# Fastaxx/Penguin.jl

Measured on AMD Instinct MI355X. Metric: time-steps/sec + SpMV GB/s (% HBM roofline), 3D mono diffusion 512^3, higher is better.
Workload: dtype f64

## Files before the change

### include/penguin_hip.h

```cpp
#ifndef PENGUIN_HIP_H
#define PENGUIN_HIP_H

#include <stddef.h>
#include <stdint.h>

#ifdef __cplusplus
extern "C" {
#endif

typedef struct pg_mesh pg_mesh;
typedef struct pg_capacity pg_capacity;
typedef struct pg_diffops pg_diffops;
typedef struct pg_solver pg_solver;
typedef struct pg_streamvort pg_streamvort;

enum { PG_BODY_BALL = 1, PG_BODY_MULTIBALL = 2, PG_BODY_HALFSPACE = 3, PG_BODY_ELLIPSOID = 4, PG_BODY_PLANE = 5 };
enum { PG_FLAG_COMPLEMENT = 1, PG_FLAG_NO_CENTROIDS = 2 };
enum { PG_CAP_V = 0, PG_CAP_GAMMA = 1, PG_CAP_CELL_TYPES = 2, PG_CAP_A = 3, PG_CAP_B = 4,
       PG_CAP_W = 5, PG_CAP_C_OMEGA = 6, PG_CAP_C_GAMMA = 7,
       PG_CAP_ST_V0 = 8, PG_CAP_ST_V1 = 9, PG_CAP_ST_CT_OMEGA = 10, PG_CAP_ST_CT_GAMMA = 11 };
enum { PG_OP_G = 0, PG_OP_H = 1, PG_OP_WINV = 2,
       PG_OP_C0 = 3 , PG_OP_K0 = 6  };
enum { PG_BC_NONE = 0, PG_BC_DIRICHLET = 1, PG_BC_NEUMANN = 2, PG_BC_ROBIN = 3, PG_BC_PERIODIC = 4 };
enum { PG_KEY_LEFT = 0 , PG_KEY_RIGHT = 1 , PG_KEY_BOTTOM = 2 ,
// ... 15 lines not shown
typedef struct {
  int32_t key;
  int32_t kind;
  double value;
} pg_border_desc;

typedef struct {
  double alpha1, alpha2, g;
  double beta1, beta2, h;
  const double* g_array;
  const double* h_array;
} pg_jump_desc;

typedef struct {
  int32_t method;
  double reltol;
  double abstol;
  int32_t maxiter;
  int32_t check_every;
  int32_t warm_start;
  int32_t restart;
  int32_t precond;
} pg_krylov_opts;
enum { PG_PRECOND_MG = -2 };
enum { PG_PRECOND_MG_CELL = -3 };
enum { PG_PRECOND_POLY_EST = -4 };
enum { PG_PRECOND_MG_STEP = -5 };
#define PG_SPECEST_MARGIN 0.0205

typedef struct {
  int32_t steps;
  int32_t admitted;
  int32_t gershgorin_admits;
  int32_t reserved;
  double g_ritz;
  double g_used;
  double margin;
  double gershgorin;
  double ritz_re_min, ritz_re_max, ritz_im_max;
  double estimate_ms;
} pg_specest_info;

#define PG_MG_MAX_LEVELS 16
typedef struct {
  int32_t levels;
  int32_t tail_level;
  int64_t rows[PG_MG_MAX_LEVELS];
  int64_t nnz[PG_MG_MAX_LEVELS];
  double setup_ms;
  int64_t bytes;
} pg_mg_info;

typedef struct {
  int32_t iters;
  int32_t converged;
  double resnorm;
  double bnorm;
  double extremum;
  double time;
} pg_step_info;

typedef struct {
  int64_t steps;
  int64_t total_iters;
  double t_final;
  double extremum;
  double solve_ms;
  double spmv_ms_total;
  int64_t spmv_launches;
  int64_t unconverged_steps;
  double worst_relres;
  double spmv_lean_ms_total;
  int64_t spmv_lean_launches;
  int64_t poly_degree;
  int64_t half_exits;
  int64_t poly_xspace;
  int64_t products;
  int64_t guess_states_read;
  int64_t poly_f32_launches;
  double poly_f32_ms_total;
  int64_t poly_f32_timed;
  int64_t poly_f32_chains;
  int64_t poly_f32_tail_sum;
} pg_run_info;

typedef struct {
  int64_t n_own;
  int64_t nnz;
  int64_t n_ghost;
  int64_t n_omega;
  int64_t n_gamma;
  int64_t M_global;
  int64_t spmv_bytes;
  int64_t spmv_slices;
  int64_t rows_uniform;
  int64_t rows_pattern;
  int64_t rows_irregular;
  int64_t neumann_ok;
  double gershgorin;
  int64_t spmv_units;
  int64_t rows_marched;
  int64_t rows_matrix;
  int64_t n_ghost_loop;
  int64_t loop_is_compact;
  int64_t rows_edge;
} pg_system_info;

typedef struct {
  int64_t steps;
  int64_t psi_iters;
  int64_t omega_iters;
  int64_t psi_products;
  int64_t omega_products;
  int64_t unconverged;
  double worst_relres;
  double t_final;
  double total_ms;
  double psi_ms;
  double velocity_ms;
  double build_ms;
  double omega_ms;
} pg_streamvort_run_info;

int32_t pg_last_error(char* buf, size_t n);
int32_t pg_init(int32_t device_id);
int32_t pg_get_unique_id(void* out128);
int32_t pg_init_distributed(int32_t device_id, int32_t rank, int32_t nranks, const void* unique_id128);
int32_t pg_finalize(void);
int32_t pg_device_synchronize(void);
int32_t pg_set_profiling(int32_t on);
int32_t pg_device_name(char* buf, size_t n);
int32_t pg_config_string(char* buf, size_t n);

int32_t pg_mesh_create(int32_t N, const int64_t* n, const double* L, const double* x0, pg_mesh** out);
int32_t pg_mesh_destroy(pg_mesh* m);
int32_t pg_mesh_get_centers(const pg_mesh* m, int32_t d, double* out, int64_t len);
int32_t pg_mesh_get_nodes(const pg_mesh* m, int32_t d, double* out, int64_t len);
int32_t pg_mesh_num_border_cells(const pg_mesh* m, int64_t* out);
int32_t pg_mesh_get_border_cells(const pg_mesh* m, int64_t* idx, double* pos, int32_t* key);

int32_t pg_capacity_create_levelset(pg_mesh* m, int32_t body_kind, const double* params, int32_t nparams,
                                    int32_t flags, pg_capacity** out);
int32_t pg_capacity_create_from_arrays(pg_mesh* m, const double* V, const double* const* A,
                                       const double* const* B, const double* const* W, const double* Gamma,
                                       const double* const* C_omega, const double* const* C_gamma,
                                       const double* cell_types, pg_capacity** out);
typedef struct {
  int32_t body_kind;
  int32_t flags;
  int32_t axis;
  int32_t nq;
  double sign;
  double t0, t1;
  const double* nodes;
  double body0[4], body1[4];
} pg_motion_desc;
int32_t pg_capacity_create_spacetime(pg_mesh* m, const pg_motion_desc* motion, pg_capacity** out);
int32_t pg_capacity_set_spacetime(pg_capacity* c, double t0, double t1, const double* V_t0, const double* V_t1,
                                  const double* Ct_omega, const double* Ct_gamma);
int32_t pg_capacity_destroy(pg_capacity* c);
int32_t pg_capacity_get(const pg_capacity* c, int32_t field, int32_t d, double* out, int64_t len);
int32_t pg_capacity_kernel_ms(const pg_capacity* c, double* ms);

int32_t pg_diffops_create(pg_capacity* c, pg_diffops** out);
int32_t pg_diffops_destroy(pg_diffops* o);
int32_t pg_diffops_export_csc(const pg_diffops* o, int32_t which, int64_t* colptr, int64_t* rowval,
                              double* nzval, int64_t* nnz);
int32_t pg_diffops_set_velocity(pg_diffops* o, const double* const* u_omega, const double* u_gamma);
int32_t pg_diffops_set_velocity_spacetime(pg_diffops* o, const double* const* u_omega, const double* u_gamma);
int32_t pg_diffops_grad(const pg_diffops* o, const double* p , double* out );
int32_t pg_diffops_div(const pg_diffops* o, const double* qw , const double* qg ,
                       double* out );

int32_t pg_solver_create_unsteady_mono(pg_capacity* c, pg_diffops* o, const pg_bc_desc* bc_interface,
                                       const pg_border_desc* borders, int32_t nborders, const double* Dcoef,
                                       const double* source, double dt, const double* T0, int32_t scheme,
                                       pg_solver** out);
int32_t pg_solver_create_unsteady_diph(pg_capacity* c1, pg_diffops* o1, pg_capacity* c2, pg_diffops* o2,
                                       const pg_jump_desc* ic, const pg_border_desc* borders, int32_t nborders,
                                       const double* D1, const double* D2, const double* f1, const double* f2,
                                       double dt, const double* T0, int32_t scheme, pg_solver** out);
int32_t pg_solver_create_moving_diph(pg_capacity* c1, pg_diffops* o1, pg_capacity* c2, pg_diffops* o2, const pg_jump_desc* ic,
                                     const pg_border_desc* borders, int32_t nborders, const double* D1, const double* D2,
                                     const double* f1_n, const double* f1_np1, const double* f2_n, const double* f2_np1,
                                     const double* T_prev, pg_solver* previous, int32_t scheme, pg_solver** out);
int32_t pg_solver_create_steady_mono(pg_capacity* c, pg_diffops* o, const pg_bc_desc* bc_interface,
                                     const pg_border_desc* borders, int32_t nborders, const double* Dcoef,
                                     const double* source, pg_solver** out);
// ... 164 lines not shown
```

### penguin/jl_amd/_lib.py

```python
from __future__ import annotations

import ctypes as C
import os
import re
from pathlib import Path

import numpy as np

_HERE = Path(__file__).resolve().parent
LIB_PATH = Path(os.environ["PG_LIB_PATH"]) if os.environ.get("PG_LIB_PATH") else _HERE / "lib" / "libpenguin_hip.so"
HEADER_PATH = _HERE.parent.parent / "include" / "penguin_hip.h"


class PenguinHipError(RuntimeError):
    pass


PG_BODY_BALL, PG_BODY_MULTIBALL, PG_BODY_HALFSPACE, PG_BODY_ELLIPSOID, PG_BODY_PLANE = 1, 2, 3, 4, 5
PG_FLAG_COMPLEMENT, PG_FLAG_NO_CENTROIDS = 1, 2
PG_CAP_V, PG_CAP_GAMMA, PG_CAP_CELL_TYPES, PG_CAP_A, PG_CAP_B, PG_CAP_W, PG_CAP_C_OMEGA, PG_CAP_C_GAMMA = range(8)
PG_CAP_ST_V0, PG_CAP_ST_V1, PG_CAP_ST_CT_OMEGA, PG_CAP_ST_CT_GAMMA = 8, 9, 10, 11
PG_OP_G, PG_OP_H, PG_OP_WINV = 0, 1, 2
PG_OP_C0, PG_OP_K0 = 3, 6
PG_BC_NONE, PG_BC_DIRICHLET, PG_BC_NEUMANN, PG_BC_ROBIN, PG_BC_PERIODIC = 0, 1, 2, 3, 4
PG_KEY = {"left": 0, "right": 1, "bottom": 2, "top": 3, "backward": 4, "forward": 5}
PG_SCHEME = {"BE": 0, "CN": 1, "STEADY": 2}
PG_METHOD = {"bicgstab": 0, "cg": 1, "gmres": 2, "bicgstabl": 3}
PG_METHOD_IDRS = 4
PG_SV_PSI, PG_SV_OMEGA, PG_SV_U, PG_SV_V = 0, 1, 2, 3
PG_PRECOND_MG = -2
PG_PRECOND_MG_CELL = -3
PG_PRECOND_POLY_EST = -4
PG_PRECOND_MG_STEP = -5
PG_SPECEST_MARGIN = 0.0205
PG_MG_MAX_LEVELS = 16

c_double_p = C.POINTER(C.c_double)
c_i64_p = C.POINTER(C.c_int64)
c_i32_p = C.POINTER(C.c_int32)


class pg_bc_desc(C.Structure):
    _fields_ = [("kind", C.c_int32), ("alpha", C.c_double), ("beta", C.c_double), ("value", C.c_double),
                ("value_array", c_double_p)]


class pg_border_desc(C.Structure):
    _fields_ = [("key", C.c_int32), ("kind", C.c_int32), ("value", C.c_double)]


class pg_jump_desc(C.Structure):
    _fields_ = [("alpha1", C.c_double), ("alpha2", C.c_double), ("g", C.c_double), ("beta1", C.c_double),
                ("beta2", C.c_double), ("h", C.c_double), ("g_array", c_double_p), ("h_array", c_double_p)]


class pg_motion_desc(C.Structure):
    _fields_ = [("body_kind", C.c_int32), ("flags", C.c_int32), ("axis", C.c_int32), ("nq", C.c_int32), ("sign", C.c_double),
                ("t0", C.c_double), ("t1", C.c_double), ("nodes", c_double_p), ("body0", C.c_double * 4),
                ("body1", C.c_double * 4)]


class pg_krylov_opts(C.Structure):
    _fields_ = [("method", C.c_int32), ("reltol", C.c_double), ("abstol", C.c_double), ("maxiter", C.c_int32),
                ("check_every", C.c_int32), ("warm_start", C.c_int32), ("restart", C.c_int32), ("precond", C.c_int32)]


class pg_step_info(C.Structure):
    _fields_ = [("iters", C.c_int32), ("converged", C.c_int32), ("resnorm", C.c_double), ("bnorm", C.c_double),
                ("extremum", C.c_double), ("time", C.c_double)]


class pg_run_info(C.Structure):
    _fields_ = [("steps", C.c_int64), ("total_iters", C.c_int64), ("t_final", C.c_double), ("extremum", C.c_double),
                ("solve_ms", C.c_double), ("spmv_ms_total", C.c_double), ("spmv_launches", C.c_int64),
                ("unconverged_steps", C.c_int64), ("worst_relres", C.c_double), ("spmv_lean_ms_total", C.c_double),
                ("spmv_lean_launches", C.c_int64), ("poly_degree", C.c_int64), ("half_exits", C.c_int64),
                ("poly_xspace", C.c_int64), ("products", C.c_int64), ("guess_states_read", C.c_int64),
                ("poly_f32_launches", C.c_int64), ("poly_f32_ms_total", C.c_double), ("poly_f32_timed", C.c_int64),
                ("poly_f32_chains", C.c_int64), ("poly_f32_tail_sum", C.c_int64)]


class pg_system_info(C.Structure):
    _fields_ = [("n_own", C.c_int64), ("nnz", C.c_int64), ("n_ghost", C.c_int64), ("n_omega", C.c_int64),
                ("n_gamma", C.c_int64), ("M_global", C.c_int64), ("spmv_bytes", C.c_int64), ("spmv_slices", C.c_int64),
                ("rows_uniform", C.c_int64), ("rows_pattern", C.c_int64), ("rows_irregular", C.c_int64),
                ("neumann_ok", C.c_int64), ("gershgorin", C.c_double), ("spmv_units", C.c_int64),
                ("rows_marched", C.c_int64), ("rows_matrix", C.c_int64), ("n_ghost_loop", C.c_int64),
                ("loop_is_compact", C.c_int64), ("rows_edge", C.c_int64)]


class pg_streamvort_run_info(C.Structure):
    _fields_ = [("steps", C.c_int64), ("psi_iters", C.c_int64), ("omega_iters", C.c_int64), ("psi_products", C.c_int64),
                ("omega_products", C.c_int64), ("unconverged", C.c_int64), ("worst_relres", C.c_double), ("t_final", C.c_double),
                ("total_ms", C.c_double), ("psi_ms", C.c_double), ("velocity_ms", C.c_double), ("build_ms", C.c_double),
                ("omega_ms", C.c_double)]


class pg_mg_info(C.Structure):
    _fields_ = [("levels", C.c_int32), ("tail_level", C.c_int32), ("rows", C.c_int64 * PG_MG_MAX_LEVELS),
                ("nnz", C.c_int64 * PG_MG_MAX_LEVELS), ("setup_ms", C.c_double), ("bytes", C.c_int64)]


class pg_specest_info(C.Structure):
    _fields_ = [("steps", C.c_int32), ("admitted", C.c_int32), ("gershgorin_admits", C.c_int32), ("reserved", C.c_int32),
                ("g_ritz", C.c_double), ("g_used", C.c_double), ("margin", C.c_double), ("gershgorin", C.c_double),
                ("ritz_re_min", C.c_double), ("ritz_re_max", C.c_double), ("ritz_im_max", C.c_double), ("estimate_ms", C.c_double)]


def declared_symbols() -> list[str]:
    txt = HEADER_PATH.read_text()
    return sorted(set(re.findall(r"\bint32_t\s+(pg_[a-z0-9_]+)\s*\(", txt)))


_lib = None
hip_runtime_source = "system"


def _share_the_hip_runtime_with_torch() -> None:
    global hip_runtime_source
    import sys

    if "torch" in sys.modules:
        hip_runtime_source = "already mapped by torch"
        return
    if os.environ.get("PG_HIP_RUNTIME", "auto") == "system":
        return
    import importlib.util

    try:
        spec = importlib.util.find_spec("torch")
    except (ImportError, ValueError):
        spec = None
    if spec is None or not spec.submodule_search_locations:
        return
    libdir = Path(list(spec.submodule_search_locations)[0]) / "lib"
    if not (libdir / "libamdhip64.so").exists():
        return
    mode = C.RTLD_GLOBAL if hasattr(C, "RTLD_GLOBAL") else 0
    for name in ("libhsa-runtime64.so", "libamdhip64.so"):
        if (libdir / name).exists():
            C.CDLL(str(libdir / name), mode=mode)
    hip_runtime_source = "torch wheel"


def lib() -> C.CDLL:
    global _lib
    if _lib is None:
        if not LIB_PATH.exists():
            raise PenguinHipError(
                f"{LIB_PATH} is missing: build it with `python -c 'import __graft_entry__ as g; g.build()'` "
                "(hipcc --offload-arch=gfx950).  penguin.jl_amd has no CPU fallback.")
        _share_the_hip_runtime_with_torch()
        _lib = C.CDLL(str(LIB_PATH), mode=C.RTLD_GLOBAL if hasattr(C, "RTLD_GLOBAL") else 0)
        for name in declared_symbols():
            getattr(_lib, name).restype = C.c_int32
    return _lib


def check(status: int) -> None:
    if status != 0:
        buf = C.create_string_buffer(4096)
        lib().pg_last_error(buf, 4096)
        raise PenguinHipError(buf.value.decode("utf-8", "replace"))


def dptr(a: np.ndarray):
    assert a.dtype == np.float64 and a.flags["C_CONTIGUOUS"]
    return a.ctypes.data_as(c_double_p)


def iptr(a: np.ndarray):
# ... 93 lines not shown
def debug_mg_step_aggregates(handle, which: int, level: int) -> np.ndarray:
    n = C.c_int64(0)
    check(lib().pg_debug_mg_step_aggregates(handle, C.c_int32(which), C.c_int32(level), C.byref(n), None))
    agg = np.zeros(max(n.value, 1), dtype=np.int32)
    check(lib().pg_debug_mg_step_aggregates(handle, C.c_int32(which), C.c_int32(level), C.byref(n), agg.ctypes.data_as(c_i32_p)))
    return agg[: n.value]


def debug_mg_step_level_csr(handle, which: int, level: int):
    n, nnz = C.c_int64(0), C.c_int64(0)
    w = C.c_int32(which)
    check(lib().pg_debug_mg_step_level_csr(handle, w, C.c_int32(level), C.byref(n), C.byref(nnz), None, None, None))
    rowptr, col, val = np.zeros(n.value + 1, dtype=np.int64), np.zeros(max(nnz.value, 1), dtype=np.int64), np.zeros(max(nnz.value, 1))
    check(lib().pg_debug_mg_step_level_csr(handle, w, C.c_int32(level), C.byref(n), C.byref(nnz), iptr(rowptr), iptr(col), dptr(val)))
    return rowptr, col[: nnz.value], val[: nnz.value]


def debug_mg_step_apply(handle, which: int, r: np.ndarray) -> np.ndarray:
    r = np.ascontiguousarray(r, dtype=np.float64)
    z = np.zeros_like(r)
    check(lib().pg_debug_mg_step_apply(handle, C.c_int32(which), dptr(r), dptr(z)))
    return z


def solver_spectral_estimate(handle, which: int = 0, run: bool = True) -> dict:
    info = pg_specest_info()
    check(lib().pg_solver_spectral_estimate(handle, C.c_int32(which | (0 if run else 4)), C.byref(info)))
    return {k: getattr(info, k) for k, _ in pg_specest_info._fields_ if k != "reserved"}


def debug_specest_hessenberg(handle, which: int = 0, run: bool = True) -> np.ndarray:
    w = C.c_int32(which | (0 if run else 4))
    k = C.c_int32(0)
    check(lib().pg_debug_specest_hessenberg(handle, w, C.byref(k), None))
    H = np.zeros((k.value + 1) * max(k.value, 1))
    check(lib().pg_debug_specest_hessenberg(handle, w, C.byref(k), dptr(H)))
    return H[: (k.value + 1) * k.value].reshape((k.value + 1, k.value), order="F")


DEBUG_SPMV_SENTINEL = 0x7FF8C0DE5EED0BAD
DEBUG_SPMV_GUARD = 64


def debug_spmv_sizes(handle, which: int) -> tuple[int, int, int, int]:
    n, nv, nnz, grid = C.c_int64(0), C.c_int64(0), C.c_int64(0), C.c_int32(0)
    check(lib().pg_debug_spmv_sizes(handle, C.c_int32(which), C.byref(n), C.byref(nv), C.byref(nnz), C.byref(grid)))
    return n.value, nv.value, nnz.value, grid.value


def loop_system_csr(handle, which: int):
    n, _, nnz, _ = debug_spmv_sizes(handle, which)
    rowptr, col, val = np.zeros(n + 1, dtype=np.int64), np.zeros(max(nnz, 1), dtype=np.int64), np.zeros(max(nnz, 1))
    check(lib().pg_solver_get_system_csr(handle, C.c_int32(which), iptr(rowptr), iptr(col), dptr(val), None, None))
    return rowptr, col[:nnz], val[:nnz]


def debug_spmv_apply(handle, which: int, variant: int, mode: int, x, aux=None, dotx=None, base=None, pc=(0.0, 0.0, 0.0),
                     fold: int = 0, done: int = 0, repeat: int = 1) -> dict:
    n, nv, _, grid = debug_spmv_sizes(handle, which)

    def arr(a, length, name):
        if a is None:
            return None, None
        a = np.ascontiguousarray(a, dtype=np.float64)
        if a.size != length:
            raise ValueError(f"debug_spmv_apply: {name} has {a.size} entries, the matrix needs {length}")
        return a, dptr(a)

    xs, xp = arr(x, nv, "x")
    auxs, auxp = arr(aux, n, "aux")
    dots, dotp = arr(dotx, n, "dotx")
    bases, basep = arr(base, n, "base")
    y = np.zeros(n + DEBUG_SPMV_GUARD)
    partials = np.zeros((5, grid))
    sums, folded = np.zeros(5), np.zeros(5)
    ticket = C.c_int64(-1)
    check(lib().pg_debug_spmv_apply(handle, C.c_int32(which), C.c_int32(variant), C.c_int32(mode), xp, auxp, dotp, basep,
                                    C.c_double(pc[0]), C.c_double(pc[1]), C.c_double(pc[2]), C.c_int32(fold), C.c_int32(done),
                                    C.c_int32(repeat), dptr(y), dptr(partials), dptr(sums), dptr(folded), C.byref(ticket)))
    return {"y": y, "partials": partials, "slot_sums": sums, "folded": folded, "ticket": ticket.value, "grid": grid, "n": n}


DEBUG_SPMV_SENTINEL_F32 = 0x7FC5EED0
TYPED_FIRST, TYPED_MIDDLE, TYPED_HANDOVER = 1, 2, 3


def debug_spmv_apply_typed(handle, which: int, kind: int, x, base=None, pc=(0.0, 0.0, 0.0), sigma: float = 1.0, done: int = 0) -> dict:
    n, nv, _, _ = debug_spmv_sizes(handle, which)
    want_x = np.float64 if kind == TYPED_FIRST else np.float32
    want_b = {TYPED_FIRST: None, TYPED_MIDDLE: np.float32, TYPED_HANDOVER: np.float64}[kind]
    x = np.ascontiguousarray(x)
    if x.dtype != want_x or x.size != nv:
        raise ValueError(f"debug_spmv_apply_typed: x must be {nv} x {np.dtype(want_x).name}")
    if (base is None) != (want_b is None):
        raise ValueError("debug_spmv_apply_typed: base goes with kinds 2 and 3, and only with them")
    bp = None
    if base is not None:
        base = np.ascontiguousarray(base)
        if base.dtype != want_b or base.size != n:
            raise ValueError(f"debug_spmv_apply_typed: base must be {n} x {np.dtype(want_b).name}")
        bp = base.ctypes.data_as(C.c_void_p)
    y64 = np.zeros(n + DEBUG_SPMV_GUARD) if kind == TYPED_HANDOVER else None
    y32 = np.zeros(n + DEBUG_SPMV_GUARD, dtype=np.float32) if kind != TYPED_HANDOVER else None
    p32 = np.zeros(n + DEBUG_SPMV_GUARD, dtype=np.float32) if kind == TYPED_FIRST else None
    ptr = lambda a: None if a is None else a.ctypes.data_as(C.c_void_p)
    check(lib().pg_debug_spmv_apply_typed(handle, C.c_int32(which), C.c_int32(kind), x.ctypes.data_as(C.c_void_p), bp,
                                          C.c_double(pc[0]), C.c_double(pc[1]), C.c_double(pc[2]), C.c_double(sigma), C.c_int32(done),
                                          ptr(y64), ptr(y32), ptr(p32)))
    return {"y": y64 if kind == TYPED_HANDOVER else y32, "p32": p32}
```

### penguin/jl_amd/csrc/pg_common.h

```cpp
#pragma once
#include <hip/hip_runtime.h>
#include "pg_rccl.h"

#include <chrono>
#include <cstdint>
#include <cstdio>
#include <cstring>
#include <stdexcept>
#include <string>
#include <vector>

#include "../../../include/penguin_hip.h"

namespace pg {

using i64 = int64_t;
using i32 = int32_t;

struct Error : std::runtime_error {
  using std::runtime_error::runtime_error;
};

void set_last_error(const std::string& msg);

#define PG_HIP(expr)                                                                              \
  do {                                                                                            \
    hipError_t _e = (expr);                                                                       \
    if (_e != hipSuccess)                                                                         \
      throw pg::Error(std::string("HIP error: ") + hipGetErrorString(_e) + " at " + __FILE__ + ":" + \
                      std::to_string(__LINE__) + " (" #expr ")");                                 \
  } while (0)

#define PG_NCCL(expr)                                                                             \
  do {                                                                                            \
    ncclResult_t _e = (expr);                                                                     \
    if (_e != ncclSuccess)                                                                        \
      throw pg::Error(std::string("RCCL error: ") + pg::rccl::api().GetErrorString(_e) + " at " + __FILE__ + ":" + \
                      std::to_string(__LINE__) + " (" #expr ")");                                 \
  } while (0)

#define PG_REQUIRE(cond, msg)                                   \
  do {                                                          \
    if (!(cond)) throw pg::Error(std::string(msg));             \
  } while (0)

#define PG_API_BEGIN try {
#define PG_API_END                                  \
  return 0;                                         \
  }                                                 \
  catch (const std::exception& e) {                 \
    pg::set_last_error(e.what());                   \
    return 1;                                       \
  }                                                 \
  catch (...) {                                     \
    pg::set_last_error("unknown exception");        \
    return 2;                                       \
  }

struct Config {
  bool debug = false;
  int alloc_poison = 0;
  int async_alloc = 0;
  int alloc_guard = 0;
  long long pool_limit_mb = 0;
  bool poly = true;
  int poly_degree = 6;
  bool poly_adapt = true;
  double poly_margin = 1.0;
  double poly_slack = -1.0;
  int poly_hist = 3;
  bool poly_trend = true;
  int poly_maxdeg = 0;
  int poly_mindeg = 4;
  bool poly_f32 = true;
  int poly_f32_tail = -1;
  int profile_sample = 3;
  bool gamma_elim = true;
  bool diag_elim = true;
  double diag_elim_frac = 0.0005;
  int spmv_variant = 70;
  int spmv_xcd = 1;
  int spmv_strip = 16;
  int spmv_march_k = 0;
  int spmv_minrun = 24;
  bool spmv_march = true;
  bool spmv_edges = true;
  int spmv_tile_units = 0;
  int spmv_blocks_per_cu = 0;
  bool halo_overlap = true;
  int guess_n = 4;
  int guess_depth = 7;
  bool guess_defer = true;
  bool guess_always = false;
  int guess_monitor = 256;
  double guess_pass_cost = 0.34;
  double guess_gain = 0.8;
  bool speculate_product = true;
  int mg_tail_rows = 2048;
  int unit_order = 0;
};
const Config& config();

struct LocalComm;

struct Context {
  bool inited = false;
  LocalComm* local = nullptr;
  int device = 0;
  hipStream_t stream = nullptr;
  hipStream_t comm_stream = nullptr;
  hipEvent_t ev_fork = nullptr, ev_join = nullptr;
  int rank = 0, nranks = 1;
  ncclComm_t comm = nullptr;
  ncclComm_t comm_halo = nullptr;
  bool profiling = false;
  std::string device_name;
};
Context& ctx();
void require_init();
void set_thread_context(Context* c);
Context* thread_context();
LocalComm* local_comm_create(int nranks);
void local_comm_destroy(LocalComm* c);
void comm_allreduce_sum_f64(double* dev, int count, hipStream_t st);
void comm_allreduce_max_f64(double* dev, int count, hipStream_t st);
void comm_allreduce_sum_u64(unsigned long long* dev, i64 count, hipStream_t st);

void* dev_alloc(size_t bytes);
void dev_free(void* p);
void dev_cache_release();
struct AsyncAllocScope {
  AsyncAllocScope();
  ~AsyncAllocScope();
};

template <class T>
struct DevBuf {
  T* p = nullptr;
  i64 n = 0;
  DevBuf() = default;
  explicit DevBuf(i64 n_) { alloc(n_); }
  DevBuf(const DevBuf&) = delete;
  DevBuf& operator=(const DevBuf&) = delete;
  DevBuf(DevBuf&& o) noexcept : p(o.p), n(o.n) { o.p = nullptr; o.n = 0; }
  DevBuf& operator=(DevBuf&& o) noexcept {
    if (this != &o) { release(); p = o.p; n = o.n; o.p = nullptr; o.n = 0; }
    return *this;
  }
  ~DevBuf() { release(); }
  void release() {
    if (p) dev_free(p);
    p = nullptr; n = 0;
  }
  void alloc(i64 n_) {
    release();
    n = n_;
    if (n > 0) p = static_cast<T*>(dev_alloc(sizeof(T) * static_cast<size_t>(n) + 64));
// ... 121 lines not shown
```

### penguin/jl_amd/csrc/pg_context.hip

```cpp
#include "pg_common.h"

#include <cxxabi.h>
#include <execinfo.h>

#include <atomic>
#include <map>
#include <mutex>
#include <unordered_map>
#include <unordered_set>
#include "pg_host_algos.h"

#include <algorithm>
#include <array>
#include <memory>
#include <set>

namespace pg {

static thread_local std::string g_last_error;
void set_last_error(const std::string& msg) { g_last_error = msg; }

Context& ctx() {
  static Context c;
  Context* t = thread_context();
  return t ? *t : c;
}

const Config& config() {
  static const Config c = [] {
    Config k;
    auto geti = [](const char* name, long long dflt) { const char* v = getenv(name); return v ? atoll(v) : dflt; };
    auto getd = [](const char* name, double dflt) { const char* v = getenv(name); return v ? atof(v) : dflt; };
    k.debug = getenv("PG_DEBUG") != nullptr;
    k.alloc_poison = (int)geti("PG_ALLOC_POISON", 0);
    k.async_alloc = (int)geti("PG_ASYNC_ALLOC", 0);
    k.alloc_guard = (int)geti("PG_ALLOC_GUARD", 0);
    k.pool_limit_mb = geti("PG_POOL_LIMIT_MB", 0);
    k.poly = geti("PG_POLY", 1) != 0;
    k.poly_degree = (int)geti("PG_POLY_DEGREE", 6);
    k.poly_adapt = geti("PG_POLY_ADAPT", getenv("PG_POLY_DEGREE") ? 0 : 1) != 0;
    k.poly_margin = getd("PG_POLY_MARGIN", 1.0);
    k.poly_slack = getd("PG_POLY_SLACK", -1.0);
    k.poly_hist = (int)std::max<long long>(1, std::min<long long>(3, geti("PG_POLY_HIST", 3)));
    k.poly_maxdeg = (int)geti("PG_POLY_MAXDEG", 0);
    k.poly_mindeg = (int)std::max<long long>(2, std::min<long long>(8, geti("PG_POLY_MINDEG", 4)));
    k.poly_trend = geti("PG_POLY_TREND", 1) != 0;
    k.poly_f32 = geti("PG_POLY_F32", 1) != 0;
    k.poly_f32_tail = (int)std::max<long long>(-1, std::min<long long>(64, geti("PG_POLY_F32_TAIL", -1)));
    k.profile_sample = (int)std::max<long long>(1, geti("PG_PROFILE_SAMPLE", 3));
    k.gamma_elim = geti("PG_GAMMA_ELIM", 1) != 0;
    k.diag_elim = geti("PG_DIAG_ELIM", 1) != 0;
    k.diag_elim_frac = getd("PG_DIAG_ELIM_FRAC", 0.0005);
    k.spmv_variant = (int)geti("PG_SPMV_VARIANT", 70);
    k.spmv_xcd = (int)geti("PG_SPMV_XCD", 1);
    k.spmv_strip = (int)geti("PG_SPMV_STRIP", 16);
    k.spmv_march_k = (int)geti("PG_SPMV_MARCH_K", 0);
    k.spmv_minrun = (int)geti("PG_SPMV_MINRUN", 24);
    k.spmv_march = geti("PG_SPMV_MARCH", 1) != 0;
    k.spmv_edges = geti("PG_SPMV_EDGES", 1) != 0;
    k.spmv_tile_units = (int)geti("PG_SPMV_TILE_UNITS", 0);
    k.spmv_blocks_per_cu = (int)geti("PG_SPMV_BLOCKS_PER_CU", 0);
    k.halo_overlap = geti("PG_HALO_OVERLAP", 1) != 0;
    k.speculate_product = geti("PG_SPECULATE", 1) != 0;
    k.guess_n = (int)std::max<long long>(0, std::min<long long>(4, geti("PG_GUESS_STATES", 4)));
    k.guess_depth = (int)std::max<long long>(1, std::min<long long>(7, geti("PG_GUESS_DEPTH", 7)));
    k.mg_tail_rows = (int)std::max<long long>(0, geti("PG_MG_TAIL_ROWS", 2048));
    k.guess_monitor = (int)std::max<long long>(1, geti("PG_GUESS_MONITOR", 256));
    k.guess_pass_cost = getd("PG_GUESS_PASS_COST", 0.34);
    k.guess_always = geti("PG_GUESS_ALWAYS", 0) != 0;
    k.guess_defer = geti("PG_GUESS_DEFER", 1) != 0;
    k.guess_gain = getd("PG_GUESS_GAIN", 0.8);
    k.unit_order = (int)geti("PG_SPMV_UNIT_ORDER", 0);
    return k;
  }();
  return c;
}

void require_init() {
  if (!ctx().inited)
    throw Error("penguin_hip: not initialised (call pg_init / pg_init_distributed first)");
}

static void init_device(int device_id) {
  Context& c = ctx();
  int ndev = 0;
  hipError_t e = hipGetDeviceCount(&ndev);
  if (e != hipSuccess || ndev <= 0)
    throw Error("penguin_hip: no HIP device visible -- this library has no CPU fallback");
  PG_REQUIRE(device_id >= 0 && device_id < ndev, "penguin_hip: device id out of range");
  PG_HIP(hipSetDevice(device_id));
  hipDeviceProp_t prop;
  PG_HIP(hipGetDeviceProperties(&prop, device_id));
  c.device = device_id;
  c.device_name = std::string(prop.name) + " (" + prop.gcnArchName + ")";
  if (!c.stream) PG_HIP(hipStreamCreateWithFlags(&c.stream, hipStreamNonBlocking));
  if (!c.comm_stream) PG_HIP(hipStreamCreateWithFlags(&c.comm_stream, hipStreamNonBlocking));
  c.inited = true;
}

}

using namespace pg;

namespace pg {
namespace {
thread_local int t_async_scope = 0;
std::mutex g_alloc_mutex;
struct BlockCache {
  std::multimap<size_t, void*> free_blocks;
  std::unordered_map<void*, size_t> owned;
  size_t free_bytes = 0;
};
BlockCache g_cache;
constexpr size_t CACHE_TRIM_BYTES = (size_t)48 << 30;

size_t round_block(size_t bytes) {
  const size_t q = bytes >= ((size_t)2 << 20) ? ((size_t)2 << 20) : 4096;
  return (bytes + q - 1) / q * q;
}

bool cache_wanted(const Context& c, size_t bytes) {
  const int mode = config().async_alloc;
  if (mode < 0 || !c.inited || !c.stream || c.local) return false;
  if (!(t_async_scope > 0 || mode > 0)) return false;
  const long long lim = config().pool_limit_mb;
  return lim <= 0 || bytes < ((size_t)lim << 20);
}

void poison(void* p, size_t bytes) {
  if (!config().alloc_poison || !p || bytes == 0) return;
// ... 157 lines not shown
  c.rank = 0;
  c.nranks = 1;
  PG_API_END
}

int32_t pg_get_unique_id(void* out128) {
  PG_API_BEGIN
  static_assert(sizeof(ncclUniqueId) == 128, "ncclUniqueId is expected to be 128 bytes");
  ncclUniqueId id;
  PG_NCCL(rccl::api().GetUniqueId(&id));
  std::memcpy(out128, &id, sizeof(id));
  PG_API_END
}

int32_t pg_init_distributed(int32_t device_id, int32_t rank, int32_t nranks, const void* unique_id128) {
  PG_API_BEGIN
  Context& c = ctx();
  PG_REQUIRE(nranks >= 1 && rank >= 0 && rank < nranks, "pg_init_distributed: bad rank / nranks");
  init_device(device_id);
  c.rank = rank;
  c.nranks = nranks;
  if (nranks > 1 || unique_id128 != nullptr) {
    PG_REQUIRE(unique_id128 != nullptr, "pg_init_distributed: unique id required when nranks > 1");
    ncclUniqueId id;
    std::memcpy(&id, unique_id128, sizeof(id));
    const rccl::Api& R = rccl::api();
    PG_NCCL(R.CommInitRank(&c.comm, nranks, id, rank));
    bool split_ok = false;
    if (R.CommSplit) {
      split_ok = R.CommSplit(c.comm, 0, rank, &c.comm_halo, nullptr) == ncclSuccess && c.comm_halo != nullptr;
      if (!split_ok) c.comm_halo = nullptr;
    }
    if (!split_ok) {
      ncclUniqueId id2;
      if (rank == 0) PG_NCCL(R.GetUniqueId(&id2));
      DevBuf<char> buf((i64)sizeof(id2));
      if (rank == 0) buf.upload(reinterpret_cast<const char*>(&id2), (i64)sizeof(id2));
      PG_NCCL(R.Broadcast(buf.p, buf.p, sizeof(id2), ncclChar, 0, c.comm, c.stream));
      buf.download(reinterpret_cast<char*>(&id2), (i64)sizeof(id2));
      PG_NCCL(R.CommInitRank(&c.comm_halo, nranks, id2, rank));
    }
  }
  PG_API_END
}

int32_t pg_finalize(void) {
  PG_API_BEGIN
  Context& c = ctx();
  if (c.inited) {
    (void)hipDeviceSynchronize();
    if (c.comm_halo) { (void)rccl::api().CommDestroy(c.comm_halo); c.comm_halo = nullptr; }
    if (c.comm) { (void)rccl::api().CommDestroy(c.comm); c.comm = nullptr; }
    dev_cache_release();
    if (c.stream) { (void)hipStreamDestroy(c.stream); c.stream = nullptr; }
    if (c.comm_stream) { (void)hipStreamDestroy(c.comm_stream); c.comm_stream = nullptr; }
    if (c.ev_fork) { (void)hipEventDestroy(c.ev_fork); c.ev_fork = nullptr; }
    if (c.ev_join) { (void)hipEventDestroy(c.ev_join); c.ev_join = nullptr; }
    c.inited = false;
  }
  PG_API_END
}

int32_t pg_device_synchronize(void) {
  PG_API_BEGIN
  require_init();
  PG_HIP(hipDeviceSynchronize());
  PG_API_END
}

int32_t pg_set_profiling(int32_t on) {
  PG_API_BEGIN
  ctx().profiling = on != 0;
  PG_API_END
}

int32_t pg_config_string(char* buf, size_t n) {
  PG_API_BEGIN
  const Config& k = config();
  char tmp[1024];
  snprintf(tmp, sizeof(tmp),
           "spmv_variant=%d spmv_xcd=%d spmv_strip=%d spmv_unit_order=%d spmv_march=%d spmv_edges=%d spmv_march_k=%d spmv_minrun=%d spmv_tile_units=%d "
           "spmv_blocks_per_cu=%d halo_overlap=%d speculate=%d poly=%d poly_degree=%d poly_adapt=%d "
           "poly_margin=%g poly_slack=%g poly_hist=%d poly_trend=%d poly_maxdeg=%d poly_f32=%d poly_f32_tail=%d gamma_elim=%d diag_elim=%d "
           "guess_states=%d guess_depth=%d guess_defer=%d async_alloc=%d cache_limit_mb=%lld alloc_poison=%d alloc_guard=%d profile_sample=%d debug=%d",
           k.spmv_variant, k.spmv_xcd, k.spmv_strip, k.unit_order, (int)k.spmv_march, (int)k.spmv_edges, k.spmv_march_k, k.spmv_minrun, k.spmv_tile_units,
           k.spmv_blocks_per_cu, (int)k.halo_overlap, (int)k.speculate_product, (int)k.poly, k.poly_degree, (int)k.poly_adapt,
           k.poly_margin, k.poly_slack, k.poly_hist, (int)k.poly_trend, k.poly_maxdeg, (int)k.poly_f32, k.poly_f32_tail,
           (int)k.gamma_elim, (int)k.diag_elim, k.guess_n, k.guess_depth, (int)k.guess_defer, k.async_alloc, k.pool_limit_mb, k.alloc_poison, k.alloc_guard, k.profile_sample, (int)k.debug);
  if (buf && n > 0) {
    std::strncpy(buf, tmp, n - 1);
    buf[n - 1] = 0;
  }
  PG_API_END
}

int32_t pg_device_name(char* buf, size_t n) {
  PG_API_BEGIN
  require_init();
  if (buf && n > 0) {
    std::strncpy(buf, ctx().device_name.c_str(), n - 1);
    buf[n - 1] = 0;
  }
  PG_API_END
}

int32_t pg_mesh_create(int32_t N, const int64_t* n, const double* L, const double* x0, pg_mesh** out) {
  PG_API_BEGIN
  PG_REQUIRE(N >= 1 && N <= 3, "pg_mesh_create: N must be 1, 2 or 3");
  PG_REQUIRE(out != nullptr, "pg_mesh_create: out is NULL");
  PG_REQUIRE(n != nullptr && L != nullptr, "pg_mesh_create: n / L is NULL");
  std::unique_ptr<pg_mesh> guard(new pg_mesh());
  pg_mesh* m = guard.get();
  m->N = N;
  for (int d = 0; d < N; ++d) {
    PG_REQUIRE(n[d] >= 1, "pg_mesh_create: n_d must be >= 1");
    m->n[d] = n[d];
    m->L[d] = L[d];
    m->x0[d] = x0 ? x0[d] : 0.0;
    const double h = L[d] / static_cast<double>(n[d]);
    m->centers[d].resize(n[d]);
    m->nodes[d].resize(n[d] + 1);
    for (i64 j = 0; j < n[d]; ++j) m->centers[d][j] = m->x0[d] + static_cast<double>(j) * h;
    for (i64 j = 0; j <= n[d]; ++j) m->nodes[d][j] = m->x0[d] + (static_cast<double>(j) + 0.5) * h;
  }
  if (ctx().inited) {
    for (int d = 0; d < N; ++d) {
      m->d_nodes[d].alloc(n[d] + 1);
      m->d_nodes[d].upload(m->nodes[d].data(), n[d] + 1);
    }
  }
  *out = guard.release();
  PG_API_END
}

int32_t pg_mesh_destroy(pg_mesh* m) {
  PG_API_BEGIN
  delete m;
  PG_API_END
}

int32_t pg_mesh_get_centers(const pg_mesh* m, int32_t d, double* out, int64_t len) {
  PG_API_BEGIN
  PG_REQUIRE(m && d >= 0 && d < m->N && len == m->n[d], "pg_mesh_get_centers: bad arguments");
  std::memcpy(out, m->centers[d].data(), sizeof(double) * len);
  PG_API_END
}

int32_t pg_mesh_get_nodes(const pg_mesh* m, int32_t d, double* out, int64_t len) {
  PG_API_BEGIN
  PG_REQUIRE(m && d >= 0 && d < m->N && len == m->n[d] + 1, "pg_mesh_get_nodes: bad arguments");
  std::memcpy(out, m->nodes[d].data(), sizeof(double) * len);
  PG_API_END
}

int32_t pg_mesh_num_border_cells(const pg_mesh* m, int64_t* out) {
  PG_API_BEGIN
  PG_REQUIRE(m && out, "pg_mesh_num_border_cells: bad arguments");
  i64 all = 1, inner = 1;
  for (int d = 0; d < m->N; ++d) {
    all *= m->n[d];
    inner *= std::max<i64>(m->n[d] - 2, 0);
  }
  *out = all - inner;
  PG_API_END
}

int32_t pg_mesh_get_border_cells(const pg_mesh* mc, int64_t* idx, double* pos, int32_t* key) {
  PG_API_BEGIN
  PG_REQUIRE(mc, "pg_mesh_get_border_cells: mesh is NULL");
  pg_mesh* m = const_cast<pg_mesh*>(mc);
  mesh_build_border(m);
// ... 102 lines not shown
```

### penguin/jl_amd/csrc/pg_host_algos.h

```cpp
#pragma once
#include <algorithm>
#include <cmath>
#include <cstdint>
#include <vector>

namespace pghost {

inline void partition_planes(const int64_t* weight, int64_t nplanes, int nranks, int64_t* bounds) {
  std::vector<double> cum(nplanes + 1, 0.0);
  for (int64_t k = 0; k < nplanes; ++k) cum[k + 1] = cum[k] + static_cast<double>(weight[k]) + 1.0;
  const double total = cum[nplanes];
  bounds[0] = 0;
  for (int r = 1; r < nranks; ++r) {
    const double target = total * r / nranks;
    int64_t k = std::lower_bound(cum.begin(), cum.end(), target) - cum.begin();
    if (k > 0 && (target - cum[k - 1]) < (cum[k] - target)) --k;
    const int64_t lo = bounds[r - 1] + 1;
    const int64_t hi = nplanes - (nranks - r);
    bounds[r] = std::min(std::max(k, lo), hi);
  }
  bounds[nranks] = nplanes;
}

constexpr int SLAB_MAX_KINDS = 4;
struct SlabNumbering {
  int K = 0;
  int64_t n_own = 0, n_ghost = 0;
  int64_t cnt_own[SLAB_MAX_KINDS], off_own[SLAB_MAX_KINDS], cntL[SLAB_MAX_KINDS], offL[SLAB_MAX_KINDS], cntU[SLAB_MAX_KINDS],
      offU[SLAB_MAX_KINDS], sendL_off[SLAB_MAX_KINDS], sendL_cnt[SLAB_MAX_KINDS], sendU_off[SLAB_MAX_KINDS], sendU_cnt[SLAB_MAX_KINDS];
};
inline void slab_numbering(int K, const int64_t* posO, const int64_t* posU, const int64_t* posFE, const int64_t* posLB,
                           const int64_t* tot, bool has_lower, bool has_upper, SlabNumbering& out) {
  out.K = K;
  int64_t off = 0;
  for (int k = 0; k < K; ++k) {
    out.cntL[k] = posO[k];
    out.cnt_own[k] = posU[k] - posO[k];
    out.cntU[k] = tot[k] - posU[k];
    out.off_own[k] = off;
    off += out.cnt_own[k];
  }
  out.n_own = off;
  for (int k = 0; k < K; ++k) { out.offL[k] = off; off += out.cntL[k]; }
  for (int k = 0; k < K; ++k) { out.offU[k] = off; off += out.cntU[k]; }
  out.n_ghost = off - out.n_own;
  for (int k = 0; k < K; ++k) {
    out.sendL_off[k] = out.off_own[k];
    out.sendL_cnt[k] = has_lower ? posFE[k] - posO[k] : 0;
    out.sendU_cnt[k] = has_upper ? posU[k] - posLB[k] : 0;
    out.sendU_off[k] = out.off_own[k] + out.cnt_own[k] - out.sendU_cnt[k];
  }
  for (int k = K; k < SLAB_MAX_KINDS; ++k)
    out.cnt_own[k] = out.off_own[k] = out.cntL[k] = out.offL[k] = out.cntU[k] = out.offU[k] = out.sendL_off[k] = out.sendL_cnt[k] =
        out.sendU_off[k] = out.sendU_cnt[k] = 0;
}

struct SlabPlanes { int64_t s0, s1, a0, a1; };
inline SlabPlanes slab_planes(int64_t p0, int64_t p1, int64_t nplanes, int halo) {
  SlabPlanes g;
  g.s0 = p0 - halo < 0 ? 0 : p0 - halo;
  g.s1 = p1 + halo > nplanes ? nplanes : p1 + halo;
  g.a0 = p0 - 1 < 0 ? 0 : p0 - 1;
  g.a1 = p1 + 1 > nplanes ? nplanes : p1 + 1;
  return g;
}

struct MRun {
  int r0, len, cnt;
};
struct RowRange {
  int64_t a, b;
  int cnt;
};
struct MarchGeometry {
  int K, KS;
  int REC;
  int W;
  int INFO;
  int kmax;
  int64_t ext0 = 0, lines = 0;
  int strip = 0;
  int unit_order = 0;
};

struct EdgeCands {
  const int* rows = nullptr;
  int64_t nrows = 0;
  const int* rowptr = nullptr;
  const int* col = nullptr;
};
constexpr int EDGE_SLOTS = 8;
constexpr int EDGE_PER_END = 8;
constexpr int EDGE_PER_UNIT = 64;
constexpr int EDGE_REC = 34;
struct EdgePlan {
  EdgeCands cand;
  std::vector<int> meta;
  int64_t rows_e = 0;
  int64_t slots_read = 0;
};

inline int64_t march_order(int64_t cell, int64_t ext0, int64_t lines, int strip) {
  const int64_t line = (cell / ext0) % lines, plane = cell / (ext0 * lines);
  return (line / strip) * ((int64_t)1 << 20) + plane;
}

inline void plan_march_units(int64_t n, const std::vector<MRun>& runs, const std::vector<int>& info, const MarchGeometry& geo,
                             std::vector<int>& mrec, std::vector<RowRange>& fallback, int64_t& rows_m,
                             std::vector<int64_t>* okeys = nullptr, EdgePlan* edges = nullptr) {
  typedef int64_t i64;
  rows_m = 0;
  const i64 nr = (i64)runs.size();
  const int RI = geo.INFO;
  auto off = [&](i64 i, int k) { return info[RI * i + k]; };
  auto same_values = [&](i64 i, i64 j, int cnt) {
    for (int k = 0; k < 2 * cnt; ++k)
      if (info[RI * i + 8 + k] != info[RI * j + 8 + k]) return false;
    return true;
  };
  std::vector<char> ok(nr, 0);
  for (i64 i = 0; i < nr; ++i) {
    const int cnt = runs[i].cnt;
    bool good = (cnt == 5 || cnt == 7) && off(i, 0) == 1 && off(i, 1) == -1 && off(i, cnt - 1) == 0;
    if (good) {
      const int up_e = cnt - 3, dn_e = cnt - 2;
      good = off(i, up_e) > 1 && off(i, dn_e) < -1;
      if (good && cnt == 7) good = off(i, 2) > 1 && off(i, 2) < off(i, up_e) && off(i, 3) < -1 && off(i, 3) > off(i, dn_e);
    }
    ok[i] = good;
    if (!ok[i]) fallback.push_back(RowRange{runs[i].r0, (i64)runs[i].r0 + runs[i].len, cnt});
  }
  std::vector<int> succ(nr, -1), pred(nr, -1);
  for (i64 i = 0; i < nr; ++i) {
    if (!ok[i]) continue;
    const int cnt = runs[i].cnt, up_off = off(i, cnt - 3);
    const i64 lo = (i64)runs[i].r0 + up_off, hi = lo + runs[i].len;
    i64 j = std::upper_bound(runs.begin(), runs.end(), lo, [](i64 v, const MRun& r) { return v < (i64)r.r0; }) - runs.begin();
    if (j > 0) --j;
    i64 best = -1, best_ov = 0;
    for (; j < nr && (i64)runs[j].r0 < hi; ++j) {
      const i64 a = runs[j].r0, b = a + runs[j].len;
      if (b <= lo || j == i || !ok[j] || pred[j] >= 0 || runs[j].cnt != cnt || off(j, cnt - 2) != -up_off || !same_values(i, j, cnt)) continue;
      const i64 ov = std::min(hi, b) - std::max(lo, a);
      if (ov > best_ov) { best_ov = ov; best = j; }
    }
    if (best >= 0) { succ[i] = (int)best; pred[best] = (int)i; }
  }
  struct Unit { int key; int64_t order; int64_t sub; std::vector<int> rec; std::vector<int> erows; };
  const bool want_edges = edges && edges->cand.nrows > 0 && geo.REC >= EDGE_REC + 2 + geo.K;
  std::vector<char> claimed(want_edges ? (size_t)edges->cand.nrows : 0, 0);
  auto edge_row = [&](i64 row, i64 run, int cnt, int& smap, i64& q) {
    const EdgeCands& c = edges->cand;
    if (row < 0 || row >= n) return false;
    q = std::lower_bound(c.rows, c.rows + c.nrows, (int)row) - c.rows;
    if (q >= c.nrows || c.rows[q] != row || claimed[q]) return false;
    const int a = c.rowptr[q], len = c.rowptr[q + 1] - a;
    if (len < 1 || len > cnt) return false;
    auto inside = [&](int s) { const i64 t = row + off(run, s); return t >= 0 && t < n; };
    int sl = 0;
    smap = len << 24;
    for (int e = 0; e < len; ++e) {
      const i64 cc = c.col[a + e];
      if (cc < 0 || cc >= n) return false;
      while (sl < cnt && off(run, sl) != cc - row) {
        if (!inside(sl)) return false;
        ++sl;
      }
      if (sl == cnt) return false;
      smap |= sl << (3 * e);
      ++sl;
    }
    for (; sl < cnt; ++sl)
      if (!inside(sl)) return false;
    return true;
  };
  const bool aligned = geo.unit_order == 1 && geo.strip > 0 && geo.ext0 > 0 && geo.lines > 0 && RI > 24;
  auto plane_of = [&](i64 run) -> i64 {
    const i64 cell = info[RI * run + 24];
    return cell >= 0 ? cell / (geo.ext0 * geo.lines) : -1;
  };
  std::vector<Unit> units;
  auto safe = [&](i64 idx0) { return idx0 >= 0 && idx0 + 130 <= n + 8; };
  std::vector<i64> chain, B;
  for (i64 h = 0; h < nr; ++h) {
    if (!ok[h] || pred[h] >= 0) continue;
    chain.clear(); B.clear();
    const int cnt = runs[h].cnt;
    const bool Y = cnt == 7;
    const int up_e = cnt - 3, dn_e = cnt - 2;
    i64 base = runs[h].r0;
    for (i64 i = h; i >= 0; i = succ[i]) {
      chain.push_back(i);
      B.push_back(base);
      base += off(i, up_e);
    }
    const i64 L = (i64)chain.size();
    i64 cmin = 0, cmax = 0;
    for (i64 k = 0; k < L; ++k) {
      const i64 a = runs[chain[k]].r0 - B[k], b = a + runs[chain[k]].len;
      cmin = k == 0 ? a : std::min(cmin, a);
      cmax = k == 0 ? b : std::max(cmax, b);
    }
    for (i64 W = cmin - 1; W + 1 < cmax; W += geo.W) {
      auto range = [&](i64 k, i64& lo, i64& hi) {
        const i64 a = runs[chain[k]].r0 - B[k], b = a + runs[chain[k]].len;
        lo = std::max(a, W + 1);
        hi = std::min(b, W + 1 + geo.W);
        return lo < hi;
      };
      i64 k = 0;
      while (k < L) {
        i64 lo, hi;
        if (!range(k, lo, hi)) { ++k; continue; }
        i64 k1 = k;
        while (k1 < L && k1 - k < geo.kmax && range(k1, lo, hi)) {
          ++k1;
          if (aligned && Y && k1 < L && plane_of(chain[k1]) >= 0 && plane_of(chain[k1]) % geo.kmax == 0) break;
        }
        const int K = (int)(k1 - k);
        bool fits = safe(B[k] + off(chain[k], dn_e) + W) && safe(B[k1 - 1] + off(chain[k1 - 1], up_e) + W);
        for (i64 q = k; q < k1 && fits; ++q) {
          fits = safe(B[q] + W);
          if (Y) fits = fits && safe(B[q] + W + off(chain[q], 2)) && safe(B[q] + W + off(chain[q], 3));
        }
        if (!fits) {
          for (i64 q = k; q < k1; ++q) {
            range(q, lo, hi);
            fallback.push_back(RowRange{B[q] + lo, B[q] + hi, cnt});
          }
          k = k1;
          continue;
        }
        Unit u;
        u.rec.assign(geo.REC, 0);
        range(k, lo, hi);
        u.key = (int)(B[k] + lo);
        u.order = 0;
        u.sub = 0;
        if (Y && geo.strip > 0 && geo.ext0 > 0 && geo.lines > 0 && RI > 24) {
          const i64 cell = info[RI * chain[k] + 24];
          if (cell >= 0) {
            u.order = march_order(cell, geo.ext0, geo.lines, geo.strip);
            if (aligned) {
              const i64 line = (cell / geo.ext0) % geo.lines, plane = cell / (geo.ext0 * geo.lines);
              u.order = (line / geo.strip) * ((i64)1 << 20) + plane / geo.kmax;
              const i64 x0 = cell % geo.ext0 + ((B[k] + lo) - (i64)runs[chain[k]].r0);
              u.sub = (x0 / geo.W) * ((i64)1 << 20) + line;
            }
          }
        }
        const int Kp = K <= geo.KS ? geo.KS : geo.K;
        u.rec[0] = Kp | (cnt << 8);
        u.rec[1] = u.key;
        for (int q = 0; q < 2 * cnt; ++q) u.rec[2 + q] = info[RI * chain[k] + 8 + q];
        u.rec[16] = (int)(B[k] + off(chain[k], dn_e) + W);
        u.rec[17] = (int)(B[k1 - 1] + off(chain[k1 - 1], up_e) + W);
        int hi_max = 0;
        for (int i = 0; i < K; ++i) {
          const i64 q = k + i;
          range(q, lo, hi);
          hi_max = std::max(hi_max, (int)(hi - W));
          u.rec[18 + 4 * i] = (int)(B[q] + W);
          u.rec[19 + 4 * i] = Y ? off(chain[q], 3) : 0;
          u.rec[20 + 4 * i] = Y ? off(chain[q], 2) : 0;
          u.rec[21 + 4 * i] = (int)(lo - W) | ((int)(hi - W) << 8);
          rows_m += hi - lo;
        }
        if (want_edges) {
          int budget = EDGE_PER_UNIT;
          for (int i = 0; i < K; ++i) {
            const i64 q = k + i, run = chain[q];
            range(q, lo, hi);
            const i64 a = runs[run].r0 - B[q], b = a + runs[run].len;
            std::vector<int> lows, highs;
            int smap = 0;
            i64 cq = 0;
            if (lo == a)
              for (i64 pos = lo - 1; pos >= W + 1 && lo - pos <= EDGE_PER_END && budget > 0 && edge_row(B[q] + pos, run, cnt, smap, cq); --pos) {
                claimed[cq] = 1; --budget;
                lows.push_back(smap); lows.push_back((int)(B[q] + pos));
              }
            if (hi == b)
              for (i64 pos = hi; pos <= W + geo.W && pos - hi < EDGE_PER_END && budget > 0 && edge_row(B[q] + pos, run, cnt, smap, cq); ++pos) {
                claimed[cq] = 1; --budget;
                highs.push_back((int)(B[q] + pos)); highs.push_back(smap);
              }
            const int nlo = (int)lows.size() / 2, nhi = (int)highs.size() / 2;
            u.rec[EDGE_REC + 2 + i] = nlo | (nhi << 8) | ((int)(u.erows.size() / 2) << 16);
            u.erows.insert(u.erows.end(), lows.rbegin(), lows.rend());
            u.erows.insert(u.erows.end(), highs.begin(), highs.end());
            hi_max = std::max(hi_max, (int)(hi - W) + nhi);
          }
          u.rec[EDGE_REC + 1] = (int)(u.erows.size() / 2);
          for (int i = K; i < Kp; ++i) u.rec[EDGE_REC + 2 + i] = u.rec[EDGE_REC + 1] << 16;
        }
        u.rec[0] |= std::min(64, hi_max / 2 + 1) << 16;
        for (int i = K; i < Kp; ++i) {
          u.rec[18 + 4 * i] = u.rec[17];
          u.rec[19 + 4 * i] = 0;
          u.rec[20 + 4 * i] = 0;
          u.rec[21 + 4 * i] = 1 | (1 << 8);
        }
        units.push_back(std::move(u));
        k = k1;
      }
    }
  }
  std::sort(units.begin(), units.end(), [](const Unit& a, const Unit& b) {
    if (a.order != b.order) return a.order < b.order;
    return a.sub != b.sub ? a.sub < b.sub : a.key < b.key;
  });
  mrec.reserve(units.size() * geo.REC);
  if (want_edges) {
    i64 first = 0;
    edges->meta.clear();
    edges->slots_read = 0;
    for (auto& u : units) {
      const int ne = (int)(u.erows.size() / 2);
      u.rec[EDGE_REC] = (int)first;
      for (int e = 0; e < ne; ++e) {
        edges->meta.push_back(u.erows[2 * e]);
        edges->meta.push_back((int)(EDGE_SLOTS * first + 2 * e));
        edges->meta.push_back(2 * ne);
        edges->meta.push_back(u.erows[2 * e + 1]);
      }
      first += ne;
      edges->slots_read += (int64_t)ne * ((((u.rec[0] >> 8) & 255) + 1) & ~1);
    }
    edges->rows_e = first;
  }
  for (auto& u : units) mrec.insert(mrec.end(), u.rec.begin(), u.rec.end());
  if (okeys) {
    okeys->clear();
    okeys->reserve(units.size());
    for (auto& u : units) okeys->push_back(u.order * ((i64)1 << 32) + u.key);
  }
}

inline void plan_tiles(const std::vector<int64_t>& ukey, const std::vector<int64_t>& skey, int T, std::vector<int>& tab) {
  typedef int64_t i64;
  const i64 nu = (i64)ukey.size(), ns = (i64)skey.size();
  tab.assign((size_t)8 * (T + 1) * 2, 0);
  for (int q = 0; q < 8; ++q) {
    const i64 u0 = nu * q / 8, u1 = nu * (q + 1) / 8, s0 = ns * q / 8, s1 = ns * (q + 1) / 8;
    i64 sprev = s0;
    for (int t = 0; t <= T; ++t) {
      const i64 u = u0 + (u1 - u0) * t / T;
      i64 sl;
      if (t == 0) sl = s0;
      else if (t == T || u >= nu) sl = s1;
      else sl = std::lower_bound(skey.begin(), skey.end(), ukey[u]) - skey.begin();
      sl = std::min(std::max(sl, sprev), s1);
      sprev = sl;
      tab[((size_t)q * (T + 1) + t) * 2] = (int)u;
      tab[((size_t)q * (T + 1) + t) * 2 + 1] = (int)sl;
    }
  }
}

inline bool mg_dense_inverse(int n, const double* a, double* inv) {
  if (n <= 0) return true;
  const size_t w = 2 * (size_t)n;
  std::vector<long double> m((size_t)n * w, 0.0L);
  for (int i = 0; i < n; ++i) {
    for (int j = 0; j < n; ++j) m[i * w + j] = a[(size_t)i * n + j];
    m[i * w + n + i] = 1.0L;
  }
  for (int c = 0; c < n; ++c) {
    int piv = c;
    long double best = m[c * w + c] < 0 ? -m[c * w + c] : m[c * w + c];
    for (int i = c + 1; i < n; ++i) {
      const long double v = m[i * w + c] < 0 ? -m[i * w + c] : m[i * w + c];
      if (v > best) { best = v; piv = i; }
    }
    if (!(best > 0.0L)) return false;
    if (piv != c)
      for (size_t j = 0; j < w; ++j) std::swap(m[c * w + j], m[piv * w + j]);
    const long double d = 1.0L / m[c * w + c];
    for (size_t j = 0; j < w; ++j) m[c * w + j] *= d;
// ... 309 lines not shown
```

### penguin/jl_amd/csrc/pg_krylov.h

```cpp
#pragma once
#include <functional>

#include "pg_system.h"

namespace pg {

struct MgHierarchy;

struct XGuess {
  const double* zbase = nullptr;
  const double* zr[8] = {nullptr, nullptr, nullptr, nullptr, nullptr, nullptr, nullptr, nullptr};
  const double* coef = nullptr;
};

struct KrylovWork {
  i64 n = 0, nvec = 0;
  DevBuf<double> r, rhat, p, v, t;
  DevBuf<double> partials;
  DevBuf<double> sc;
  double* h_sc = nullptr;
  int grid = 1;
  DevBuf<unsigned> ticket;
  double last_rate2 = 0.0;
  int last_iters = 0;
  const void* adapt_matrix = nullptr;
  int adapt_m = 0, adapt_h = 0;
  const void* need_matrix = nullptr;
  double need_hist[3] = {0.0, 0.0, 0.0};
  const void* fail_matrix = nullptr;
  int fail_deg = 0, good_deg = 0;
  double fail_L = 0.0;
  int fail_wait = 0, fail_backoff = 1;
  const int* scatter = nullptr;
  MgHierarchy* mg = nullptr;
  XGuess xguess;
  bool p_in_rhat = false;
  bool start_folded = false;
  const int* moved_flag = nullptr;
  int moved_stamp = 0;
  DevBuf<double> ya, yb, wa, wb;
  DevBuf<float> fa, fb, p32;
  const void* mix_matrix = nullptr;
  double mix_sigma = 0.0, mix_need = 0.0;
  int mix_wait = 0;
  DevBuf<double> gm_basis, gm, gm_partials;
  int gm_m = -1;
  DevBuf<double> bl_vecs, bl, bl_partials;
  int bl_l = -1;
  i64 bl_stride = 0;
  DevBuf<double> id_vecs, id, id_partials;
  int id_s = -1;
  i64 id_stride = 0;
  std::function<void()> after_first_batch;
  hipEvent_t ev_poll = nullptr;
  void init(i64 n_own, i64 n_vec);
  ~KrylovWork();
};

struct SolveStats {
  int iters = 0;
  int converged = 0;
  double resnorm = 0.0, bnorm = 0.0;
  double spmv_ms = 0.0, spmv_lean_ms = 0.0;
  i64 spmv_launches = 0, spmv_lean_launches = 0;
  int poly_degree = 0;
  int half_exit = 0;
  int poly_xspace = 0;
  i64 products = 0;
  int polls = 0;
  i64 f32_launches = 0, f32_timed = 0, f32_chains = 0, f32_tail_sum = 0;
  double f32_ms = 0.0;
};

void halo_exchange(const Numbering& nb, const Slab& slab, double* vec, hipStream_t st);
void halo_begin(const Numbering& nb, const Slab& slab, double* vec, hipStream_t st);
void halo_end(hipStream_t st);
void spmv(const CsrMatrix& A, const double* x, double* y, hipStream_t st);
void spmv_halo(const CsrMatrix& A, const Numbering& nb, const Slab& slab, double* x, double* y, hipStream_t st);
void krylov_solve(const CsrMatrix& A, const Numbering& nb, const Slab& slab, const double* b, double* x,
                  KrylovWork& w, const pg_krylov_opts& opts, SolveStats& stats, const double* x0 = nullptr,
                  const double* Ax0 = nullptr, bool preinit = false);

bool krylov_uses_polynomial(const CsrMatrix& A, const pg_krylov_opts& opts);

extern int g_poly_give_up;

void gmres_solve(const CsrMatrix& A, const Numbering& nb, const Slab& slab, const double* b, double* x, KrylovWork& w,
                 const pg_krylov_opts& opts, SolveStats& stats);

void bicgstabl_solve(const CsrMatrix& A, const Numbering& nb, const Slab& slab, const double* b, double* x, KrylovWork& w,
                     const pg_krylov_opts& opts, SolveStats& stats);
void idrs_solve(const CsrMatrix& A, const Numbering& nb, const Slab& slab, const double* b, double* x, KrylovWork& w,
                const pg_krylov_opts& opts, SolveStats& stats, const double* x0 = nullptr, const double* Ax0 = nullptr);
const char* krylov_method_refusal(int method);

}
```

### penguin/jl_amd/csrc/pg_krylov.hip

```cpp
#include "pg_host_algos.h"
#include "pg_krylov.h"
#include "pg_multigrid.h"
#include "pg_spmv.h"
#include "pg_specest.h"

using namespace pg;

namespace pg { extern double g_host_wait_us; }

namespace {


__global__ __launch_bounds__(BLOCK) void k_bicg_init(i64 n, i64 nvec, const double* __restrict__ b,
                                                     const double* x0, const double* __restrict__ Ax0,
                                                     double* x, double* __restrict__ r,
                                                     double* __restrict__ rhat, double* __restrict__ p,
                                                     double* __restrict__ v, double* __restrict__ partials,
                                                     const double* __restrict__ ds) {
  __shared__ double s_red[BLOCK / 64];
  double acc = 0.0, accb = 0.0, accw = 0.0;
  for (i64 i = blockIdx.x * (i64)BLOCK + threadIdx.x; i < nvec; i += (i64)gridDim.x * BLOCK) {
    if (i < n) {
      const double bi = b[i];
      const double ri = x0 ? bi - Ax0[i] : bi;
// ... 576 lines not shown
  int maxiter = opts.maxiter;
  if (maxiter <= 0) {
    maxiter = 100000;
  }
  struct HookReset { KrylovWork& w; ~HookReset() { w.after_first_batch = nullptr; } } hook_reset{w};
  const bool p_in_rhat = w.p_in_rhat && preinit && opts.method == PG_METHOD_BICGSTAB;
  w.p_in_rhat = false;
  const XGuess xg = w.xguess;
  w.xguess = XGuess();
  const bool start_folded = w.start_folded && preinit && opts.method == PG_METHOD_BICGSTAB;
  w.start_folded = false;
  const int* moved_flag = w.moved_flag;
  const int moved_stamp = w.moved_stamp;
  w.moved_flag = nullptr;
  const bool fused_start = !start_folded && preinit && opts.method == PG_METHOD_BICGSTAB && cx.nranks == 1 && !cx.comm;
  if (!fused_start && !start_folded)
    hipLaunchKernelGGL(k_sc_reset, dim3(1), dim3(S_COUNT), 0, st, w.sc.p, opts.reltol * opts.reltol, opts.abstol * opts.abstol);
  SpmvTimer timer(cx.profiling);

  const bool cg = opts.method == PG_METHOD_CG;
  const Config& cfg = config();
  const bool poly_env = cfg.poly;
  const int degree_env = cfg.poly_degree;
  int m = 0;
  const bool by_estimate = est_opt && !A.poly_ok && !A.poly_gave_up && A.est.tried && A.est.admitted;
  if (poly_env && precond >= 0 && !cg && (A.poly_ok || by_estimate) && spmv_supports_preconditioner_product() && n > 0)
    m = std::min(precond > 0 ? precond : degree_env, MAX_POLY_DEGREE);
  const bool adapt_env = cfg.poly_adapt;
  const bool adaptive = adapt_env && m >= 2 && precond == 0 && preinit;
  int expect_halves = 0;
  if (adaptive && w.adapt_matrix == &A && w.adapt_m >= 2) { m = w.adapt_m; expect_halves = w.adapt_h; }
  if (m < 2) m = 0;
  const bool poly = m > 0;
  MgHierarchy* const mgh = w.mg;
  w.mg = nullptr;
  const bool mg = mg_any_precond(opts.precond);
  if (mg) {
    PG_REQUIRE(!cg, "multigrid preconditioner refused: the method must be BiCGStab");
    PG_REQUIRE(spmv_supports_preconditioner_product(), "multigrid preconditioner refused: the x-space loop needs the slice kernel (PG_SPMV_VARIANT)");
    mg_require_one_rank_of(opts.precond);
    PG_REQUIRE(mgh && !w.scatter && !xg.zbase && n > 0,
               mg_is_step(opts.precond)
                   ? "multigrid preconditioner refused: this solve has no hierarchy (the full systems of the unsteady monophasic "
                     "diffusion time loop only)"
                   : "multigrid preconditioner refused: this solve has no hierarchy (steady monophasic "
                     "diffusion systems and the stream-function solve only)");
    PG_REQUIRE(mgh->rule == mg_rule_of_any(opts.precond) && mgh->matrix == &A,
               std::string("multigrid preconditioner: the hierarchy handed over was not built for precond = ") +
                   mg_precond_name_of(opts.precond));
  }
  const bool pre = poly || mg;
  stats.poly_degree = m;
  stats.poly_xspace = poly ? 1 : 0;
  PG_REQUIRE(!w.scatter || (poly && preinit), "a compact system needs the polynomial path and a prepared start");
  double tau[MAX_POLY_DEGREE];
  if (poly) {
    const double g = std::min(std::max(by_estimate ? A.est.g_used : A.gersh, 0.05), 0.95);
    double lam[MAX_POLY_DEGREE];
    for (int k = 0; k < m; ++k) lam[k] = 1.0 + g * std::cos(M_PI * (2.0 * k + 1.0) / (2.0 * m));
    for (int k = 0, lo = 0, hi = m - 1; k < m; ++k) tau[k] = 1.0 / ((k & 1) ? lam[hi--] : lam[lo++]);
  }
  if (pre && w.ya.n < nvec) {
    w.ya.alloc(nvec); w.wa.alloc(nvec); w.wb.alloc(nvec); w.yb.alloc(nvec);
    w.ya.zero(); w.wa.zero(); w.wb.zero(); w.yb.zero();
  }
  pghost::MixedChain mc;
  bool mixed = false;
  double mix_sigma = 1.0;
  double mtau[MAX_POLY_DEGREE];
  if (poly && cfg.poly_f32 && cx.nranks == 1 && !cx.comm && !A.halo_needed && spmv_supports_typed_chain() && w.mix_matrix == &A &&
      w.mix_sigma > 0.0) {
    const double g = std::min(std::max(by_estimate ? A.est.g_used : A.gersh, 0.05), 0.95);
    int j = cfg.poly_f32_tail >= 0 ? cfg.poly_f32_tail : pghost::mixed_chain_tail(w.mix_need, g, m);
    if (j >= 0 && w.mix_wait > 0 && cfg.poly_f32_tail < 0) j += 2;
    if (w.mix_wait > 0) --w.mix_wait;
    if (j >= 0 && pghost::mixed_chain_schedule(m, g, j, mc)) {
      mixed = true;
      mix_sigma = w.mix_sigma;
      for (int i = 0; i < m; ++i) mtau[i] = 1.0 / pghost::mixed_root(m, g, mc.order[i]);
      if (w.fa.n < nvec) {
        w.fa.alloc(nvec); w.fb.alloc(nvec); w.p32.alloc(nvec);
        w.fa.zero(); w.fb.zero(); w.p32.zero();
      }
    }
  }
  bool mixed_ran = false;
  const bool half_test = m >= 3 || mg;
  PG_REQUIRE(!xg.zbase || (poly && p_in_rhat && w.scatter), "an unformed extrapolated state needs the polynomial loop on a compact system");
  PG_REQUIRE(!preinit || !cg, "preinit is a BiCGStab path");
  if (!cg) {
    if (!preinit)
      hipLaunchKernelGGL(k_bicg_init, dim3(G), dim3(BLOCK), 0, st, n, nvec, b, x0, Ax0, x, w.r.p, w.rhat.p, w.p.p, w.v.p,
                       w.partials.p, (const double*)A.ds.p);
    static_assert(S_COUNT <= BLOCK, "k_start resets the scalar block with one thread per scalar");
    if (start_folded) {
    } else if (fused_start)
      hipLaunchKernelGGL(k_start, dim3(1), dim3(BLOCK), 0, st, (int)PH_INIT, 3, w.grid, (const double*)w.partials.p, w.sc.p,
                         opts.reltol * opts.reltol, opts.abstol * opts.abstol);
    else if (moved_flag && preinit && !(cx.nranks == 1 && !cx.comm)) {
      hipLaunchKernelGGL(k_start_sums_moved, dim3(1), dim3(BLOCK), 0, st, w.grid, (const double*)w.partials.p, w.sc.p, moved_flag,
                         moved_stamp);
      comm_allreduce_sum_f64(w.sc.p + S_RED0, 4, st);
      hipLaunchKernelGGL(k_derive_start_moved, dim3(1), dim3(1), 0, st, w.sc.p);
    } else
      finalize(PH_INIT, 3, w, st, false);
  } else {
    hipLaunchKernelGGL(k_cg_init, dim3(G), dim3(BLOCK), 0, st, n, nvec, b, x, w.r.p, w.p.p, w.partials.p, (const double*)A.ds.p);
    finalize(PH_CG_INIT, 2, w, st, false);
  }
  PG_HIP(hipGetLastError());

  int launched = 0, polls = 0;
  bool mid = false;
  bool done = false, poly_failed = false;
  const int poly_give_up = g_poly_give_up > 0 ? g_poly_give_up : 40 + 400 / std::max(m, 1);
  const int derive_here = (cx.nranks == 1 && !cx.comm) ? 1 : 0;
  auto apply = [&](double* in, double* out, int phase, int nslots, int itn) {
    const bool second = phase == PH_BICG_2;
    double* src = in;
    if (poly) {
      double* hat = second ? w.yb.p : w.ya.p;
      if (mixed && itn == 0 && !second) {
        const int n32 = mc.n32, nf32 = n32 + 1, nf64 = m - 1 - nf32;
        const void* src32 = nullptr;
        timer.begin(st, itn, true, second, nf32, true);
        for (int i = 0; i <= n32; ++i) {
          const double tk = mtau[i + 1];
          FinArgs f{nullptr, nullptr, PH_NONE, 0, 0, nullptr};
          if (i == 0) {
            float* dst = w.fa.p;
            f.pc0 = mix_sigma * mtau[0]; f.pc1 = -mix_sigma * (mtau[0] * tk); f.pc2 = mix_sigma * tk;
            f.base = in; f.p32 = w.p32.p; f.psig = mix_sigma;
            launch_spmv_typed(TYPED_FIRST, A, in, dst, w.sc.p, G, st, f);
            src32 = dst;
          } else if (i < n32) {
            float* dst = (i & 1) ? w.fb.p : w.fa.p;
            f.pc0 = 1.0; f.pc1 = -tk; f.pc2 = tk;
            f.base = reinterpret_cast<const double*>(w.p32.p);
            launch_spmv_typed(TYPED_MIDDLE, A, src32, dst, w.sc.p, G, st, f);
            src32 = dst;
          } else {
            double* dst = i == m - 2 ? hat : ((i & 1) ? w.wb.p : w.wa.p);
            const double inv = 1.0 / mix_sigma;
            f.pc0 = inv; f.pc1 = -inv * tk; f.pc2 = tk;
            f.base = in;
            launch_spmv_typed(TYPED_HANDOVER, A, src32, dst, w.sc.p, G, st, f);
            src = dst;
          }
        }
        timer.end(st);
        if (nf64 > 0) {
          timer.begin(st, itn, true, second, nf64);
          for (int i = n32 + 1; i <= m - 2; ++i) {
            double* dst = i == m - 2 ? hat : ((i & 1) ? w.wb.p : w.wa.p);
            FinArgs f{nullptr, nullptr, PH_NONE, 0, 0, nullptr};
            f.pc0 = 1.0; f.pc1 = -mtau[i + 1]; f.pc2 = mtau[i + 1]; f.base = in;
            launch_spmv(8, A, src, dst, nullptr, nullptr, w.sc.p, G, st, &f);
            src = dst;
          }
          timer.end(st);
        }
        mixed_ran = true;
        stats.f32_launches += nf32;
        stats.f32_chains += 1;
        stats.f32_tail_sum += mc.j;
      } else {
      timer.begin(st, itn, true, second, m - 1);
      for (int k = m - 2; k >= 0; --k) {
        double* dst = k == 0 ? hat : ((k & 1) ? w.wb.p : w.wa.p);
        FinArgs f{nullptr, nullptr, PH_NONE, 0, 0, nullptr};
        const double lead = k == m - 2 ? tau[m - 1] : 1.0;
        f.pc0 = lead; f.pc1 = -lead * tau[k]; f.pc2 = tau[k]; f.base = in;
        spmv_with_halo(8, A, nb, slab, src, dst, nullptr, nullptr, w.sc.p, G, st, &f);
        src = dst;
      }
      timer.end(st);
      }
    } else if (mg) {
      double* hat = second ? w.yb.p : w.ya.p;
      timer.begin(st, itn, true, second, 1);
      mg_apply(*mgh, A, nb, slab, in, hat, w.sc.p, st);
      timer.end(st);
      src = hat;
    }
    FinArgs f{w.ticket.p, w.sc.p, phase, nslots, derive_here, pre ? in : nullptr};
    timer.begin(st, itn, false, second);
    const bool folded = spmv_with_halo(phase == PH_BICG_1 ? 1 : 3, A, nb, slab, src, out, w.rhat.p, w.partials.p, w.sc.p, G, st, &f);
    timer.end(st);
    if (folded) finalize_folded(phase, nslots, w, st); else finalize(phase, nslots, w, st, true);
  };
  auto first_half = [&](int itn, bool test) {
    double* pvec = (p_in_rhat && itn == 0) ? w.rhat.p : w.p.p;
    apply(pvec, w.v.p, PH_BICG_1, 3, itn);
    unsigned* tk = (test && derive_here) ? w.ticket.p : nullptr;
    if (pre)
      hipLaunchKernelGGL(k_bicg_s_x, dim3(G), dim3(BLOCK), 0, st, n, w.sc.p, w.v.p, w.rhat.p, w.r.p, w.partials.p, (const double*)A.ds.p, tk,
                         p_in_rhat ? 1 : 0, (const double*)w.ya.p, x, w.scatter, xg, itn == 0 ? 1 : 0);
    else
      hipLaunchKernelGGL(k_bicg_s, dim3(G), dim3(BLOCK), 0, st, n, w.sc.p, w.v.p, w.rhat.p, w.r.p, w.partials.p, (const double*)A.ds.p, tk,
                         p_in_rhat ? 1 : 0);
    if (test && !tk) finalize(PH_BICG_S, 1, w, st, true, 4);
  };
  auto second_half = [&](int itn) {
    apply(w.r.p, w.t.p, PH_BICG_2, 5, itn);
    hipLaunchKernelGGL(k_bicg_xrp, dim3(G), dim3(BLOCK), 0, st, n, w.sc.p, w.t.p, w.v.p, x, w.r.p, w.p.p, w.rhat.p, w.partials.p,
                       (const double*)A.ds.p, p_in_rhat ? 1 : 0, pre ? (const double*)w.yb.p : nullptr, w.scatter);
  };
  while (!done) {
    int want = check_every;
    if (w.last_iters > 1) want = polls == 0 ? w.last_iters - 1 : (polls <= 4 ? 1 : check_every);
    if (expect_halves > 0) want = polls == 0 ? (expect_halves + 1) / 2 : (polls <= 4 ? 1 : check_every);
    const int batch = std::max(1, std::min(want, maxiter - launched));
    int halves = 2 * batch;
    if (half_test && expect_halves > 0 && polls == 0) halves = std::max(1, std::min(expect_halves, 2 * (maxiter - launched)));
    ++polls;
    if (!cg) {
      const bool predicted = half_test && expect_halves > 0 && polls == 1;
      for (int h = 0; h < halves; ++h) {
        if (!mid) {
          if (launched >= maxiter) break;
          first_half(launched, half_test && (!predicted || h + 2 >= halves));
          ++launched;
          mid = true;
        } else {
          second_half(launched - 1);
          mid = false;
        }
      }
    } else {
      for (int it = 0; it < batch; ++it) {
        timer.begin(st, launched + it);
        spmv_with_halo(2, A, nb, slab, w.p.p, w.v.p, nullptr, w.partials.p, w.sc.p, G, st);
        timer.end(st);
        finalize(PH_CG_1, 1, w, st, true);
        hipLaunchKernelGGL(k_cg_xr, dim3(G), dim3(BLOCK), 0, st, n, w.sc.p, w.p.p, w.v.p, x, w.r.p, w.partials.p, (const double*)A.ds.p);
        finalize(PH_CG_2, 2, w, st, true);
        hipLaunchKernelGGL(k_cg_p, dim3(G), dim3(BLOCK), 0, st, n, w.sc.p, w.r.p, w.p.p);
      }
      launched += batch;
    }
    if (!cg && !mid) finalize(PH_BICG_3, 2, w, st, true, 1);
    PG_HIP(hipGetLastError());
    PG_HIP(hipMemcpyAsync(w.h_sc, w.sc.p, sizeof(double) * S_COUNT, hipMemcpyDeviceToHost, st));
    const auto t_wait0 = std::chrono::steady_clock::now();
    struct WaitClock {
      std::chrono::steady_clock::time_point t0;
      ~WaitClock() { g_host_wait_us += std::chrono::duration<double, std::micro>(std::chrono::steady_clock::now() - t0).count(); }
    } wait_clock{t_wait0};
    if (w.after_first_batch && polls == 1) {
      if (!w.ev_poll) PG_HIP(hipEventCreateWithFlags(&w.ev_poll, hipEventDisableTiming));
      PG_HIP(hipEventRecord(w.ev_poll, st));
      std::function<void()> hook;
      hook.swap(w.after_first_batch);
      hook();
      PG_HIP(hipEventSynchronize(w.ev_poll));
    } else {
      PG_HIP(hipStreamSynchronize(st));
    }
    if (w.h_sc[S_DONE] != 0.0 || (launched >= maxiter && !mid)) done = true;
    if (!done && poly && launched >= poly_give_up) { poly_failed = true; done = true; }
  }
  if (poly_failed) {
    const_cast<CsrMatrix&>(A).poly_ok = false;
    const_cast<CsrMatrix&>(A).est.admitted = false;
    const_cast<CsrMatrix&>(A).poly_gave_up = true;
    timer.collect(stats, launched, false);
    if (w.scatter) {
      stats.iters = launched;
      stats.converged = 0;
      stats.poly_degree = -1;
      return;
    }
    if (cfg.debug) fprintf(stderr, "[pg_krylov] polynomial preconditioner (m = %d) stagnated after %d iterations: plain iteration\n", m, launched);
    spmv_with_halo(0, A, nb, slab, x, w.t.p, nullptr, nullptr, nullptr, G, st);
    SolveStats rest;
    krylov_solve(A, nb, slab, b, x, w, opts, rest, x, w.t.p, false);
    stats = rest;
    stats.iters += launched;
    return;
  }
  if (cfg.debug)
    fprintf(stderr, "[pg_krylov] done=%g iters=%g rr0=%g rr=%g tol2=%g rho=%g rho_old=%g alpha=%g omega=%g beta=%g red0=%g red1=%g\n",
            w.h_sc[S_DONE], w.h_sc[S_ITERS], w.h_sc[S_RR0], w.h_sc[S_RR], w.h_sc[S_TOL2], w.h_sc[S_RHO], w.h_sc[S_RHO_OLD], w.h_sc[S_ALPHA],
            w.h_sc[S_OMEGA], w.h_sc[S_BETA], w.h_sc[S_RED0], w.h_sc[S_RED1]);
  stats.iters = (int)w.h_sc[S_ITERS];
  stats.polls = polls;
  w.last_iters = stats.iters;
  stats.converged = w.h_sc[S_DONE] == 1.0 ? 1 : 0;
  stats.half_exit = w.h_sc[S_HALF] != 0.0 ? 1 : 0;
  stats.resnorm = std::sqrt((cg ? w.h_sc[S_RRW] : w.h_sc[S_RR]) + w.h_sc[S_HELD]);
  stats.bnorm = std::sqrt(w.h_sc[S_BB]);
  timer.collect(stats, stats.iters, w.h_sc[S_HALF] != 0.0);
  stats.products = (i64)(2 * stats.iters - stats.half_exit) * (m >= 2 ? m : 1);
  if (!cg && stats.converged && stats.products > 0) {
    const double rr0 = w.h_sc[S_RR0], rr = w.h_sc[S_HALF] != 0.0 ? w.h_sc[S_RED4] : w.h_sc[S_RR];
    if (rr0 > 0.0 && rr > 0.0 && rr < rr0) w.last_rate2 = std::log(rr0 / rr) / (double)stats.products;
  }
  const bool mix_env = poly && cfg.poly_f32 && cx.nranks == 1 && !cx.comm && !A.halo_needed && spmv_supports_typed_chain();
  choose_next_degree(A, stats, m, adaptive, w,
                     mix_env && cfg.poly_f32_tail < 0 ? std::min(std::max(by_estimate ? A.est.g_used : A.gersh, 0.05), 0.95) : 0.0);
  if (stats.iters == 0) stats.f32_launches = stats.f32_chains = stats.f32_tail_sum = 0;
  if (mixed_ran && expect_halves == 1 && !(stats.iters == 1 && stats.half_exit)) w.mix_wait = 2 * (m + 3);
  w.mix_matrix = nullptr;
  if (mix_env && stats.converged) {
    const double rr0 = w.h_sc[S_RR0], tol2 = w.h_sc[S_TOL2];
    if (rr0 > 0.0 && rr0 < 1e300 && tol2 > 0.0) {
      int e = 0;
      (void)std::frexp(std::sqrt(rr0 / (double)n), &e);
      const int h = (adaptive && w.adapt_matrix == &A && w.adapt_h >= 1) ? w.adapt_h : std::max(1, 2 * stats.iters - stats.half_exit);
      if (e > -100 && e < 100) {
        w.mix_matrix = &A;
        w.mix_sigma = std::ldexp(1.0, -e);
        w.mix_need = std::pow(std::sqrt(std::min(1.0, tol2 / rr0)), 1.0 / h);
      }
    }
  }
}

}
```

### penguin/jl_amd/csrc/pg_solver.hip

```cpp
#include <algorithm>
#include <cmath>
#include <memory>

#include "pg_krylov.h"
#include "pg_reduce.h"
#include "pg_multigrid.h"
#include "pg_program.h"
#include "pg_scan.h"
#include "pg_solver_internal.h"
#include "pg_spmv.h"
#include "pg_specest.h"

using namespace pg;

namespace pg { extern double g_host_wait_us; }

struct pg_solver {
  int nphase = 1;
  pg_capacity* cap[2] = {nullptr, nullptr};
  pg_diffops* ops[2] = {nullptr, nullptr};
  Slab slab;
  int K = 2;
  i64 Mloc = 0, M = 0;
  double dt = 0.0, t = 0.0;
// ... 2693 lines not shown
  PG_HIP(hipEventElapsedTime(&ms, ev.e0, ev.e1));
  *ms_per_eval = (double)ms / repeats;
  if (bytes) {
    const i64 n = s->nb.n_own;
    i64 b = (i64)M.G * M.K * 8;
    bool any_dense = false;
    for (int m = 0; m < M.K; ++m) {
      if (M.sparse[m]) b += MON_SPARSE_ENTRY_BYTES * M.stored[m];
      else { b += 8 * n; any_dense = true; }
    }
    if (any_dense) b += (s->x_valid ? 8 : 16) * n;
    *bytes = b;
  }
  PG_API_END
}

int32_t pg_debug_monitor_eval(pg_solver* s, double* values, int32_t* x_form) {
  PG_API_BEGIN
  require_init();
  PG_REQUIRE(s && values, "pg_debug_monitor_eval: NULL argument");
  const pg_solver::Monitors& M = s->mon;
  PG_REQUIRE(M.K > 0 && s->initial_done, "pg_debug_monitor_eval: monitors and a solved state are needed");
  DevBuf<double> out((i64)M.G * M.K);
  mon_launch(s, out.p, ctx().stream);
  std::vector<double> part((size_t)M.G * M.K);
  out.download(part.data(), (i64)M.G * M.K);
  for (int m = 0; m < M.K; ++m) {
    double v = 0.0;
    for (int g = 0; g < M.G; ++g) v += part[(size_t)g * M.K + m];
    values[m] = v;
  }
  if (x_form) *x_form = s->x_valid ? 1 : 0;
  PG_API_END
}

int32_t pg_solver_initial_solve(pg_solver* s, const pg_krylov_opts* opts, pg_step_info* info) {
  PG_API_BEGIN
  require_init();
  PG_REQUIRE(s, "Solver is not initialized. Call a solver constructor first.");
  SolveStats st;
  std::unique_ptr<AsyncAllocScope> pool(s->moving ? new AsyncAllocScope() : nullptr);
  do_initial(s, opts, st);
  mon_record(s);
  fill_info(s, st, info);
  PG_API_END
}

int32_t pg_solver_step(pg_solver* s, int32_t scheme, const pg_krylov_opts* opts, pg_step_info* info) {
  PG_API_BEGIN
  require_init();
  PG_REQUIRE(s, "Solver is not initialized. Call a solver constructor first.");
  PG_REQUIRE(scheme == PG_SCHEME_BE || scheme == PG_SCHEME_CN, "scheme must be BE or CN");
  SolveStats st;
  do_step(s, scheme, opts, st);
  mon_record(s);
  fill_info(s, st, info);
  PG_API_END
}

int32_t pg_solver_run(pg_solver* s, double Tend, int32_t scheme, const pg_krylov_opts* opts, int32_t do_initial_flag,
                      int64_t max_steps, int32_t save_every, pg_run_info* info) {
  PG_API_BEGIN
  require_init();
  PG_REQUIRE(s, "Solver is not initialized. Call a solver constructor first.");
  PG_REQUIRE(scheme == PG_SCHEME_BE || scheme == PG_SCHEME_CN, "scheme must be BE or CN");
  hipStream_t stream = ctx().stream;
  EventPair ev;
  const auto t_run0 = std::chrono::steady_clock::now();
  const double wait0 = pg::g_host_wait_us;
  PG_HIP(hipEventRecord(ev.e0, stream));
  double used0 = 0.0;
  if (s->guess_coef.n >= 16) s->guess_coef.download(&used0, 1, 13);
  SolveStats tot;
  i64 steps = 0, iters = 0, unconverged = 0;
  double worst = 0.0;
  auto account = [&](const SolveStats& st) {
    iters += st.iters; tot.spmv_ms += st.spmv_ms; tot.spmv_launches += st.spmv_launches;
    tot.spmv_lean_ms += st.spmv_lean_ms; tot.spmv_lean_launches += st.spmv_lean_launches;
    tot.poly_degree = st.poly_degree;
    tot.poly_xspace = st.poly_xspace;
    tot.half_exit += st.half_exit;
    tot.products += st.products;
    tot.f32_launches += st.f32_launches; tot.f32_ms += st.f32_ms; tot.f32_timed += st.f32_timed;
    tot.f32_chains += st.f32_chains; tot.f32_tail_sum += st.f32_tail_sum;
    if (!st.converged) ++unconverged;
    if (st.bnorm > 0.0) worst = std::max(worst, st.resnorm / st.bnorm);
  };
  if (s->mon.K > 0) {
    const i64 limit = 1 << 16;
    i64 rows = do_initial_flag ? 1 : 0, n = 0;
    for (double t = s->t; t < Tend && (max_steps < 0 || n < max_steps) && n < limit; t += s->dt) ++n;
    mon_reserve(s, rows + n);
  }
  if (do_initial_flag) {
    SolveStats st;
    do_initial(s, opts, st);
    mon_record(s);
    account(st);
    if (save_every > 0) keep_state(s);
  }
  while (s->t < Tend) {
    if (max_steps >= 0 && steps >= max_steps) break;
    SolveStats st;
    s->hint_more_steps = (s->t + s->dt < Tend) && (max_steps < 0 || steps + 1 < max_steps);
    struct HintReset { pg_solver* s; ~HintReset() { s->hint_more_steps = false; } } hint_reset{s};
    do_step(s, scheme, opts, st);
    mon_record(s);
    account(st);
    ++steps;
    if (save_every > 0 && steps % save_every == 0) keep_state(s);
  }
  PG_HIP(hipEventRecord(ev.e1, stream));
  PG_HIP(hipEventSynchronize(ev.e1));
  float ms = 0.f;
  PG_HIP(hipEventElapsedTime(&ms, ev.e0, ev.e1));
  if (config().debug && steps > 0) {
    const double wall_us = std::chrono::duration<double, std::micro>(std::chrono::steady_clock::now() - t_run0).count();
    fprintf(stderr, "[pg_solver_run] %lld steps: wall %.1f us per step, of which the host waited %.1f us for the device (the rest: queueing "
            "launches and bookkeeping); device time by events %.1f us per step\n", (long long)steps, wall_us / steps,
            (pg::g_host_wait_us - wait0) / steps, ms * 1e3 / steps);
  }
  if (info) {
    info->steps = steps;
    info->total_iters = iters;
    info->t_final = s->t;
    info->extremum = max_abs(s);
    info->solve_ms = ms;
    info->spmv_ms_total = tot.spmv_ms;
    info->spmv_launches = tot.spmv_launches;
    info->unconverged_steps = unconverged;
    info->worst_relres = worst;
    info->spmv_lean_ms_total = tot.spmv_lean_ms;
    info->spmv_lean_launches = tot.spmv_lean_launches;
    info->poly_degree = tot.poly_degree;
    info->poly_xspace = tot.poly_xspace;
    info->half_exits = tot.half_exit;
    info->products = tot.products;
    info->poly_f32_launches = tot.f32_launches;
    info->poly_f32_ms_total = tot.f32_ms;
    info->poly_f32_timed = tot.f32_timed;
    info->poly_f32_chains = tot.f32_chains;
    info->poly_f32_tail_sum = tot.f32_tail_sum;
    info->guess_states_read = 0;
    if (s->guess_coef.n >= 16) {
      double hc[16];
      s->guess_coef.download(hc, 16);
      info->guess_states_read = (int64_t)(hc[13] - used0);
    }
  }
  PG_API_END
}

int32_t pg_solver_num_states(const pg_solver* s, int64_t* out) {
  PG_API_BEGIN
  PG_REQUIRE(s && out, "pg_solver_num_states: NULL argument");
  *out = (int64_t)s->states.size();
  PG_API_END
}

int32_t pg_solver_get_state(const pg_solver* s, int64_t state_index, double* x, int64_t len) {
  PG_API_BEGIN
  require_init();
  PG_REQUIRE(s && x, "pg_solver_get_state: NULL argument");
  PG_REQUIRE(len == (i64)s->K * s->M, "pg_solver_get_state: len must be 2M (mono) or 4M (diph)");
  if (state_index < 0) materialize_x(const_cast<pg_solver*>(s));
  const double* src = s->x.p;
  if (state_index >= 0) {
    PG_REQUIRE(state_index < (i64)s->states.size(), "pg_solver_get_state: state index out of range");
    src = s->states[state_index].p;
  }
  hipStream_t st = ctx().stream;
  DevBuf<double> pad((i64)s->K * s->Mloc);
  pad.zero();
  if (s->nb.n_own > 0) {
    hipLaunchKernelGGL(k_scatter_active, dim3(grid_for(s->nb.n_own, BLOCK)), dim3(BLOCK), 0, st, make_segs(s->nb),
                       s->nb.n_own, s->Mloc, s->nb.row_cell.p, src, pad.p);
    PG_HIP(hipGetLastError());
  }
  const i64 own_lo = (s->slab.p0 - s->slab.s0) * s->slab.plane, own_n = (s->slab.p1 - s->slab.p0) * s->slab.plane;
  for (int k = 0; k < s->K; ++k)
    pad.download(x + (i64)k * s->M + s->slab.p0 * s->slab.plane, own_n, (i64)k * s->Mloc + own_lo);
  PG_API_END
}

int32_t pg_solver_system_info(const pg_solver* s, int32_t which, pg_system_info* out) {
  PG_API_BEGIN
  PG_REQUIRE(s && out, "pg_solver_system_info: NULL argument");
  const CsrMatrix& Af = ((which & 1) == 0 || !s->have_run) ? s->A_ctor : run_matrix(s);
  const GammaElim& E = (&Af == &s->A_ctor) ? s->elim_ctor : s->elim_run;
  const DiagElim& DE = (&Af == &s->A_ctor) ? s->diag_ctor : s->diag_run;
  const CsrMatrix& A = ((which & 4) && DE.active) ? DE.A : (((which & 4) && E.active) ? E.A : Af);
  out->n_own = s->nb.n_own;
  out->nnz = (which & 6) ? A.nnz : A.nnz_raw;
  out->n_ghost = s->nb.n_ghost;
  i64 nw = 0, ng = 0;
  for (int k = 0; k < s->K; ++k) ((k & 1) ? ng : nw) += s->nb.cnt_own[k];
  out->n_omega = nw;
  out->n_gamma = ng;
  out->M_global = s->M;
  out->spmv_bytes = A.spmv_bytes;
  out->spmv_slices = A.nslices;
  out->rows_uniform = A.rows_u;
  out->rows_pattern = A.rows_p + A.rows_e;
  out->rows_edge = A.rows_e;
  out->rows_irregular = A.rows_g;
  out->neumann_ok = A.poly_ok ? 1 : 0;
  out->gershgorin = A.gersh;
  out->spmv_units = A.nunits;
  out->rows_marched = A.rows_m;
  out->rows_matrix = A.n;
  out->n_ghost_loop = ((which & 4) && DE.active) ? DE.nb.n_ghost : s->nb.n_ghost;
  out->loop_is_compact = DE.active ? 1 : 0;
  PG_API_END
}

static const CsrMatrix& debug_matrix(const pg_solver* s, int32_t which, i64* nv);

int32_t pg_solver_get_system_csr(const pg_solver* s, int32_t which, int64_t* rowptr, int64_t* col, double* val, double* b,
                                 int64_t* idx) {
  PG_API_BEGIN
  require_init();
  PG_REQUIRE(s, "pg_solver_get_system_csr: NULL argument");
  const bool precond = (which & 2) != 0;
  const int sel = which & 1;
  if (sel == 1) PG_REQUIRE(s->have_run, "run matrix not assembled yet");
  if (which & 4) {
    PG_REQUIRE(precond, "pg_solver_get_system_csr: which = 6 / 7 (the loop's matrix is a preconditioned one)");
    PG_REQUIRE(!b && !idx, "pg_solver_get_system_csr: b and idx belong to the full system: NULL for which = 6 / 7");
    i64 nv = 0;
    const CsrMatrix& L = debug_matrix(s, which, &nv);
    if (rowptr) {
      std::vector<int> h(L.n + 1, 0);
      if (L.n > 0) L.rowptr.download(h.data(), L.n + 1);
      for (i64 i = 0; i <= L.n; ++i) rowptr[i] = h[i];
    }
    if (col && L.nnz > 0) {
      std::vector<int> h(L.nnz);
      L.col.download(h.data(), L.nnz);
      for (i64 i = 0; i < L.nnz; ++i) col[i] = h[i];
    }
    if (val && L.nnz > 0) L.val.download(val, L.nnz);
    return 0;
  }
  const CsrMatrix& Ah = sel == 0 ? s->A_ctor : run_matrix(s);
  const i64 n = s->nb.n_own;
  CsrMatrix raw;
  if (!precond && (rowptr || col || val))
    assemble_csr(make_params(s, sel == 0 ? s->scheme_ctor : s->scheme_run), s->slab, s->nb, raw, false);
  const CsrMatrix& A = precond ? Ah : raw;
  if (rowptr) {
    std::vector<int> h(n + 1);
    A.rowptr.download(h.data(), n + 1);
    for (i64 i = 0; i <= n; ++i) rowptr[i] = h[i];
  }
  if (col && A.nnz > 0) {
    std::vector<int> h(A.nnz);
    A.col.download(h.data(), A.nnz);
    for (i64 i = 0; i < A.nnz; ++i) col[i] = h[i];
  }
  if (val && A.nnz > 0) A.val.download(val, A.nnz);
  if (b && n > 0) {
    s->b.download(b, n);
    if (!precond) {
      std::vector<double> hb(b, b + n), hds(n);
      Ah.ds.download(hds.data(), n);
      for (i64 r = 0; r < n; ++r) b[r] = hb[r] / hds[r];
      if (Ah.n_blk > 0) {
        const i64 nq = Ah.n_blk;
        std::vector<int> rows(nq), bi(nq * MAX_KINDS);
        std::vector<double> fw(nq * MAX_KINDS);
        Ah.blk_rows.download(rows.data(), nq);
        Ah.blk_idx.download(bi.data(), nq * MAX_KINDS);
        Ah.blk_fw.download(fw.data(), nq * MAX_KINDS);
        for (i64 q = 0; q < nq; ++q) {
          double v = 0.0;
          for (int a = 0; a < MAX_KINDS; ++a)
            if (bi[q * MAX_KINDS + a] >= 0) v += fw[q * MAX_KINDS + a] * hb[bi[q * MAX_KINDS + a]];
          b[rows[q]] = v / hds[rows[q]];
        }
      }
    }
  }
  if (idx && n > 0) {
    std::vector<int> h(n);
    s->nb.row_cell.download(h.data(), n);
    for (i64 r = 0; r < n; ++r) {
      const int k = s->nb.kind_of_row(r);
      idx[r] = (i64)k * s->M + s->slab.first_cell() + h[r];
    }
  }
  PG_API_END
}

int32_t pg_solver_stefan_terms(const pg_solver* s, double* out) {
  PG_API_BEGIN
// ... 317 lines not shown
}

int32_t pg_debug_spmv_apply(pg_solver* s, int32_t which, int32_t variant, int32_t mode, const double* x, const double* aux,
                            const double* dotx, const double* base, double pc0, double pc1, double pc2, int32_t fold,
                            int32_t done, int32_t repeat, double* y, double* partials, double* slot_sums, double* folded,
                            int64_t* ticket) {
  PG_API_BEGIN
  require_init();
  PG_REQUIRE(s && x && y && slot_sums && folded && ticket, "pg_debug_spmv_apply: NULL argument");
  PG_REQUIRE(ctx().nranks == 1 && !ctx().comm, "pg_debug_spmv_apply: one rank (the split launch of a slab is not covered)");
  PG_REQUIRE(variant == 70 || variant == 38 || variant == 2 || variant == 1, "pg_debug_spmv_apply: variants 70, 38, 2 and 1");
  PG_REQUIRE(mode == 0 || mode == 1 || mode == 2 || mode == 3 || mode == 8, "pg_debug_spmv_apply: launch modes 0, 1, 2, 3 and 8");
  PG_REQUIRE(repeat == 1 || repeat == 2, "pg_debug_spmv_apply: repeat is 1 or 2");
  PG_REQUIRE(fold == 0 || fold == 1, "pg_debug_spmv_apply: fold is 0 or 1");
  const bool slices = (variant & 64) != 0;
  PG_REQUIRE(slices || (mode != 8 && !dotx && !fold),
             "pg_debug_spmv_apply: mode 8, a separate dot operand and the folded scalar phase exist in the slice kernel (variant 70) only");
  PG_REQUIRE(!fold || (mode >= 1 && mode <= 3), "pg_debug_spmv_apply: only the modes with dots (1, 2, 3) fold a scalar phase");
  PG_REQUIRE((mode == 1 || mode == 3) == (aux != nullptr), "pg_debug_spmv_apply: aux goes with modes 1 and 3, and only with them");
  PG_REQUIRE(!dotx || mode == 2 || mode == 3, "pg_debug_spmv_apply: dotx goes with modes 2 and 3");
  PG_REQUIRE(!base || mode == 8, "pg_debug_spmv_apply: base goes with mode 8");
  i64 nv = 0;
  const CsrMatrix& A = debug_matrix(s, which, &nv);
  const i64 n = A.n;
  PG_REQUIRE(n > 0, "pg_debug_spmv_apply: the matrix has no rows");
  PG_REQUIRE(!slices || A.srec.p, "pg_debug_spmv_apply: the matrix has no slice image");
  nv = std::max(nv, n);
  hipStream_t st = ctx().stream;
  const int grid = spmv_default_grid(n);
  constexpr i64 GUARD = 64;
  double sentinel;
  const unsigned long long sbits = PG_DEBUG_SPMV_SENTINEL;
  std::memcpy(&sentinel, &sbits, sizeof(double));
  DevBuf<double> dx(nv), daux(nv), ddot(nv), dbase(nv), dy(n + GUARD), dpart(5 * (i64)grid), dsc(S_COUNT);
  DevBuf<unsigned> dticket(1);
  daux.zero(); ddot.zero(); dbase.zero(); dsc.zero(); dticket.zero();
  dx.upload(x, nv);
  if (aux) daux.upload(aux, n);
  if (dotx) ddot.upload(dotx, n);
  if (base) dbase.upload(base, n);
  {
    std::vector<double> fill((size_t)std::max<i64>(n + GUARD, 5 * (i64)grid), sentinel);
    dy.upload(fill.data(), n + GUARD);
    if (fold && mode == 3) std::fill(fill.begin() + 2 * (size_t)grid, fill.begin() + 4 * (size_t)grid, 0.0);
    dpart.upload(fill.data(), 5 * (i64)grid);
    std::vector<double> hsc(S_COUNT, 0.0);
    for (int k = 0; k < 5; ++k) hsc[S_RED0 + k] = sentinel;
    hsc[S_DONE] = (double)done;
    dsc.upload(hsc.data(), S_COUNT);
  }
  FinArgs f{fold ? dticket.p : nullptr, fold ? dsc.p : nullptr, PH_NONE, fold ? (mode == 1 ? 1 : (mode == 2 ? 2 : 5)) : 0, 0,
            dotx ? ddot.p : nullptr};
  if (mode == 8) { f.pc0 = pc0; f.pc1 = pc1; f.pc2 = pc2; f.base = base ? dbase.p : dx.p; }
  const bool with_fin = mode == 8 || fold || dotx;
  for (int r = 0; r < repeat; ++r) {
    const bool folded_here = launch_spmv_as(variant, mode, A, dx.p, dy.p, aux ? daux.p : nullptr, mode >= 1 && mode <= 3 ? dpart.p : nullptr,
                                            dsc.p, grid, st, with_fin ? &f : nullptr);
    PG_REQUIRE(folded_here == (fold != 0), "pg_debug_spmv_apply: the launch did not report the scalar phase as asked");
  }
  PG_HIP(hipGetLastError());
  dy.download(y, n + GUARD);
  std::vector<double> hp(5 * (size_t)grid), hsc(S_COUNT);
  dpart.download(hp.data(), 5 * (i64)grid);
  dsc.download(hsc.data(), S_COUNT);
  if (partials) std::memcpy(partials, hp.data(), sizeof(double) * hp.size());
  for (int k = 0; k < 5; ++k) {
    double a = 0.0;
    for (int i = 0; i < grid; ++i) a += hp[(size_t)k * grid + i];
    slot_sums[k] = a;
    folded[k] = hsc[S_RED0 + k];
  }
  unsigned ht = 0;
  dticket.download(&ht, 1);
  *ticket = (int64_t)ht;
  PG_API_END
}

int32_t pg_debug_spmv_apply_typed(pg_solver* s, int32_t which, int32_t kind, const void* x, const void* base, double pc0, double pc1,
                                  double pc2, double sigma, int32_t done, double* y64, float* y32, float* p32) {
  PG_API_BEGIN
  require_init();
  PG_REQUIRE(s && x, "pg_debug_spmv_apply_typed: NULL argument");
  PG_REQUIRE(ctx().nranks == 1 && !ctx().comm, "pg_debug_spmv_apply_typed: one rank");
  PG_REQUIRE(kind == TYPED_FIRST || kind == TYPED_MIDDLE || kind == TYPED_HANDOVER, "pg_debug_spmv_apply_typed: kinds 1 (first), 2 (middle), 3 (hand-over)");
  PG_REQUIRE((kind == TYPED_FIRST) == (base == nullptr), "pg_debug_spmv_apply_typed: the first launch's base is its x; the others take one");
  PG_REQUIRE((kind == TYPED_FIRST) == (p32 != nullptr), "pg_debug_spmv_apply_typed: p32 is the first launch's output, and only its");
  PG_REQUIRE(kind == TYPED_HANDOVER ? (y64 && !y32) : (y32 && !y64), "pg_debug_spmv_apply_typed: y32 for kinds 1 and 2, y64 for kind 3");
  PG_REQUIRE(spmv_supports_typed_chain(), "pg_debug_spmv_apply_typed: the typed launches exist in the slice kernel with the stream hint only");
  i64 nv = 0;
  const CsrMatrix& A = debug_matrix(s, which, &nv);
  const i64 n = A.n;
  PG_REQUIRE(n > 0 && A.srec.p, "pg_debug_spmv_apply_typed: the matrix has no rows or no slice image");
  nv = std::max(nv, n);
  hipStream_t st = ctx().stream;
  const int grid = spmv_default_grid(n);
  constexpr i64 GUARD = 64;
  double sentinel;
  const unsigned long long sbits = PG_DEBUG_SPMV_SENTINEL;
  std::memcpy(&sentinel, &sbits, sizeof(double));
  float sentinel32;
  const unsigned sbits32 = PG_DEBUG_SPMV_SENTINEL_F32;
  std::memcpy(&sentinel32, &sbits32, sizeof(float));
  DevBuf<double> dx64(nv), db64(nv), dy64(n + GUARD), dsc(S_COUNT);
  DevBuf<float> dx32(nv), db32(nv), dy32(n + GUARD), dp32(n + GUARD);
  db64.zero(); db32.zero();
  if (kind == TYPED_FIRST) dx64.upload(static_cast<const double*>(x), nv);
  else dx32.upload(static_cast<const float*>(x), nv);
  if (kind == TYPED_MIDDLE) db32.upload(static_cast<const float*>(base), n);
  if (kind == TYPED_HANDOVER) db64.upload(static_cast<const double*>(base), n);
  {
    std::vector<double> f64((size_t)(n + GUARD), sentinel);
    std::vector<float> f32((size_t)(n + GUARD), sentinel32);
    dy64.upload(f64.data(), n + GUARD);
    dy32.upload(f32.data(), n + GUARD);
    dp32.upload(f32.data(), n + GUARD);
    std::vector<double> hsc(S_COUNT, 0.0);
    hsc[S_DONE] = (double)done;
    dsc.upload(hsc.data(), S_COUNT);
  }
  FinArgs f{nullptr, nullptr, PH_NONE, 0, 0, nullptr};
  f.pc0 = pc0; f.pc1 = pc1; f.pc2 = pc2;
  if (kind == TYPED_FIRST) {
    f.base = dx64.p; f.p32 = dp32.p; f.psig = sigma;
    launch_spmv_typed(kind, A, dx64.p, dy32.p, dsc.p, grid, st, f);
  } else if (kind == TYPED_MIDDLE) {
    f.base = reinterpret_cast<const double*>(db32.p);
    launch_spmv_typed(kind, A, dx32.p, dy32.p, dsc.p, grid, st, f);
  } else {
    f.base = db64.p;
    launch_spmv_typed(kind, A, dx32.p, dy64.p, dsc.p, grid, st, f);
  }
  PG_HIP(hipGetLastError());
  if (y64) dy64.download(y64, n + GUARD);
  if (y32) dy32.download(y32, n + GUARD);
  if (p32) dp32.download(p32, n + GUARD);
  PG_API_END
}

__global__ void k_scale_rows(i64 n_e, const int* __restrict__ elist, double factor, double* __restrict__ z) {
  for (i64 q = blockIdx.x * (i64)blockDim.x + threadIdx.x; q < n_e; q += (i64)gridDim.x * blockDim.x) z[elist[q]] *= factor;
}

int32_t pg_debug_scale_diagonal_rows(pg_solver* s, double factor) {
  PG_API_BEGIN
  require_init();
  PG_REQUIRE(s && s->have_run, "pg_debug_scale_diagonal_rows: no run matrix yet");
  const CsrMatrix& A = run_matrix(s);
  DiagElim& DE = (&A == &s->A_ctor) ? s->diag_ctor : s->diag_run;
  PG_REQUIRE(DE.active && DE.n_e > 0, "pg_debug_scale_diagonal_rows: the loop of this solver is not the compact one");
  hipLaunchKernelGGL(k_scale_rows, dim3(grid_for(DE.n_e, BLOCK)), dim3(BLOCK), 0, ctx().stream, DE.n_e, (const int*)DE.elist.p, factor,
                     s->z.p);
  PG_HIP(hipGetLastError());
  PG_HIP(hipStreamSynchronize(ctx().stream));
  s->x_valid = false;
  s->spec_y_valid = false;
  PG_API_END
}

int32_t pg_solver_guess_info(pg_solver* s, int32_t* kept, int32_t* nstates, int32_t* offsets, double* coef, double* rr_plain,
                             double* rr_taken) {
  PG_API_BEGIN
  require_init();
  PG_REQUIRE(s && kept && nstates && offsets && coef && rr_plain && rr_taken, "pg_solver_guess_info: NULL argument");
  *kept = s->hist_cnt;
  *nstates = 0;
  *rr_plain = *rr_taken = 0.0;
  for (int j = 0; j < 4; ++j) { offsets[j] = 0; coef[j] = 0.0; }
  if (s->guess_coef.n >= 16 && s->hist_cnt > 0) {
    double hc[16];
    s->guess_coef.download(hc, 16);
    *nstates = (int32_t)hc[4];
    for (int j = 0; j < *nstates && j < 4; ++j) { offsets[j] = (int32_t)hc[5 + j] + 1; coef[j] = hc[j]; }
    *rr_plain = hc[9];
    *rr_taken = hc[10];
  }
  PG_API_END
}

int32_t pg_solver_time_spmv(pg_solver* s, int32_t which, int32_t reps, double* avg_ms) {
  PG_API_BEGIN
  require_init();
  PG_REQUIRE(s && avg_ms && reps > 0, "pg_solver_time_spmv: bad arguments");
  const int sel = which & 1, mode = (which & 2048) ? 8 : ((which >> 4) & 7);
  PG_REQUIRE(mode <= 3 || mode == 8, "pg_solver_time_spmv: unknown launch mode");
  if (sel == 1) PG_REQUIRE(s->have_run, "run matrix not assembled yet");
  const CsrMatrix& Afull = sel == 0 ? s->A_ctor : run_matrix(s);
  GammaElim& E = (&Afull == &s->A_ctor) ? s->elim_ctor : s->elim_run;
  if ((which & 512) && !E.tried) build_gamma_elim(Afull, s->nb, E);
  DiagElim& DE = (&Afull == &s->A_ctor) ? s->diag_ctor : s->diag_run;
  if ((which & 4096) && !DE.tried) build_diag_elim(Afull, s->nb, s->slab, DE);
  const CsrMatrix& A = ((which & 4096) && DE.active) ? DE.A : (((which & 512) && E.active) ? E.A : Afull);
  const bool chained = (which & 1024) != 0;
  hipStream_t st = ctx().stream;
  EventPair ev;
  KrylovWork& w = s->work;
  const bool cold = (which & 256) != 0;
  constexpr int RING = 7;
  std::vector<DevBuf<double>> ring;
  const i64 nv = s->nb.n_vec();
  if (cold) {
    ring.resize(RING);
    for (auto& b : ring) {
      b.alloc(nv > 0 ? nv : 1);
      if (nv > 0) PG_HIP(hipMemcpyAsync(b.p, s->z.p, sizeof(double) * (size_t)nv, hipMemcpyDeviceToDevice, st));
    }
  }
  int it = 0;
  auto one = [&]() {
// ... 150 lines not shown
```

### penguin/jl_amd/csrc/pg_spmv.h

```cpp
#pragma once
#include "pg_system.h"

namespace pg {

enum { S_RHO = 0, S_RHO_OLD, S_ALPHA, S_OMEGA, S_BETA, S_RR, S_BB, S_TOL2, S_DONE, S_ITERS, S_RELTOL2, S_ABSTOL2,
       S_RESTART, S_RHAT2, S_FORCE, S_PENDING3, S_RRW, S_HALF, S_RR0 ,
       S_MOVED ,
       S_HELD ,
       S_RED0, S_RED1, S_RED2, S_RED3, S_RED4, S_COUNT };

constexpr int BLOCK = 256;

__device__ inline double wave_sum(double v) {
#pragma unroll
  for (int off = 32; off > 0; off >>= 1) v += __shfl_down(v, off, 64);
  return v;
}

__device__ inline double block_sum(double v, double* sh ) {
  v = wave_sum(v);
  const int lane = threadIdx.x & 63, wave = threadIdx.x >> 6;
  __syncthreads();
  if (lane == 0) sh[wave] = v;
  __syncthreads();
// ... 68 lines not shown
      if (sc[S_PENDING3] != 0.0) end_of_iteration(sc);
      break;
    case PH_BICG_S:
      if (sc[S_DONE] == 0.0 && sc[S_RED4] <= sc[S_TOL2]) {
        sc[S_RR] = sc[S_RED4];
        sc[S_ITERS] += 1.0;
        sc[S_PENDING3] = 0.0;
        sc[S_DONE] = 1.0;
        sc[S_HALF] = sc[S_ITERS];
      }
      break;
    case PH_CG_1:
      if (r0 == 0.0) sc[S_DONE] = 2.0; else sc[S_ALPHA] = sc[S_RR] / r0;
      break;
    case PH_CG_2: {
      const double rr_old = sc[S_RR];
      sc[S_RR] = r0;
      sc[S_RRW] = r1;
      sc[S_ITERS] += 1.0;
      if (r1 <= sc[S_TOL2]) sc[S_DONE] = 1.0;
      else sc[S_BETA] = r0 / rr_old;
      break;
    }
  }
}


__device__ inline void store_partial(double* p, double v) {
  __hip_atomic_store(reinterpret_cast<unsigned long long*>(p), (unsigned long long)__double_as_longlong(v), __ATOMIC_RELAXED,
                     __HIP_MEMORY_SCOPE_AGENT);
}
__device__ inline double load_partial(const double* p) {
  return __longlong_as_double((long long)__hip_atomic_load(reinterpret_cast<const unsigned long long*>(p), __ATOMIC_RELAXED,
                                                            __HIP_MEMORY_SCOPE_AGENT));
}

__device__ inline void put_partial(double* p, double v, int accum) { store_partial(p, accum ? v + load_partial(p) : v); }

__device__ inline bool last_block_arrives(unsigned* ticket, unsigned nblocks, double* sh ) {
  asm volatile("s_waitcnt vmcnt(0)" ::: "memory");
  __syncthreads();
  if (threadIdx.x == 0) {
    const unsigned t = __hip_atomic_fetch_add(ticket, 1u, __ATOMIC_RELAXED, __HIP_MEMORY_SCOPE_AGENT);
    const bool last = t == nblocks - 1;
    if (last) __hip_atomic_store(ticket, 0u, __ATOMIC_RELAXED, __HIP_MEMORY_SCOPE_AGENT);
    sh[0] = last ? 1.0 : 0.0;
  }
  __syncthreads();
  const bool last = sh[0] != 0.0;
  __syncthreads();
  return last;
}

struct FinArgs {
  unsigned* ticket;
  double* sc;
  int phase;
  int nslots;
  int do_derive;
  const double* dotx;
  double pc0 = 0.0, pc1 = 0.0;
  const double* base = nullptr;
  double pc2 = 0.0;
  float* p32 = nullptr;
  double psig = 0.0;
};

__device__ inline void fold_scalar_phase(const FinArgs& fin, const double* __restrict__ partials, double* s_red, int nparts) {
  if (!fin.ticket) return;
  if (!last_block_arrives(fin.ticket, gridDim.x, s_red)) return;
  for (int sl = 0; sl < fin.nslots; ++sl) {
    double a = 0.0;
    for (int i = threadIdx.x; i < nparts; i += BLOCK) a += load_partial(partials + (size_t)sl * nparts + i);
    const double t = block_sum(a, s_red);
    if (threadIdx.x == 0) fin.sc[S_RED0 + sl] = t;
  }
  if (threadIdx.x == 0 && fin.do_derive) derive(fin.phase, fin.sc);
}

bool launch_spmv(int mode, const CsrMatrix& A, const double* x, double* y, const double* aux, double* partials,
                 const double* sc, int grid, hipStream_t st, const FinArgs* fin = nullptr);
bool launch_spmv_as(int variant, int mode, const CsrMatrix& A, const double* x, double* y, const double* aux, double* partials,
                    const double* sc, int grid, hipStream_t st, const FinArgs* fin = nullptr);
enum { TYPED_FIRST = 1, TYPED_MIDDLE = 2, TYPED_HANDOVER = 3 };
void launch_spmv_typed(int kind, const CsrMatrix& A, const void* x, void* y, const double* sc, int grid, hipStream_t st,
                       const FinArgs& fin);
bool spmv_supports_typed_chain();
bool spmv_with_halo(int mode, const CsrMatrix& A, const Numbering& nb, const Slab& slab, double* x, double* y, const double* aux,
                    double* partials, const double* sc, int grid, hipStream_t st, const FinArgs* fin = nullptr);
void launch_spmv_variant(int variant, const CsrMatrix& A, const double* x, double* y, hipStream_t st);
void spmv_mode_compare(const CsrMatrix& A, i64 nv, int mode, double* max_abs_diff, double* max_abs, double* max_dot_rel);
int spmv_default_grid(i64 n);
bool spmv_supports_preconditioner_product();

}
```

### penguin/jl_amd/csrc/pg_spmv.hip

```cpp
#include <algorithm>
#include <cstdlib>
#include <thread>
#include <type_traits>
#include <vector>

#include "pg_host_algos.h"
#include "pg_krylov.h"
#include "pg_spmv.h"

namespace pg {
namespace {

constexpr int SPMV_ROWS = 256;
constexpr int SPMV_LDS_ENTRIES = 3584;

template <int MODE>
__global__ __launch_bounds__(BLOCK) void k_spmv(i64 n, const int* __restrict__ rowptr, const int* __restrict__ col,
                                                const double* __restrict__ val, const double* __restrict__ x,
                                                double* __restrict__ y, const double* __restrict__ aux,
                                                double* __restrict__ partials, const double* __restrict__ sc) {
  __shared__ double s_val[SPMV_LDS_ENTRIES];
  __shared__ int s_col[SPMV_LDS_ENTRIES];
  __shared__ double s_red[BLOCK / 64];
  if (sc && sc[S_DONE] != 0.0) return;
// ... 123 lines not shown
  if (first < nchunks) {
    dcur = load_desc(chunk_desc, first);
    dnext = load_desc(chunk_desc, first + wstride < nchunks ? first + wstride : lastc);
  }
  for (i64 chunk = first; chunk < nchunks; chunk += wstride) {
    stream_issue_w<NT>(q, dcur, rowptr, col, val, lane);
    const int r = dcur.r0 + lane;
    const bool live = r < dcur.r1;
    const int basev = dcur.base & ~1, basec = dcur.base & ~3;
    const int av = q.ra - basev, ac = q.ra - basec, len = q.rb - q.ra;
#pragma unroll
    for (int j = 0; j < XV_IT; ++j) sv2[lane + 64 * j] = q.v[j];
#pragma unroll
    for (int j = 0; j < XC_IT; ++j) sc4[lane + 64 * j] = q.c[j];
    __builtin_amdgcn_wave_barrier();
    double xv[WUNR], vv[WUNR];
    const int c0 = dcur.base - basec;
#pragma unroll
    for (int j = 0; j < WUNR; ++j) {
      const bool ok = j < len;
      xv[j] = x[scl[ok ? ac + j : c0]];
      vv[j] = ok ? sv[av + j] : 0.0;
    }
    const i64 c2 = chunk + 2 * wstride;
    const Desc dnext2 = load_desc(chunk_desc, c2 < nchunks ? c2 : lastc);
    double sum = 0.0;
#pragma unroll
    for (int j = 0; j < WUNR; ++j) sum += vv[j] * xv[j];
    if (__builtin_expect(len > WUNR, 0))
      for (int k = WUNR; k < len; ++k) sum += sv[av + k] * x[scl[ac + k]];
    __builtin_amdgcn_wave_barrier();
    if (live) {
      y[r] = sum;
      if (MODE == 1) acc0 += aux[r] * sum;
      if (MODE >= 2) {
        acc0 += sum * x[r];
        acc1 += sum * sum;
      }
      if (MODE == 3) acc2 += aux[r] * sum;
    }
    dcur = dnext;
    dnext = dnext2;
  }
  if (MODE >= 1) {
    const double t0 = block_sum(acc0, s_red);
    if (threadIdx.x == 0) partials[blockIdx.x] = t0;
  }
  if (MODE >= 2) {
    const double t1 = block_sum(acc1, s_red);
    if (threadIdx.x == 0) partials[gridDim.x + blockIdx.x] = t1;
  }
  if (MODE == 3) {
    const double t2 = block_sum(acc2, s_red);
    if (threadIdx.x == 0) partials[4 * (size_t)gridDim.x + blockIdx.x] = t2;
  }
}

enum { SL_U = 0, SL_P = 1, SL_G = 2 };
constexpr int SL_MAXROWS_U = 254, SL_MAXROWS_P = 128, SL_MAXCNT = 8, SL_REC = 32;

struct SDesc {
  int r0, meta, base, aux;
};

__device__ inline int rlane(int v, int l) { return __builtin_amdgcn_readlane(v, l); }

typedef double d2u_t __attribute__((ext_vector_type(2), aligned(8)));

template <bool NT>
__device__ inline d2_t load_pair(const double* p) {
  const d2u_t* q = reinterpret_cast<const d2u_t*>(p);
  d2u_t v = NT ? __builtin_nontemporal_load(q) : *q;
  d2_t r;
  r.x = v.x; r.y = v.y;
  return r;
}

template <class TX_, class TB_, class TY_, bool P32_>
struct VecTypes {
  using TX = TX_;
  using TB = TB_;
  using TY = TY_;
  static constexpr bool P32 = P32_;
};
using VecF64 = VecTypes<double, double, double, false>;

typedef float f2u_t __attribute__((ext_vector_type(2), aligned(4)));

template <bool NT>
__device__ inline d2_t load_pair_t(const double* p) { return load_pair<NT>(p); }
template <bool NT>
__device__ inline d2_t load_pair_t(const float* p) {
  const f2u_t* q = reinterpret_cast<const f2u_t*>(p);
  f2u_t v = NT ? __builtin_nontemporal_load(q) : *q;
  d2_t r;
  r.x = (double)v.x; r.y = (double)v.y;
  return r;
}
typedef float f2_t __attribute__((ext_vector_type(2)));
template <class T> struct PairOf { typedef d2_t type; };
template <> struct PairOf<float> { typedef f2_t type; };
template <bool NT>
__device__ inline d2_t load_raw(const double* p) { return load_pair<NT>(p); }
template <bool NT>
__device__ inline f2_t load_raw(const float* p) {
  const f2u_t* q = reinterpret_cast<const f2u_t*>(p);
  f2u_t v = NT ? __builtin_nontemporal_load(q) : *q;
  f2_t r;
  r.x = v.x; r.y = v.y;
  return r;
}
__device__ inline d2_t widen(const d2_t& v) { return v; }
__device__ inline d2_t widen(const f2_t& v) {
  d2_t r;
  r.x = (double)v.x; r.y = (double)v.y;
  return r;
}
__device__ inline void store_pair_t(double* p, double a, double b, bool plain) {
  d2u_t out;
  out.x = a; out.y = b;
  if (!plain) __builtin_nontemporal_store(out, reinterpret_cast<d2u_t*>(p));
  else *reinterpret_cast<d2u_t*>(p) = out;
}
__device__ inline float narrow(double a) {
  const float f = (float)a;
  return __builtin_fminf(__builtin_fmaxf(f, -3.402823466e+38f), 3.402823466e+38f);
}
__device__ inline void store_pair_t(float* p, double a, double b, bool plain) {
  f2u_t out;
  out.x = narrow(a); out.y = narrow(b);
  if (!plain) __builtin_nontemporal_store(out, reinterpret_cast<f2u_t*>(p));
  else *reinterpret_cast<f2u_t*>(p) = out;
}
__device__ inline void store_one_t(double* p, double a) { *p = a; }
__device__ inline void store_one_t(float* p, double a) { *p = narrow(a); }

template <int MODE>
struct ModeInfo {
  static constexpr bool OWN = MODE == 8;
  static constexpr bool HAS_A = MODE == 1 || MODE == 2 || MODE == 3;
  static constexpr bool HAS_B = MODE == 3 || MODE == 8;
  static constexpr bool DOT0 = MODE == 1 || MODE == 2 || MODE == 3;
  static constexpr bool DOT1 = MODE == 2 || MODE == 3;
  static constexpr bool DOT2 = MODE == 3;
};

template <int MODE>
__device__ __forceinline__ double mode_out(double s, double own, double b, double pc0, double pc1, double pc2) {
  if (MODE == 8) return __builtin_fma(pc2, b, __builtin_fma(pc0, own, pc1 * s));
  return s;
}

template <int CNT, int NB, bool PSL, int MODE, bool NT, class VT>
__device__ __forceinline__ void slice_rows(const SDesc& d, int nrows, int rec, const double* __restrict__ pval,
                                  const typename VT::TX* __restrict__ x, typename VT::TY* __restrict__ y, const double* __restrict__ pa,
                                  const typename VT::TB* __restrict__ pb, int lane, double& acc0, double& acc1, double& acc2, int dbg,
                                  double pc0, double pc1, double pc2, float* __restrict__ p32, double psig) {
  using MI = ModeInfo<MODE>;
  int o[CNT];
#pragma unroll
  for (int j = 0; j < CNT; ++j) o[j] = (dbg & 4) ? 0 : rlane(rec, 4 + j);
  int l0[NB];
  bool live0[NB], live1[NB];
  typename PairOf<typename VT::TX>::type xv[NB][CNT];
#pragma unroll
  for (int b = 0; b < NB; ++b) {
    const int l = 128 * b + 2 * lane;
    live0[b] = l < nrows;
// ... 193 lines not shown
  return xc_nx;
}

template <int CNT, int MODE, bool EDGE, class VT, int KK, int Q0 = 0, int KTOT = KK>
__device__ __forceinline__ void march_unit(int rec, int lane, const typename VT::TX* __restrict__ x, typename VT::TY* __restrict__ y,
                                  const double* __restrict__ pa, const typename VT::TB* __restrict__ pb, double pc0, double pc1,
                                  double pc2, double& acc0, double& acc1, double& acc2, int dbg,
                                  const double* __restrict__ e_val, double* sv, double* sx, float* __restrict__ p32, double psig) {
  using MI = ModeInfo<MODE>;
  constexpr bool Y = CNT == 7;
  const int amask = (dbg & 128) ? ~1 : ~0;
  const int one = (dbg & 128) ? 0 : 1;
  const bool nolat = (dbg & 64) != 0;
  double c[CNT];
#pragma unroll
  for (int j = 0; j < CNT; ++j) c[j] = __hiloint2double(rlane(rec, 3 + 2 * j), rlane(rec, 2 + 2 * j));
  const int l2 = 2 * lane;
  int rb[KK];
  typedef typename PairOf<typename VT::TX>::type xpair_t;
  typedef typename PairOf<typename VT::TB>::type bpair_t;
  xpair_t ln[KK + 2];
  MarchSide<typename VT::TX, typename VT::TB> sd[KK];
  const bool act = lane < (rlane(rec, 0) >> 16);
  d2_t zero;
  zero.x = zero.y = 0.0;
  xpair_t xzero;
  xzero.x = xzero.y = 0;
  bpair_t bzero;
  bzero.x = bzero.y = 0;
#pragma unroll
  for (int q = 0; q < KK + 2; ++q) ln[q] = xzero;
#pragma unroll
  for (int q = 0; q < KK; ++q) {
    rb[q] = rlane(rec, 18 + 4 * (Q0 + q)) & amask;
    sd[q].ym = sd[q].yp = xzero;
    sd[q].ax = zero;
    sd[q].ax2 = bzero;
  }
  if (act) {
    ln[0] = load_raw<false>(x + (rlane(rec, Q0 == 0 ? 16 : 18 + 4 * (Q0 - 1)) & amask) + l2);
#pragma unroll
    for (int q = 0; q < KK; ++q) ln[q + 1] = load_raw<false>(x + rb[q] + l2);
    ln[KK + 1] = load_raw<false>(x + (rlane(rec, Q0 + KK == KTOT ? 17 : 18 + 4 * (Q0 + KK)) & amask) + l2);
#pragma unroll
    for (int q = 0; q < KK; ++q) {
      if (Y && !nolat) {
        sd[q].ym = load_raw<false>(x + rb[q] + (rlane(rec, 19 + 4 * (Q0 + q)) & amask) + l2 + one);
        sd[q].yp = load_raw<false>(x + rb[q] + (rlane(rec, 20 + 4 * (Q0 + q)) & amask) + l2 + one);
      }
      if (MI::HAS_A) sd[q].ax = load_pair<false>(pa + rb[q] + l2 + one);
      if (MI::HAS_B && !VT::P32) sd[q].ax2 = load_raw<false>(pb + rb[q] + l2 + one);
    }
  }
  const int e_first = rlane(rec, MARCH_EDGE + 2 + Q0) >> 16;
  const int e_cnt = (Q0 + KK == KTOT ? rlane(rec, MARCH_EDGE + 1) : rlane(rec, MARCH_EDGE + 2 + Q0 + KK) >> 16) - e_first;
  int elane = lane;
  if (EDGE) asm volatile("" : "+v"(elane));
  if (EDGE && e_cnt > 0) {
    const int e_all = rlane(rec, MARCH_EDGE + 1);
    const double* ep = e_val + (i64)MARCH_ESLOTS * rlane(rec, MARCH_EDGE) + 2 * (e_first + elane);
    asm volatile("s_waitcnt lgkmcnt(0)" ::: "memory");
    if (elane < e_cnt) {
#pragma unroll
      for (int jp = 0; jp < (CNT + 1) / 2; ++jp)
        __builtin_amdgcn_global_load_lds((const __attribute__((address_space(1))) void*)(ep + 2 * jp * e_all),
                                         (__attribute__((address_space(3))) void*)(sv + 128 * jp), 16, 0, 0);
    }
    asm volatile("s_waitcnt vmcnt(0)" ::: "memory");
  }
  if (EDGE) {
    const int k = elane - 2;
    if (k >= 0 && k < 2 * CNT) reinterpret_cast<int*>(sx)[256 * (k >> 2) + (k & 3)] = rec;
  }
  const d2_t* el = reinterpret_cast<const d2_t*>(sv);
  const d2_t* cl = reinterpret_cast<const d2_t*>(sx);
  double xm_n = lane_up((double)ln[0].x);
#pragma unroll
  for (int q = 0; q < KK; ++q)
    xm_n = march_plane<CNT, MODE, EDGE, VT>(c, rlane(rec, 21 + 4 * (Q0 + q)), l2, y + rb[q] + l2 + one, ln[q], xm_n, ln[q + 1], ln[q + 2], sd[q], pc0,
                                  pc1, pc2, acc0, acc1, acc2, dbg, rlane(rec, MARCH_EDGE + 2 + Q0 + q), e_first, el, cl,
                                  VT::P32 ? p32 + rb[q] + l2 + one : nullptr, psig);
}

template <int CNT, int MODE, bool EDGE, class VT>
__device__ __forceinline__ void march_dispatch(int rec, int lane, const typename VT::TX* __restrict__ x, typename VT::TY* __restrict__ y,
                                      const double* __restrict__ pa, const typename VT::TB* __restrict__ pb, double pc0, double pc1,
                                      double pc2, double& acc0, double& acc1, double& acc2, int dbg,
                                      const double* __restrict__ e_val, double* sv, double* sx, float* __restrict__ p32, double psig) {
  constexpr bool SPLIT = MODE == 3 && MARCH_K == 2 * MARCH_KS && PG_MARCH_SPLIT;
  if ((rlane(rec, 0) & 255) == MARCH_K) {
    if (SPLIT) {
      march_unit<CNT, MODE, EDGE, VT, MARCH_KS, 0, MARCH_K>(rec, lane, x, y, pa, pb, pc0, pc1, pc2, acc0, acc1, acc2, dbg, e_val, sv, sx, p32, psig);
      march_unit<CNT, MODE, EDGE, VT, MARCH_KS, MARCH_KS, MARCH_K>(rec, lane, x, y, pa, pb, pc0, pc1, pc2, acc0, acc1, acc2, dbg, e_val, sv, sx, p32, psig);
    } else {
      march_unit<CNT, MODE, EDGE, VT, MARCH_K>(rec, lane, x, y, pa, pb, pc0, pc1, pc2, acc0, acc1, acc2, dbg, e_val, sv, sx, p32, psig);
    }
  } else {
    march_unit<CNT, MODE, EDGE, VT, MARCH_KS>(rec, lane, x, y, pa, pb, pc0, pc1, pc2, acc0, acc1, acc2, dbg, e_val, sv, sx, p32, psig);
  }
}

template <int MODE, bool NT, bool DIAG, class VT = VecF64>
__global__ __launch_bounds__(BLOCK, 4) void k_spmv_s(i64 nslices, const int* __restrict__ srec,
                                                  const double* __restrict__ pval, const int* __restrict__ g_rowid,
                                                  const int* __restrict__ g_rowptr, const int* __restrict__ g_col,
                                                  const double* __restrict__ g_val, const typename VT::TX* __restrict__ x,
                                                  typename VT::TY* __restrict__ y, const double* __restrict__ aux,
                                                  double* __restrict__ partials, const double* __restrict__ sc, int xcd,
                                                  FinArgs fin, int pstride, int accum, const int* __restrict__ mrec,
                                                  i64 nunits, const int* __restrict__ tiles, int tpx,
                                                  const double* __restrict__ e_val) {
  __shared__ __attribute__((aligned(16))) double s_val[BLOCK / 64][512];
  __shared__ __attribute__((aligned(16))) double s_x[BLOCK / 64][512];
  __shared__ double s_red[BLOCK / 64];
  if (sc && sc[S_DONE] != 0.0) return;
  using MI = ModeInfo<MODE>;
  constexpr bool DOTS = MI::DOT0;
  static_assert(MODE == 8 || std::is_same<VT, VecF64>::value, "element types per stream exist for mode 8 only");
  const double* __restrict__ dx = fin.dotx ? fin.dotx : reinterpret_cast<const double*>(x);
  const double* __restrict__ pa = MODE == 1 ? aux : ((MODE == 2 || MODE == 3) ? dx : nullptr);
  const typename VT::TB* __restrict__ pb = reinterpret_cast<const typename VT::TB*>(MODE == 3 ? aux : (MODE == 8 ? fin.base : nullptr));
  float* __restrict__ p32 = VT::P32 ? fin.p32 : nullptr;
  const double psig = fin.psig;
  const int lane = threadIdx.x & 63;
  const int wave = __builtin_amdgcn_readfirstlane(threadIdx.x >> 6);
  double* __restrict__ sv = s_val[wave];
  double* __restrict__ sx = s_x[wave];
  d2_t* sv2 = reinterpret_cast<d2_t*>(sv);
  d2_t* sx2 = reinterpret_cast<d2_t*>(sx);
  double acc0 = 0.0, acc1 = 0.0, acc2 = 0.0;
  const int dbg = DIAG ? (xcd >> 8) : 0;
  xcd &= 255;
  xcd &= 1;
  const bool xsplit = xcd && gridDim.x >= 8;
  const int xid = xsplit ? (blockIdx.x & 7) : 0;
  const int woff = xsplit ? (int)(blockIdx.x >> 3) * (BLOCK / 64) + wave : (int)blockIdx.x * (BLOCK / 64) + wave;
  const int wstr = xsplit ? (int)(((i64)gridDim.x + 7 - xid) >> 3) * (BLOCK / 64) : (int)gridDim.x * (BLOCK / 64);
  const int* __restrict__ tb = tiles ? tiles + 2 * (tpx + 1) * xid : nullptr;
  const int ntile = tiles ? tpx : 1;
  const int l31 = lane & 31;
  for (int tile = 0; tile < ntile; ++tile) {
  i64 ulo, uhi, slo, shi, ubase, sbase;
  if (tiles) {
    ubase = tb[0]; sbase = tb[1];
    ulo = tb[2 * tile]; slo = tb[2 * tile + 1]; uhi = tb[2 * tile + 2]; shi = tb[2 * tile + 3];
  } else if (xsplit) {
    ubase = ulo = nunits * xid / 8; uhi = nunits * (xid + 1) / 8;
    sbase = slo = nslices * xid / 8; shi = nslices * (xid + 1) / 8;
  } else {
    ubase = ulo = 0; uhi = nunits;
    sbase = slo = 0; shi = nslices;
  }
  auto run_units = [&]() __attribute__((always_inline)) {
  if (nunits > 0) {
    int d = (woff - (int)(ulo - ubase)) % wstr;
    d = d < 0 ? d + wstr : d;
    i64 ucur = ulo + d;
    const i64 ustride = wstr;
    int urec = ucur < uhi ? mrec[(unsigned)(MARCH_REC * (int)ucur + lane)] : 0;
    for (; ucur < uhi; ucur += ustride) {
      const i64 un = ucur + ustride;
      const int urec_n = mrec[(unsigned)(MARCH_REC * (int)(un < uhi ? un : ucur) + lane)];
      if (!(dbg & 16)) {
        const bool edge = rlane(urec, MARCH_EDGE + 1) > 0;
        if (((rlane(urec, 0) >> 8) & 255) == 7) {
          if (edge) march_dispatch<7, MODE, true, VT>(urec, lane, x, y, pa, pb, fin.pc0, fin.pc1, fin.pc2, acc0, acc1, acc2, dbg, e_val, sv, sx, p32, psig);
          else march_dispatch<7, MODE, false, VT>(urec, lane, x, y, pa, pb, fin.pc0, fin.pc1, fin.pc2, acc0, acc1, acc2, dbg, e_val, sv, sx, p32, psig);
        } else {
          if (edge) march_dispatch<5, MODE, true, VT>(urec, lane, x, y, pa, pb, fin.pc0, fin.pc1, fin.pc2, acc0, acc1, acc2, dbg, e_val, sv, sx, p32, psig);
          else march_dispatch<5, MODE, false, VT>(urec, lane, x, y, pa, pb, fin.pc0, fin.pc1, fin.pc2, acc0, acc1, acc2, dbg, e_val, sv, sx, p32, psig);
        }
      }
      urec = urec_n;
// ... 164 lines not shown
  return config().spmv_variant;
}

int xcd_map() {
  return config().spmv_xcd;
}

}
void ensure_csr_chunks(const CsrMatrix& A);
namespace {

#define PG_LAUNCH_C_ARGS(KERNEL, X, Y, AUX, PART)                                                               \
  hipLaunchKernelGGL(HIP_KERNEL_NAME(KERNEL), dim3(grid), dim3(BLOCK), 0, st, A.n, A.nchunks, A.chunk_desc.p, \
                     A.rowptr.p, A.col.p, A.val.p, X, Y, AUX, PART, (const double*)nullptr)
#define PG_LAUNCH_C(KERNEL)                                                                                    \
  hipLaunchKernelGGL(HIP_KERNEL_NAME(KERNEL), dim3(grid), dim3(BLOCK), 0, st, A.n, A.nchunks, A.chunk_desc.p, \
                     A.rowptr.p, A.col.p, A.val.p, x, y, aux, partials, sc)

template <int MODE>
bool launch_slices(int v, const CsrMatrix& A, i64 s0, i64 ns, const double* x, double* y, const double* aux, double* partials,
                   const double* sc, int grid, int pstride, int accum, hipStream_t st, const FinArgs* fin, bool units = true) {
  FinArgs fa{nullptr, nullptr, PH_NONE, 0, 0, nullptr};
  if (fin && MODE >= 1) fa = *fin;
  const int* rec = A.srec.p + SL_REC * s0;
  const i64 nu = units ? A.nunits : 0;
  const bool tiled = units && A.tiles_per_xcd > 0 && s0 == 0 && ns == A.tile_ns && (xcd_map() & 1) && grid >= 8;
  const int* tiles = tiled ? (const int*)A.tiles.p : nullptr;
  const int tpx = tiled ? A.tiles_per_xcd : 0;
  if (xcd_map() >= 256)
    hipLaunchKernelGGL(HIP_KERNEL_NAME(k_spmv_s<MODE, true, true>), dim3(grid), dim3(BLOCK), 0, st, ns, rec, A.pval.p,
                       A.g_rowid.p, A.g_rowptr.p, A.g_col.p, A.g_val.p, x, y, aux, partials, sc, xcd_map(), fa, pstride, accum,
                       (const int*)A.mrec.p, nu, tiles, tpx, (const double*)A.e_val.p);
  else if (v & 4)
    hipLaunchKernelGGL(HIP_KERNEL_NAME(k_spmv_s<MODE, true, false>), dim3(grid), dim3(BLOCK), 0, st, ns, rec, A.pval.p,
                       A.g_rowid.p, A.g_rowptr.p, A.g_col.p, A.g_val.p, x, y, aux, partials, sc, xcd_map(), fa, pstride, accum,
                       (const int*)A.mrec.p, nu, tiles, tpx, (const double*)A.e_val.p);
  else
    hipLaunchKernelGGL(HIP_KERNEL_NAME(k_spmv_s<MODE, false, false>), dim3(grid), dim3(BLOCK), 0, st, ns, rec, A.pval.p,
                       A.g_rowid.p, A.g_rowptr.p, A.g_col.p, A.g_val.p, x, y, aux, partials, sc, xcd_map(), fa, pstride, accum,
                       (const int*)A.mrec.p, nu, tiles, tpx, (const double*)A.e_val.p);
  return fa.ticket != nullptr;
}

template <int MODE>
bool launch_mode(int v, const CsrMatrix& A, const double* x, double* y, const double* aux, double* partials,
                 const double* sc, int grid, hipStream_t st, const FinArgs* fin) {
  if (v & 64) return launch_slices<MODE>(v, A, 0, A.nslices, x, y, aux, partials, sc, grid, grid, 0, st, fin);
  PG_REQUIRE(MODE != 8 && !(fin && fin->dotx), "the preconditioner products and separate dot operands need the slice kernel");
  if (v != 1) ensure_csr_chunks(A);
  if (v == 1) {
    hipLaunchKernelGGL(HIP_KERNEL_NAME(k_spmv<MODE>), dim3(grid), dim3(BLOCK), 0, st, A.n, A.rowptr.p, A.col.p, A.val.p, x, y,
                       aux, partials, sc);
    return false;
  }
  if (v & 4) PG_LAUNCH_C((k_spmv_cw<MODE, true>));
  else PG_LAUNCH_C((k_spmv_cw<MODE, false>));
  return false;
}

template <class VT>
void launch_typed(const CsrMatrix& A, const void* x, void* y, const double* sc, int grid, hipStream_t st, const FinArgs& fin) {
  const bool tiled = A.tiles_per_xcd > 0 && A.nslices == A.tile_ns && (xcd_map() & 1) && grid >= 8;
  hipLaunchKernelGGL(HIP_KERNEL_NAME(k_spmv_s<8, true, false, VT>), dim3(grid), dim3(BLOCK), 0, st, A.nslices, (const int*)A.srec.p,
                     (const double*)A.pval.p, (const int*)A.g_rowid.p, (const int*)A.g_rowptr.p, (const int*)A.g_col.p,
                     (const double*)A.g_val.p, static_cast<const typename VT::TX*>(x), static_cast<typename VT::TY*>(y),
                     (const double*)nullptr, (double*)nullptr, sc, xcd_map(), fin, grid, 0, (const int*)A.mrec.p, A.nunits,
                     tiled ? (const int*)A.tiles.p : (const int*)nullptr, tiled ? A.tiles_per_xcd : 0, (const double*)A.e_val.p);
}

}

bool spmv_supports_typed_chain() { return (variant() & 64) != 0 && (variant() & 4) != 0 && xcd_map() < 256; }

void launch_spmv_typed(int kind, const CsrMatrix& A, const void* x, void* y, const double* sc, int grid, hipStream_t st,
                       const FinArgs& fin) {
  if (A.n == 0) return;
  PG_REQUIRE(spmv_supports_typed_chain() && A.srec.p, "typed Horner launches need the slice kernel with the stream hint (PG_SPMV_VARIANT 70)");
  PG_REQUIRE(!fin.ticket && fin.base, "typed Horner launch: a base operand and no scalar phase");
  if (kind == TYPED_FIRST) {
    PG_REQUIRE(fin.p32 && x == (const void*)fin.base, "typed Horner launch (first): x = base and a p32 output");
    launch_typed<VecTypes<double, double, float, true>>(A, x, y, sc, grid, st, fin);
  } else if (kind == TYPED_MIDDLE) {
    launch_typed<VecTypes<float, float, float, false>>(A, x, y, sc, grid, st, fin);
  } else {
    PG_REQUIRE(kind == TYPED_HANDOVER, "unknown typed Horner launch");
    launch_typed<VecTypes<float, double, double, false>>(A, x, y, sc, grid, st, fin);
  }
}


namespace {

struct Slice {
  int r0, meta, base, aux;
  int key;
  int bnd;
  i64 okey = 0;
};

using pghost::MRun;

constexpr int RUN_INFO = 25;

__global__ void k_run_info(i64 nruns, const int* __restrict__ run_r0, const int* __restrict__ rowptr,
                           const int* __restrict__ col, const double* __restrict__ val, const int* __restrict__ cell,
                           const int* __restrict__ map, int* __restrict__ out) {
  for (i64 q = blockIdx.x * (i64)blockDim.x + threadIdx.x; q < nruns; q += (i64)gridDim.x * blockDim.x) {
    const int r = run_r0[q], a = rowptr[r], len = rowptr[r + 1] - a;
    out[RUN_INFO * q + 24] = cell ? cell[map ? map[r] : r] : -1;
    for (int k = 0; k < 8; ++k) {
      out[RUN_INFO * q + k] = k < len ? col[a + k] - r : 0;
      const double v = k < len ? val[a + k] : 0.0;
      out[RUN_INFO * q + 8 + 2 * k] = __double2loint(v);
      out[RUN_INFO * q + 9 + 2 * k] = __double2hiint(v);
    }
  }
}

__global__ void k_fill_units(i64 nunits, int* __restrict__ mrec, const int* __restrict__ rowptr,
                             const double* __restrict__ val) {
  for (i64 q = blockIdx.x * (i64)blockDim.x + threadIdx.x; q < nunits; q += (i64)gridDim.x * blockDim.x) {
    int* rec = mrec + MARCH_REC * q;
    const int cnt = (rec[0] >> 8) & 255, a = rowptr[rec[1]];
    for (int k = 0; k < cnt; ++k) {
      rec[2 + 2 * k] = __double2loint(val[a + k]);
      rec[3 + 2 * k] = __double2hiint(val[a + k]);
    }
  }
}

__global__ void k_fill_edges(i64 ne, const int* __restrict__ meta, const int* __restrict__ rowptr, const double* __restrict__ val,
                             double* __restrict__ e_val) {
  for (i64 q = blockIdx.x * (i64)blockDim.x + threadIdx.x; q < ne; q += (i64)gridDim.x * blockDim.x) {
    const int r = meta[4 * q], dst = meta[4 * q + 1], dist = meta[4 * q + 2], sm = meta[4 * q + 3];
    const int a = rowptr[r], len = sm >> 24;
    for (int j = 0; j < MARCH_ESLOTS; ++j) e_val[dst + (i64)(j >> 1) * dist + (j & 1)] = 0.0;
    for (int k = 0; k < len; ++k) {
      const int j = (sm >> (3 * k)) & 7;
      e_val[dst + (i64)(j >> 1) * dist + (j & 1)] = val[a + k];
    }
  }
}

__global__ void k_edges_invalid(i64 ne, const int* __restrict__ meta, const int* __restrict__ rowptr_t, const int* __restrict__ col_t,
                                const int* __restrict__ rowptr, const int* __restrict__ col, unsigned long long* __restrict__ out) {
  unsigned long long c = 0;
  for (i64 q = blockIdx.x * (i64)blockDim.x + threadIdx.x; q < ne; q += (i64)gridDim.x * blockDim.x) {
    const int r = meta[4 * q], a = rowptr[r], at = rowptr_t[r], len = rowptr[r + 1] - a;
    bool same = len == rowptr_t[r + 1] - at && len == (meta[4 * q + 3] >> 24);
    for (int k = 0; same && k < len; ++k) same = col[a + k] == col_t[at + k];
    c += same ? 0 : 1;
  }
  if (c) atomicAdd(out, c);
}

__global__ void k_units_invalid(i64 nunits, const int* __restrict__ mrec, const int* __restrict__ rowptr,
                                const double* __restrict__ val, const unsigned char* __restrict__ flags,
                                unsigned long long* __restrict__ out) {
  unsigned long long c = 0;
  for (i64 q = blockIdx.x; q < nunits; q += gridDim.x) {
    const int* rec = mrec + MARCH_REC * q;
    const int K = rec[0] & 255, cnt = (rec[0] >> 8) & 255, a0 = rowptr[rec[1]];
    for (int i = 0; i < K; ++i) {
      const int rb = rec[18 + 4 * i], lo = rec[21 + 4 * i] & 255, hi = rec[21 + 4 * i] >> 8;
      for (int l = lo + threadIdx.x; l < hi; l += blockDim.x) {
        const int r = rb + l;
        if (l > lo) {
          c += (flags[r] & 3) != 3 ? 1 : 0;
        } else {
          const int a = rowptr[r];
          bool same = rowptr[r + 1] - a == cnt;
          for (int k = 0; same && k < cnt; ++k)
            same = __double_as_longlong(val[a + k]) == __double_as_longlong(val[a0 + k]);
          c += same ? 0 : 1;
        }
      }
    }
  }
  if (c) atomicAdd(out, c);
}

__global__ void k_row_cells(i64 nrows, const int* __restrict__ rows, const int* __restrict__ cell, const int* __restrict__ map,
                            int* __restrict__ out) {
  for (i64 q = blockIdx.x * (i64)blockDim.x + threadIdx.x; q < nrows; q += (i64)gridDim.x * blockDim.x) {
    const int r = rows[q];
    out[q] = cell[map ? map[r] : r];
  }
}

int march_strip() {
  return config().spmv_strip;
}
bool has_geo(const CsrMatrix& A) { return A.geo_cell && A.geo_ext0 > 0 && A.geo_lines > 0 && march_strip() > 0; }

std::vector<i64> row_orders(const CsrMatrix& A, const std::vector<int>& rows) {
  std::vector<i64> ord(rows.size(), 0);
  if (!has_geo(A) || rows.empty()) return ord;
  const i64 nr = (i64)rows.size();
  DevBuf<int> d_rows(nr), d_cells(nr);
  d_rows.upload(rows.data(), nr);
  hipLaunchKernelGGL(k_row_cells, dim3(grid_for(nr, 256)), dim3(256), 0, ctx().stream, nr, d_rows.p, A.geo_cell, A.geo_map, d_cells.p);
  PG_HIP(hipGetLastError());
  std::vector<int> cells(rows.size());
  d_cells.download(cells.data(), nr);
  for (i64 q = 0; q < nr; ++q) ord[q] = pghost::march_order(cells[q], A.geo_ext0, A.geo_lines, march_strip());
  return ord;
}

void emit_u_rows(std::vector<Slice>& up, i64 a, i64 b, int cnt) {
  for (i64 r = a; r < b; r += SL_MAXROWS_U) {
    const int rows = (int)std::min<i64>(SL_MAXROWS_U, b - r);
    up.push_back(Slice{(int)r, rows | (SL_U << 8) | (cnt << 16), 0, 0, (int)r, 0});
  }
}

void build_march_units(CsrMatrix& A, const std::vector<MRun>& runs, std::vector<int>& mrec, std::vector<Slice>& up,
                       std::vector<i64>& ukeys, pghost::EdgePlan* edges) {
  A.rows_m = 0;
  const i64 nr = (i64)runs.size();
  if (nr == 0) return;
  hipStream_t st = ctx().stream;
  std::vector<int> info((size_t)RUN_INFO * nr);
  {
    std::vector<int> r0s(nr);
    for (i64 i = 0; i < nr; ++i) r0s[i] = runs[i].r0;
    DevBuf<int> d_r0(nr), d_info(RUN_INFO * nr);
    d_r0.upload(r0s.data(), nr);
    hipLaunchKernelGGL(k_run_info, dim3(grid_for(nr, 256)), dim3(256), 0, st, nr, d_r0.p, A.rowptr.p, A.col.p, A.val.p,
                       A.geo_cell, A.geo_map, d_info.p);
    PG_HIP(hipGetLastError());
    d_info.download(info.data(), RUN_INFO * nr);
  }
  const int kmax = config().spmv_march_k > 0 ? std::max(1, std::min(MARCH_K, config().spmv_march_k)) : MARCH_K;
  pghost::MarchGeometry geo{MARCH_K, MARCH_KS, MARCH_REC, MARCH_W, RUN_INFO, kmax, A.geo_ext0, A.geo_lines, march_strip(),
                            has_geo(A) ? config().unit_order : 0};
  std::vector<pghost::RowRange> fallback;
  i64 rows_m = 0;
  pghost::plan_march_units(A.n, runs, info, geo, mrec, fallback, rows_m, &ukeys, edges);
  A.rows_m = rows_m;
  for (const auto& f : fallback) emit_u_rows(up, f.a, f.b, f.cnt);
}

void build_slices(CsrMatrix& A, const int* rp) {
  hipStream_t st = ctx().stream;
  Laps laps;
  const i64 n = A.n;
  const int minrun = config().spmv_minrun;
  unsigned char* fl = static_cast<unsigned char*>(pinned_scratch(1, (size_t)n));
  A.rowflags.alloc(n);
  hipLaunchKernelGGL(k_row_same, dim3(grid_for(n, 256, 256 * 16)), dim3(256), 0, st, n, A.rowptr.p, A.col.p, A.val.p,
                     A.rowflags.p);
  PG_HIP(hipGetLastError());
  A.rowflags.download(fl, n);
  laps.lap("    slices: row flags");
  struct Part {
    std::vector<Slice> up;
    std::vector<int> grows;
    std::vector<MRun> runs;
    i64 rows_u = 0, rows_p = 0, nnz_p = 0;
  };
  const bool march_env = config().spmv_march;
  const bool march_on = march_env && A.want_units;
  auto classify = [&](i64 lo, i64 hi, Part& out) {
    auto emit = [&](int type, i64 a, i64 b, int cnt) {
      if (march_on && type == SL_U && (cnt == 5 || cnt == 7)) {
        bool ghost = false;
        for (i64 q = a; q < b; ++q) ghost = ghost || ((fl[q] >> 2) & 1);
        if (!ghost) {
          out.runs.push_back(MRun{(int)a, (int)(b - a), cnt});
          out.rows_u += b - a;
          return;
        }
      }
      const i64 maxrows = type == SL_U ? SL_MAXROWS_U : SL_MAXROWS_P;
      for (i64 r = a; r < b; r += maxrows) {
        const int rows = (int)std::min<i64>(maxrows, b - r);
        int bnd = 0;
        for (i64 q = r; q < r + rows; ++q) bnd |= (fl[q] >> 2) & 1;
        out.up.push_back(Slice{(int)r, rows | (type << 8) | (cnt << 16), 0, 0, (int)r, bnd});
      }
      (type == SL_U ? out.rows_u : out.rows_p) += b - a;
      if (type == SL_P) out.nnz_p += (b - a) * cnt;
    };
    auto irregular = [&](i64 a, i64 b) {
      for (i64 r = a; r < b; ++r) out.grows.push_back((int)r);
    };
    i64 i = lo;
    while (i < hi) {
      i64 j = i + 1;
      while (j < n && (fl[j] & 1)) ++j;
      const int cnt = rp[i + 1] - rp[i];
      if (j - i >= minrun && cnt >= 1 && cnt <= SL_MAXCNT) {
        i64 pstart = i, k = i;
        auto flush_p = [&](i64 a, i64 b) {
          if (b - a >= minrun) emit(SL_P, a, b, cnt);
          else irregular(a, b);
        };
        while (k < j) {
          i64 m = k + 1;
          while (m < j && (fl[m] & 2)) ++m;
          if (m - k >= minrun) {
            flush_p(pstart, k);
            emit(SL_U, k, m, cnt);
            pstart = m;
          }
          k = m;
        }
        flush_p(pstart, j);
      } else {
        irregular(i, j);
      }
      i = j;
    }
  };
  const int nthreads = n > (i64)1 << 20 ? (int)std::min<unsigned>(8u, std::max(1u, std::thread::hardware_concurrency())) : 1;
  std::vector<i64> cut(nthreads + 1, n);
  cut[0] = 0;
  for (int t = 1; t < nthreads; ++t) {
    i64 c = n * t / nthreads;
    while (c < n && (fl[c] & 1)) ++c;
    cut[t] = std::max(c, cut[t - 1]);
  }
// ... 142 lines not shown
  }
  std::stable_sort(all.begin(), all.end(), [](const Slice& a, const Slice& b) { return a.bnd != b.bnd ? a.bnd < b.bnd : a.okey < b.okey; });
  A.nslices = (i64)all.size();
  A.nslices_int = 0;
  while (A.nslices_int < A.nslices && !all[A.nslices_int].bnd) ++A.nslices_int;
  {
    const int tile_units = config().spmv_tile_units;
    const i64 T = tile_units > 0 ? std::min<i64>(256, (A.nunits / 8 + tile_units / 2) / tile_units) : 0;
    A.tiles_per_xcd = 0;
    A.tile_ns = 0;
    A.tiles.release();
    if (T >= 2 && A.nslices_int > 0 && (i64)ukeys.size() == A.nunits) {
      std::vector<i64> skeys((size_t)A.nslices_int);
      for (i64 q = 0; q < A.nslices_int; ++q) skeys[q] = all[q].okey;
      std::vector<int> tab;
      pghost::plan_tiles(ukeys, skeys, (int)T, tab);
      A.tiles.alloc((i64)tab.size());
      A.tiles.upload(tab.data(), (i64)tab.size());
      A.tiles_per_xcd = (int)T;
      A.tile_ns = A.nslices_int;
    }
  }
  std::vector<int> sd(SL_REC * (A.nslices + 1), 0);
  for (i64 q = 0; q < A.nslices; ++q) {
    int* rec = sd.data() + SL_REC * q;
    rec[0] = all[q].r0; rec[1] = all[q].meta; rec[2] = all[q].base; rec[3] = all[q].aux;
  }
  A.srec.alloc((i64)sd.size());
  A.srec.upload(sd.data(), (i64)sd.size());
  if (A.nslices > 0) {
    hipLaunchKernelGGL(k_fill_records, dim3(grid_for(A.nslices, 256)), dim3(256), 0, st, A.nslices, A.srec.p, A.rowptr.p, A.col.p,
                       A.val.p);
    PG_HIP(hipGetLastError());
  }
  if (A.nnz_p > 0) {
    hipLaunchKernelGGL(k_pval_fill, dim3((unsigned)std::min<i64>(A.nslices, 65535)), dim3(256), 0, st, A.nslices, A.srec.p,
                       A.rowptr.p, A.val.p, A.pval.p);
    PG_HIP(hipGetLastError());
  }
  PG_HIP(hipStreamSynchronize(st));
  laps.lap("    slices: packing + records");
  A.spmv_bytes = 4 * SL_REC * A.nslices + 4 * MARCH_REC * A.nunits + 8 * A.nnz_p + 12 * A.nnz_g + 8 * ng + 8 * A.e_slots + 16 * n;
  if (config().debug)
    fprintf(stderr, "[pg_spmv] slices %lld (%lld wait for the halo), marching units %lld (%lld rows, %lld edge rows): rows U %lld P %lld G %lld of %lld; nnz P %lld G %lld of %lld; bytes/launch %lld (CSR %lld)\n",
            (long long)A.nslices, (long long)(A.nslices - A.nslices_int), (long long)A.nunits, (long long)A.rows_m, (long long)A.rows_e, (long long)A.rows_u, (long long)A.rows_p, (long long)A.rows_g,
            (long long)n, (long long)A.nnz_p, (long long)A.nnz_g, (long long)A.nnz, (long long)A.spmv_bytes,
            (long long)(12 * A.nnz + 20 * n));
}

}

void ensure_csr_chunks(const CsrMatrix& Ac) {
  CsrMatrix& A = const_cast<CsrMatrix&>(Ac);
  if (A.chunk_desc.p || A.n == 0) return;
  std::vector<int> rp(A.n + 1);
  A.rowptr.download(rp.data(), A.n + 1);
  std::vector<int> cd;
  cd.reserve(2 * (A.n / 60 + 16));
  i64 r = 0;
  while (r < A.n) {
    i64 e = r + 1;
    PG_REQUIRE(rp[e] - rp[r] <= SPMV_CHUNK_ENTRIES, "CSR row longer than an SpMV chunk");
    while (e < A.n && e - r < 64 && rp[e + 1] - rp[r] <= SPMV_CHUNK_ENTRIES) ++e;
    cd.push_back((int)r);
    cd.push_back(rp[r]);
    r = e;
  }
  A.nchunks = (i64)cd.size() / 2;
  cd.push_back((int)A.n);
  cd.push_back(rp[A.n]);
  cd.push_back((int)A.n);
  cd.push_back(rp[A.n]);
  A.chunk_desc.alloc((i64)cd.size());
  A.chunk_desc.upload(cd.data(), (i64)cd.size());
}

void build_spmv_chunks(CsrMatrix& A) {
  Laps laps;
  int* rp = static_cast<int*>(pinned_scratch(0, sizeof(int) * (size_t)(A.n + 1)));
  A.rowptr.download(rp, A.n + 1);
  laps.lap("    chunks: rowptr download");
  A.chunk_desc.release();
  A.nchunks = 0;
  build_slices(A, rp);
}

__global__ void k_slices_invalid(i64 nslices, const int* __restrict__ srec, const unsigned char* __restrict__ flags,
                                 unsigned long long* __restrict__ out) {
  unsigned long long c = 0;
  for (i64 q = blockIdx.x; q < nslices; q += gridDim.x) {
    const int r0 = srec[SL_REC * q], meta = srec[SL_REC * q + 1];
    const int nrows = meta & 255, type = (meta >> 8) & 3;
    const unsigned char need = type == SL_U ? 3 : 1;
    for (int l = 1 + threadIdx.x; l < nrows; l += blockDim.x) c += (flags[r0 + l] & need) != need ? 1 : 0;
  }
  if (c) atomicAdd(out, c);
}

template <class T>
static void clone_buf(DevBuf<T>& dst, const DevBuf<T>& src, hipStream_t st) {
  dst.alloc(src.n > 0 ? src.n : 1);
  if (src.n > 0) PG_HIP(hipMemcpyAsync(dst.p, src.p, sizeof(T) * (size_t)src.n, hipMemcpyDeviceToDevice, st));
}

bool build_slices_like(const CsrMatrix& T, CsrMatrix& A) {
  hipStream_t st = ctx().stream;
  const i64 n = A.n;
  if (!T.rowflags.p || T.n != n || !T.srec.p) return false;
  A.rowflags.alloc(n);
  DevBuf<unsigned long long> diff(1);
  diff.zero();
  hipLaunchKernelGGL(k_row_same, dim3(grid_for(n, 256, 256 * 16)), dim3(256), 0, st, n, A.rowptr.p, A.col.p, A.val.p,
                     A.rowflags.p);
  if (T.nslices > 0)
    hipLaunchKernelGGL(k_slices_invalid, dim3((unsigned)std::min<i64>(T.nslices, 16384)), dim3(64), 0, st, T.nslices, T.srec.p,
                       A.rowflags.p, diff.p);
  if (T.nunits > 0)
    hipLaunchKernelGGL(k_units_invalid, dim3((unsigned)std::min<i64>(T.nunits, 16384)), dim3(64), 0, st, T.nunits, T.mrec.p,
                       A.rowptr.p, A.val.p, A.rowflags.p, diff.p);
  if (T.rows_e > 0)
    hipLaunchKernelGGL(k_edges_invalid, dim3(grid_for(T.rows_e, 256)), dim3(256), 0, st, T.rows_e, (const int*)T.e_meta.p,
                       (const int*)T.rowptr.p, (const int*)T.col.p, (const int*)A.rowptr.p, (const int*)A.col.p, diff.p);
  PG_HIP(hipGetLastError());
  unsigned long long h = 0;
  diff.download(&h, 1);
  if (h != 0) return false;
  A.chunk_desc.release();
  A.nchunks = 0;
  A.nslices = T.nslices;
  A.nslices_int = T.nslices_int;
  A.rows_u = T.rows_u; A.rows_p = T.rows_p; A.rows_g = T.rows_g; A.nnz_p = T.nnz_p; A.nnz_g = T.nnz_g;
  A.spmv_bytes = T.spmv_bytes;
  A.nunits = T.nunits; A.rows_m = T.rows_m;
  A.tiles_per_xcd = T.tiles_per_xcd; A.tile_ns = T.tile_ns;
  if (T.tiles_per_xcd > 0) clone_buf(A.tiles, T.tiles, st);
  else A.tiles.release();
  clone_buf(A.mrec, T.mrec, st);
  if (A.nunits > 0)
    hipLaunchKernelGGL(k_fill_units, dim3(grid_for(A.nunits, 256)), dim3(256), 0, st, A.nunits, A.mrec.p, A.rowptr.p, A.val.p);
  A.rows_e = T.rows_e; A.e_slots = T.e_slots;
  clone_buf(A.e_meta, T.e_meta, st);
  A.e_val.alloc((i64)MARCH_ESLOTS * A.rows_e + 8);
  A.e_val.zero();
  if (A.rows_e > 0)
    hipLaunchKernelGGL(k_fill_edges, dim3(grid_for(A.rows_e, 256)), dim3(256), 0, st, A.rows_e, (const int*)A.e_meta.p, A.rowptr.p,
                       A.val.p, A.e_val.p);
  clone_buf(A.srec, T.srec, st);
  clone_buf(A.g_rowid, T.g_rowid, st);
  clone_buf(A.g_rowptr, T.g_rowptr, st);
  A.pval.alloc(A.nnz_p + 8);
  A.g_col.alloc(A.nnz_g + 8);
  A.g_val.alloc(A.nnz_g + 8);
  A.g_col.zero();
  A.g_val.zero();
  if (A.nslices > 0)
    hipLaunchKernelGGL(k_fill_records, dim3(grid_for(A.nslices, 256)), dim3(256), 0, st, A.nslices, A.srec.p, A.rowptr.p, A.col.p,
                       A.val.p);
  if (A.nnz_p > 0)
    hipLaunchKernelGGL(k_pval_fill, dim3((unsigned)std::min<i64>(A.nslices, 65535)), dim3(256), 0, st, A.nslices, A.srec.p,
                       A.rowptr.p, A.val.p, A.pval.p);
  if (A.rows_g > 0)
    hipLaunchKernelGGL(k_gpack, dim3(grid_for(A.rows_g, 256)), dim3(256), 0, st, A.rows_g, A.g_rowid.p, A.g_rowptr.p, A.rowptr.p,
                       A.col.p, A.val.p, A.g_col.p, A.g_val.p);
  PG_HIP(hipGetLastError());
  PG_HIP(hipStreamSynchronize(st));
  return true;
}

bool spmv_supports_preconditioner_product() { return (variant() & 64) != 0; }

int spmv_default_grid(i64 n) {
  const int per_cu = config().spmv_blocks_per_cu > 0 ? config().spmv_blocks_per_cu : ((variant() & 64) ? 4 : 6);
  static int cus = 0;
  if (cus == 0) {
    hipDeviceProp_t prop;
    cus = 256;
    if (hipGetDeviceProperties(&prop, ctx().device) == hipSuccess && prop.multiProcessorCount > 0) cus = prop.multiProcessorCount;
  }
  return grid_for(n, BLOCK, cus * per_cu);
}

static inline __attribute__((always_inline)) bool launch_by_mode(int v, int mode, const CsrMatrix& A, const double* x, double* y,
                                                                 const double* aux, double* partials, const double* sc, int grid,
                                                                 hipStream_t st, const FinArgs* fin) {
  if (mode == 0) return launch_mode<0>(v, A, x, y, aux, partials, sc, grid, st, fin);
  if (mode == 1) return launch_mode<1>(v, A, x, y, aux, partials, sc, grid, st, fin);
  if (mode == 2) return launch_mode<2>(v, A, x, y, aux, partials, sc, grid, st, fin);
  if (mode == 8) return launch_mode<8>(v, A, x, y, aux, partials, sc, grid, st, fin);
  PG_REQUIRE(mode == 3, "unknown SpMV launch mode");
  return launch_mode<3>(v, A, x, y, aux, partials, sc, grid, st, fin);
}

bool launch_spmv(int mode, const CsrMatrix& A, const double* x, double* y, const double* aux, double* partials,
                 const double* sc, int grid, hipStream_t st, const FinArgs* fin) {
  if (A.n == 0) return false;
  return launch_by_mode(variant(), mode, A, x, y, aux, partials, sc, grid, st, fin);
}

bool launch_spmv_as(int v, int mode, const CsrMatrix& A, const double* x, double* y, const double* aux, double* partials,
                    const double* sc, int grid, hipStream_t st, const FinArgs* fin) {
  if (A.n == 0) return false;
  return launch_by_mode(v, mode, A, x, y, aux, partials, sc, grid, st, fin);
}

bool spmv_with_halo(int mode, const CsrMatrix& A, const Numbering& nb, const Slab& slab, double* x, double* y, const double* aux,
                    double* partials, const double* sc, int grid, hipStream_t st, const FinArgs* fin) {
  if (A.n == 0 || !A.halo_needed) {
    if (A.halo_needed) halo_exchange(nb, slab, x, st);
    return launch_spmv(mode, A, x, y, aux, partials, sc, grid, st, fin);
  }
  const int v = variant();
  const bool overlap = config().halo_overlap;
  const i64 ni = A.nslices_int, nbnd = A.nslices - A.nslices_int;
  if (!(v & 64) || !overlap || (ni == 0 && A.nunits == 0) || nbnd == 0) {
    halo_exchange(nb, slab, x, st);
    return launch_spmv(mode, A, x, y, aux, partials, sc, grid, st, fin);
  }
  const int grid2 = (int)std::max<i64>(1, std::min<i64>(grid, (nbnd + BLOCK / 64 - 1) / (BLOCK / 64)));
  halo_begin(nb, slab, x, st);
  bool folded;
  FinArgs fin_nofold{nullptr, nullptr, PH_NONE, 0, 0, fin ? fin->dotx : nullptr};
  if (fin) { fin_nofold.pc0 = fin->pc0; fin_nofold.pc1 = fin->pc1; fin_nofold.pc2 = fin->pc2; fin_nofold.base = fin->base; }
#define PG_SPLIT(MODE_)                                                                                              \
  launch_slices<MODE_>(v, A, 0, ni, x, y, aux, partials, sc, grid, grid, 0, st, fin ? &fin_nofold : nullptr);      \
  halo_end(st);                                                                                                      \
  folded = launch_slices<MODE_>(v, A, ni, nbnd, x, y, aux, partials, sc, grid2, grid, 1, st, fin, false)
  if (mode == 0) { PG_SPLIT(0); }
  else if (mode == 1) { PG_SPLIT(1); }
  else if (mode == 2) { PG_SPLIT(2); }
  else if (mode == 8) { PG_SPLIT(8); }
  else { PG_REQUIRE(mode == 3, "unknown SpMV launch mode"); PG_SPLIT(3); }
#undef PG_SPLIT
  return folded;
}

namespace {

__global__ void k_hash_vector(i64 n, unsigned long long seed, double* x) {
  for (i64 i = blockIdx.x * (i64)blockDim.x + threadIdx.x; i < n; i += (i64)gridDim.x * blockDim.x) {
    unsigned long long h = ((unsigned long long)i + seed) * 0x9E3779B97F4A7C15ull + 0x632BE59BD9B4E019ull;
    h ^= h >> 29; h *= 0xBF58476D1CE4E5B9ull; h ^= h >> 32;
    x[i] = (double)(h >> 11) * (1.0 / 9007199254740992.0) - 0.5;
  }
}

template <int MODE>
__global__ void k_mode_epilogue(i64 n, double* __restrict__ y, const double* __restrict__ x, const double* __restrict__ b, double pc0,
                                double pc1, double pc2) {
  for (i64 i = blockIdx.x * (i64)blockDim.x + threadIdx.x; i < n; i += (i64)gridDim.x * blockDim.x)
// ... 65 lines not shown
```

### penguin/jl_amd/csrc/pg_system.h

```cpp
#pragma once
#include <vector>

#include "pg_stencil.h"

namespace pg {

struct SpecEst {
  bool tried = false;
  bool admitted = false;
  int steps = 0;
  double g_ritz = 0.0, g_used = 0.0;
  double re_min = 0.0, re_max = 0.0, im_max = 0.0;
  double ms = 0.0;
  std::vector<double> H;
};

struct Numbering {
  int K = 2;
  i64 Mloc = 0;
  i64 n_own = 0, n_ghost = 0;
  i64 cnt_own[MAX_KINDS] = {0, 0, 0, 0}, off_own[MAX_KINDS] = {0, 0, 0, 0};
  i64 cntL[MAX_KINDS] = {0, 0, 0, 0}, offL[MAX_KINDS] = {0, 0, 0, 0};
  i64 cntU[MAX_KINDS] = {0, 0, 0, 0}, offU[MAX_KINDS] = {0, 0, 0, 0};
  i64 sendL_off[MAX_KINDS] = {0, 0, 0, 0}, sendL_cnt[MAX_KINDS] = {0, 0, 0, 0};
  i64 sendU_off[MAX_KINDS] = {0, 0, 0, 0}, sendU_cnt[MAX_KINDS] = {0, 0, 0, 0};
  DevBuf<int> red;
  DevBuf<int> row_cell;
  i64 n_vec() const { return n_own + n_ghost; }
  int kind_of_row(i64 r) const {
    int k = 0;
    while (k + 1 < K && r >= off_own[k + 1]) ++k;
    return k;
  }
};

struct CsrMatrix {
  i64 n = 0, nnz = 0;
  int scheme = -1;
  DevBuf<int> rowptr, col;
  DevBuf<double> val;
  DevBuf<double> ds;
  DevBuf<int> chunk_desc;
  i64 nchunks = 0;
  DevBuf<int> srec;
  DevBuf<double> pval;
  DevBuf<int> g_rowid, g_rowptr, g_col;
  DevBuf<double> g_val;
  DevBuf<int> mrec;
  i64 nunits = 0, rows_m = 0;
  DevBuf<int> e_meta;
  DevBuf<double> e_val;
  i64 rows_e = 0, e_slots = 0;
  DevBuf<int> tiles;
  int tiles_per_xcd = 0;
  i64 tile_ns = 0;
  const int* geo_cell = nullptr;
  const int* geo_map = nullptr;
  i64 geo_ext0 = 0, geo_lines = 0;
  bool want_units = true;
  i64 nslices = 0;
  i64 nslices_int = 0;
  DevBuf<unsigned char> rowflags;
  i64 rows_u = 0, rows_p = 0, rows_g = 0, nnz_p = 0, nnz_g = 0;
  i64 spmv_bytes = 0;
  bool halo_needed = true;
  bool poly_ok = false;
  double gersh = 0.0;
  SpecEst est;
  bool poly_gave_up = false;
  i64 n_blk = 0;
  i64 nnz_raw = 0;
  DevBuf<int> blk_rows, blk_idx;
  DevBuf<double> blk_coef, blk_cn, blk_fw;
  DevBuf<unsigned char> isblk;
};
constexpr int SPMV_CHUNK_ENTRIES = 508;
void build_spmv_chunks(CsrMatrix& A);

void build_numbering(const SysParams& P, const Slab& slab, Numbering& nb);
void assemble_csr(const SysParams& P, const Slab& slab, const Numbering& nb, CsrMatrix& A, bool scale = true);
void assemble_csr_preconditioned(const SysParams& P, const Slab& slab, const Numbering& nb, CsrMatrix& A,
                                 const bool* inherit_halo = nullptr);
void assemble_csr_like(const SysParams& P, const Slab& slab, const Numbering& nb, const CsrMatrix& T, CsrMatrix& A);
bool build_slices_like(const CsrMatrix& T, CsrMatrix& A);
void decide_poly(CsrMatrix& A);
void apply_left(const CsrMatrix& A, const double* in, double* out, hipStream_t st);
void apply_rows_padded(const SysParams& P, const Slab& slab, const double* x, double* y);

}
```

Before: 1343.

## Add wide 4-rows-per-lane march units for f32 middle Horner SpMV steps

Builds a second 'wide' unit image of the matrix in which each lane of a march unit covers four consecutive rows, with a window of 63×4 rows, and loads x, y-neighbours and base as float4 quads. The middle f32 Horner launches of the mixed-precision polynomial chain use this image by default. The aim is wider loads and fewer units and records per row, cutting instruction and metadata overhead in the bandwidth-bound f32 SpMV. In exchange it costs a second unit plan and edge data per matrix, extra setup time, more memory, and higher register pressure per lane.

Result: no change. 1357, median of 6 (+1.0%).

```diff
diff --git a/include/penguin_hip.h b/include/penguin_hip.h
--- a/include/penguin_hip.h
+++ b/include/penguin_hip.h
@@ -121,6 +121,7 @@
   int64_t poly_f32_timed;
   int64_t poly_f32_chains;
   int64_t poly_f32_tail_sum;
+  int64_t poly_f32_wide_launches;
 } pg_run_info;
 
 typedef struct {
@@ -143,6 +144,10 @@
   int64_t n_ghost_loop;
   int64_t loop_is_compact;
   int64_t rows_edge;
+  int64_t wide_units;
+  int64_t wide_rows_marched;
+  int64_t wide_rows_edge;
+  int64_t wide_plane_rows_max;
 } pg_system_info;
 
 typedef struct {
diff --git a/penguin/jl_amd/_lib.py b/penguin/jl_amd/_lib.py
--- a/penguin/jl_amd/_lib.py
+++ b/penguin/jl_amd/_lib.py
@@ -77,7 +77,8 @@
                 ("spmv_lean_launches", C.c_int64), ("poly_degree", C.c_int64), ("half_exits", C.c_int64),
                 ("poly_xspace", C.c_int64), ("products", C.c_int64), ("guess_states_read", C.c_int64),
                 ("poly_f32_launches", C.c_int64), ("poly_f32_ms_total", C.c_double), ("poly_f32_timed", C.c_int64),
-                ("poly_f32_chains", C.c_int64), ("poly_f32_tail_sum", C.c_int64)]
+                ("poly_f32_chains", C.c_int64), ("poly_f32_tail_sum", C.c_int64),
+                ("poly_f32_wide_launches", C.c_int64)]
 
 
 class pg_system_info(C.Structure):
@@ -86,7 +87,8 @@
                 ("rows_uniform", C.c_int64), ("rows_pattern", C.c_int64), ("rows_irregular", C.c_int64),
                 ("neumann_ok", C.c_int64), ("gershgorin", C.c_double), ("spmv_units", C.c_int64),
                 ("rows_marched", C.c_int64), ("rows_matrix", C.c_int64), ("n_ghost_loop", C.c_int64),
-                ("loop_is_compact", C.c_int64), ("rows_edge", C.c_int64)]
+                ("loop_is_compact", C.c_int64), ("rows_edge", C.c_int64), ("wide_units", C.c_int64),
+                ("wide_rows_marched", C.c_int64), ("wide_rows_edge", C.c_int64), ("wide_plane_rows_max", C.c_int64)]
 
 
 class pg_streamvort_run_info(C.Structure):
@@ -346,13 +348,13 @@
 
 
 DEBUG_SPMV_SENTINEL_F32 = 0x7FC5EED0
-TYPED_FIRST, TYPED_MIDDLE, TYPED_HANDOVER = 1, 2, 3
+TYPED_FIRST, TYPED_MIDDLE, TYPED_HANDOVER, TYPED_MIDDLE_WIDE = 1, 2, 3, 4
 
 
 def debug_spmv_apply_typed(handle, which: int, kind: int, x, base=None, pc=(0.0, 0.0, 0.0), sigma: float = 1.0, done: int = 0) -> dict:
     n, nv, _, _ = debug_spmv_sizes(handle, which)
     want_x = np.float64 if kind == TYPED_FIRST else np.float32
-    want_b = {TYPED_FIRST: None, TYPED_MIDDLE: np.float32, TYPED_HANDOVER: np.float64}[kind]
+    want_b = {TYPED_FIRST: None, TYPED_MIDDLE: np.float32, TYPED_HANDOVER: np.float64, TYPED_MIDDLE_WIDE: np.float32}[kind]
     x = np.ascontiguousarray(x)
     if x.dtype != want_x or x.size != nv:
         raise ValueError(f"debug_spmv_apply_typed: x must be {nv} x {np.dtype(want_x).name}")
diff --git a/penguin/jl_amd/csrc/pg_common.h b/penguin/jl_amd/csrc/pg_common.h
--- a/penguin/jl_amd/csrc/pg_common.h
+++ b/penguin/jl_amd/csrc/pg_common.h
@@ -73,6 +73,7 @@
   int poly_maxdeg = 0;
   int poly_mindeg = 4;
   bool poly_f32 = true;
+  bool poly_f32_wide = true;
   int poly_f32_tail = -1;
   int profile_sample = 3;
   bool gamma_elim = true;
diff --git a/penguin/jl_amd/csrc/pg_context.hip b/penguin/jl_amd/csrc/pg_context.hip
--- a/penguin/jl_amd/csrc/pg_context.hip
+++ b/penguin/jl_amd/csrc/pg_context.hip
@@ -46,6 +46,7 @@
     k.poly_mindeg = (int)std::max<long long>(2, std::min<long long>(8, geti("PG_POLY_MINDEG", 4)));
     k.poly_trend = geti("PG_POLY_TREND", 1) != 0;
     k.poly_f32 = geti("PG_POLY_F32", 1) != 0;
+    k.poly_f32_wide = geti("PG_POLY_F32_WIDE", 1) != 0;
     k.poly_f32_tail = (int)std::max<long long>(-1, std::min<long long>(64, geti("PG_POLY_F32_TAIL", -1)));
     k.profile_sample = (int)std::max<long long>(1, geti("PG_PROFILE_SAMPLE", 3));
     k.gamma_elim = geti("PG_GAMMA_ELIM", 1) != 0;
@@ -369,11 +370,11 @@
            "spmv_variant=%d spmv_xcd=%d spmv_strip=%d spmv_unit_order=%d spmv_march=%d spmv_edges=%d spmv_march_k=%d spmv_minrun=%d spmv_tile_units=%d "
            "spmv_blocks_per_cu=%d halo_overlap=%d speculate=%d poly=%d poly_degree=%d poly_adapt=%d "
            "poly_margin=%g poly_slack=%g poly_hist=%d poly_trend=%d poly_maxdeg=%d poly_f32=%d poly_f32_tail=%d gamma_elim=%d diag_elim=%d "
-           "guess_states=%d guess_depth=%d guess_defer=%d async_alloc=%d cache_limit_mb=%lld alloc_poison=%d alloc_guard=%d profile_sample=%d debug=%d",
+           "guess_states=%d guess_depth=%d guess_defer=%d async_alloc=%d cache_limit_mb=%lld alloc_poison=%d alloc_guard=%d profile_sample=%d debug=%d poly_f32_wide=%d",
            k.spmv_variant, k.spmv_xcd, k.spmv_strip, k.unit_order, (int)k.spmv_march, (int)k.spmv_edges, k.spmv_march_k, k.spmv_minrun, k.spmv_tile_units,
            k.spmv_blocks_per_cu, (int)k.halo_overlap, (int)k.speculate_product, (int)k.poly, k.poly_degree, (int)k.poly_adapt,
            k.poly_margin, k.poly_slack, k.poly_hist, (int)k.poly_trend, k.poly_maxdeg, (int)k.poly_f32, k.poly_f32_tail,
-           (int)k.gamma_elim, (int)k.diag_elim, k.guess_n, k.guess_depth, (int)k.guess_defer, k.async_alloc, k.pool_limit_mb, k.alloc_poison, k.alloc_guard, k.profile_sample, (int)k.debug);
+           (int)k.gamma_elim, (int)k.diag_elim, k.guess_n, k.guess_depth, (int)k.guess_defer, k.async_alloc, k.pool_limit_mb, k.alloc_poison, k.alloc_guard, k.profile_sample, (int)k.debug, (int)k.poly_f32_wide);
   if (buf && n > 0) {
     std::strncpy(buf, tmp, n - 1);
     buf[n - 1] = 0;
diff --git a/penguin/jl_amd/csrc/pg_host_algos.h b/penguin/jl_amd/csrc/pg_host_algos.h
--- a/penguin/jl_amd/csrc/pg_host_algos.h
+++ b/penguin/jl_amd/csrc/pg_host_algos.h
@@ -2,6 +2,7 @@
 #include <algorithm>
 #include <cmath>
 #include <cstdint>
+#include <stdexcept>
 #include <vector>
 
 namespace pghost {
@@ -81,6 +82,8 @@
   int64_t ext0 = 0, lines = 0;
   int strip = 0;
   int unit_order = 0;
+  int R = 2;
+  int slack = 8;
 };
 
 struct EdgeCands {
@@ -180,7 +183,10 @@
     return cell >= 0 ? cell / (geo.ext0 * geo.lines) : -1;
   };
   std::vector<Unit> units;
-  auto safe = [&](i64 idx0) { return idx0 >= 0 && idx0 + 130 <= n + 8; };
+  if (!(geo.W == 63 * geo.R && geo.W + 1 <= 255 && geo.slack >= 0))
+    throw std::logic_error("plan_march_units: the window is 63 R rows and its ranges are packed into bytes");
+  const i64 reach = 64 * (i64)geo.R + 2;
+  auto safe = [&](i64 idx0) { return idx0 >= 0 && idx0 + reach <= n + geo.slack; };
   std::vector<i64> chain, B;
   for (i64 h = 0; h < nr; ++h) {
     if (!ok[h] || pred[h] >= 0) continue;
@@ -263,6 +269,7 @@
           u.rec[18 + 4 * i] = (int)(B[q] + W);
           u.rec[19 + 4 * i] = Y ? off(chain[q], 3) : 0;
           u.rec[20 + 4 * i] = Y ? off(chain[q], 2) : 0;
+          if (!(lo - W >= 1 && lo < hi && hi - W <= geo.W + 1)) throw std::logic_error("plan_march_units: range outside its window");
           u.rec[21 + 4 * i] = (int)(lo - W) | ((int)(hi - W) << 8);
           rows_m += hi - lo;
         }
@@ -294,7 +301,7 @@
           u.rec[EDGE_REC + 1] = (int)(u.erows.size() / 2);
           for (int i = K; i < Kp; ++i) u.rec[EDGE_REC + 2 + i] = u.rec[EDGE_REC + 1] << 16;
         }
-        u.rec[0] |= std::min(64, hi_max / 2 + 1) << 16;
+        u.rec[0] |= std::min(64, hi_max / geo.R + 1) << 16;
         for (int i = K; i < Kp; ++i) {
           u.rec[18 + 4 * i] = u.rec[17];
           u.rec[19 + 4 * i] = 0;
diff --git a/penguin/jl_amd/csrc/pg_krylov.h b/penguin/jl_amd/csrc/pg_krylov.h
--- a/penguin/jl_amd/csrc/pg_krylov.h
+++ b/penguin/jl_amd/csrc/pg_krylov.h
@@ -69,6 +69,7 @@
   i64 products = 0;
   int polls = 0;
   i64 f32_launches = 0, f32_timed = 0, f32_chains = 0, f32_tail_sum = 0;
+  i64 f32_wide_launches = 0;
   double f32_ms = 0.0;
 };
 
diff --git a/penguin/jl_amd/csrc/pg_krylov.hip b/penguin/jl_amd/csrc/pg_krylov.hip
--- a/penguin/jl_amd/csrc/pg_krylov.hip
+++ b/penguin/jl_amd/csrc/pg_krylov.hip
@@ -682,6 +682,7 @@
         w.fa.alloc(nvec); w.fb.alloc(nvec); w.p32.alloc(nvec);
         w.fa.zero(); w.fb.zero(); w.p32.zero();
       }
+      if (cfg.poly_f32_wide && mc.n32 > 1) ensure_wide_image(A);
     }
   }
   bool mixed_ran = false;
@@ -723,6 +724,7 @@
       if (mixed && itn == 0 && !second) {
         const int n32 = mc.n32, nf32 = n32 + 1, nf64 = m - 1 - nf32;
         const void* src32 = nullptr;
+        const bool wide_mid = cfg.poly_f32_wide && A.wide;
         timer.begin(st, itn, true, second, nf32, true);
         for (int i = 0; i <= n32; ++i) {
           const double tk = mtau[i + 1];
@@ -737,7 +739,8 @@
             float* dst = (i & 1) ? w.fb.p : w.fa.p;
             f.pc0 = 1.0; f.pc1 = -tk; f.pc2 = tk;
             f.base = reinterpret_cast<const double*>(w.p32.p);
-            launch_spmv_typed(TYPED_MIDDLE, A, src32, dst, w.sc.p, G, st, f);
+            launch_spmv_typed(wide_mid ? TYPED_MIDDLE_WIDE : TYPED_MIDDLE, A, src32, dst, w.sc.p, G, st, f);
+            if (wide_mid) stats.f32_wide_launches += 1;
             src32 = dst;
           } else {
             double* dst = i == m - 2 ? hat : ((i & 1) ? w.wb.p : w.wa.p);
@@ -899,7 +902,7 @@
   const bool mix_env = poly && cfg.poly_f32 && cx.nranks == 1 && !cx.comm && !A.halo_needed && spmv_supports_typed_chain();
   choose_next_degree(A, stats, m, adaptive, w,
                      mix_env && cfg.poly_f32_tail < 0 ? std::min(std::max(by_estimate ? A.est.g_used : A.gersh, 0.05), 0.95) : 0.0);
-  if (stats.iters == 0) stats.f32_launches = stats.f32_chains = stats.f32_tail_sum = 0;
+  if (stats.iters == 0) stats.f32_launches = stats.f32_chains = stats.f32_tail_sum = stats.f32_wide_launches = 0;
   if (mixed_ran && expect_halves == 1 && !(stats.iters == 1 && stats.half_exit)) w.mix_wait = 2 * (m + 3);
   w.mix_matrix = nullptr;
   if (mix_env && stats.converged) {
diff --git a/penguin/jl_amd/csrc/pg_solver.hip b/penguin/jl_amd/csrc/pg_solver.hip
--- a/penguin/jl_amd/csrc/pg_solver.hip
+++ b/penguin/jl_amd/csrc/pg_solver.hip
@@ -2799,7 +2799,7 @@
     tot.half_exit += st.half_exit;
     tot.products += st.products;
     tot.f32_launches += st.f32_launches; tot.f32_ms += st.f32_ms; tot.f32_timed += st.f32_timed;
-    tot.f32_chains += st.f32_chains; tot.f32_tail_sum += st.f32_tail_sum;
+    tot.f32_chains += st.f32_chains; tot.f32_tail_sum += st.f32_tail_sum; tot.f32_wide_launches += st.f32_wide_launches;
     if (!st.converged) ++unconverged;
     if (st.bnorm > 0.0) worst = std::max(worst, st.resnorm / st.bnorm);
   };
@@ -2858,6 +2858,7 @@
     info->poly_f32_timed = tot.f32_timed;
     info->poly_f32_chains = tot.f32_chains;
     info->poly_f32_tail_sum = tot.f32_tail_sum;
+    info->poly_f32_wide_launches = tot.f32_wide_launches;
     info->guess_states_read = 0;
     if (s->guess_coef.n >= 16) {
       double hc[16];
@@ -2928,6 +2929,10 @@
   out->rows_matrix = A.n;
   out->n_ghost_loop = ((which & 4) && DE.active) ? DE.nb.n_ghost : s->nb.n_ghost;
   out->loop_is_compact = DE.active ? 1 : 0;
+  out->wide_units = A.wide ? A.wide->nunits : 0;
+  out->wide_rows_marched = A.wide ? A.wide->rows_m : 0;
+  out->wide_rows_edge = A.wide ? A.wide->rows_e : 0;
+  out->wide_plane_rows_max = A.wide ? A.wide->plane_rows_max : 0;
   PG_API_END
 }
 
@@ -3411,7 +3416,8 @@
   require_init();
   PG_REQUIRE(s && x, "pg_debug_spmv_apply_typed: NULL argument");
   PG_REQUIRE(ctx().nranks == 1 && !ctx().comm, "pg_debug_spmv_apply_typed: one rank");
-  PG_REQUIRE(kind == TYPED_FIRST || kind == TYPED_MIDDLE || kind == TYPED_HANDOVER, "pg_debug_spmv_apply_typed: kinds 1 (first), 2 (middle), 3 (hand-over)");
+  PG_REQUIRE(kind == TYPED_FIRST || kind == TYPED_MIDDLE || kind == TYPED_HANDOVER || kind == TYPED_MIDDLE_WIDE,
+             "pg_debug_spmv_apply_typed: kinds 1 (first), 2 (middle), 3 (hand-over), 4 (middle on the wide image)");
   PG_REQUIRE((kind == TYPED_FIRST) == (base == nullptr), "pg_debug_spmv_apply_typed: the first launch's base is its x; the others take one");
   PG_REQUIRE((kind == TYPED_FIRST) == (p32 != nullptr), "pg_debug_spmv_apply_typed: p32 is the first launch's output, and only its");
   PG_REQUIRE(kind == TYPED_HANDOVER ? (y64 && !y32) : (y32 && !y64), "pg_debug_spmv_apply_typed: y32 for kinds 1 and 2, y64 for kind 3");
@@ -3435,7 +3441,8 @@
   db64.zero(); db32.zero();
   if (kind == TYPED_FIRST) dx64.upload(static_cast<const double*>(x), nv);
   else dx32.upload(static_cast<const float*>(x), nv);
-  if (kind == TYPED_MIDDLE) db32.upload(static_cast<const float*>(base), n);
+  if (kind == TYPED_MIDDLE || kind == TYPED_MIDDLE_WIDE) db32.upload(static_cast<const float*>(base), n);
+  if (kind == TYPED_MIDDLE_WIDE) ensure_wide_image(A);
   if (kind == TYPED_HANDOVER) db64.upload(static_cast<const double*>(base), n);
   {
     std::vector<double> f64((size_t)(n + GUARD), sentinel);
@@ -3452,7 +3459,7 @@
   if (kind == TYPED_FIRST) {
     f.base = dx64.p; f.p32 = dp32.p; f.psig = sigma;
     launch_spmv_typed(kind, A, dx64.p, dy32.p, dsc.p, grid, st, f);
-  } else if (kind == TYPED_MIDDLE) {
+  } else if (kind == TYPED_MIDDLE || kind == TYPED_MIDDLE_WIDE) {
     f.base = reinterpret_cast<const double*>(db32.p);
     launch_spmv_typed(kind, A, dx32.p, dy32.p, dsc.p, grid, st, f);
   } else {
diff --git a/penguin/jl_amd/csrc/pg_spmv.h b/penguin/jl_amd/csrc/pg_spmv.h
--- a/penguin/jl_amd/csrc/pg_spmv.h
+++ b/penguin/jl_amd/csrc/pg_spmv.h
@@ -174,7 +174,7 @@
                  const double* sc, int grid, hipStream_t st, const FinArgs* fin = nullptr);
 bool launch_spmv_as(int variant, int mode, const CsrMatrix& A, const double* x, double* y, const double* aux, double* partials,
                     const double* sc, int grid, hipStream_t st, const FinArgs* fin = nullptr);
-enum { TYPED_FIRST = 1, TYPED_MIDDLE = 2, TYPED_HANDOVER = 3 };
+enum { TYPED_FIRST = 1, TYPED_MIDDLE = 2, TYPED_HANDOVER = 3, TYPED_MIDDLE_WIDE = 4 };
 void launch_spmv_typed(int kind, const CsrMatrix& A, const void* x, void* y, const double* sc, int grid, hipStream_t st,
                        const FinArgs& fin);
 bool spmv_supports_typed_chain();
diff --git a/penguin/jl_amd/csrc/pg_spmv.hip b/penguin/jl_amd/csrc/pg_spmv.hip
--- a/penguin/jl_amd/csrc/pg_spmv.hip
+++ b/penguin/jl_amd/csrc/pg_spmv.hip
@@ -229,8 +229,12 @@
   using TB = TB_;
   using TY = TY_;
   static constexpr bool P32 = P32_;
+  static constexpr bool WIDE = false;
 };
 using VecF64 = VecTypes<double, double, double, false>;
+struct VecF32Wide : VecTypes<float, float, float, false> {
+  static constexpr bool WIDE = true;
+};
 
 typedef float f2u_t __attribute__((ext_vector_type(2), aligned(4)));
 
@@ -590,13 +594,163 @@
                                   VT::P32 ? p32 + rb[q] + l2 + one : nullptr, psig);
 }
 
+typedef float f4u_t __attribute__((ext_vector_type(4), aligned(4)));
+typedef float f4_t __attribute__((ext_vector_type(4)));
+constexpr int MARCH_R_WIDE = 4, MARCH_W_WIDE = 63 * MARCH_R_WIDE;
+#ifndef PG_MARCH_K_WIDE
+#define PG_MARCH_K_WIDE 2
+#endif
+constexpr int MARCH_K_WIDE = PG_MARCH_K_WIDE;
+static_assert(MARCH_K_WIDE >= MARCH_KS && MARCH_K_WIDE <= MARCH_K, "wide units use the narrow units' record");
+
+__device__ inline f4_t load_quad(const float* p) {
+  const f4u_t v = *reinterpret_cast<const f4u_t*>(p);
+  f4_t r;
+  r.x = v.x; r.y = v.y; r.z = v.z; r.w = v.w;
+  return r;
+}
+__device__ inline float lane_up_f(float v) { return __shfl_down(v, 1, 64); }
+
+template <int CNT, bool EDGE>
+__device__ __forceinline__ float march_plane_w(const double (&c)[CNT], int rng, int l4, float* __restrict__ yrow, const f4_t& xm,
+                                               float xm_n, const f4_t& xc, const f4_t& xp, const f4_t& ym, const f4_t& yp,
+                                               const f4_t& bs, double pc0, double pc1, double pc2, int einfo, int e_first,
+                                               const d2_t* el, const d2_t* cl) {
+  constexpr bool Y = CNT == 7;
+  const float xc_n0 = lane_up_f(xc.x), xc_n1 = lane_up_f(xc.y), xp_n0 = lane_up_f(xp.x);
+  const float ce[6] = {xc.x, xc.y, xc.z, xc.w, xc_n0, xc_n1};
+  const float pe[4] = {xp.y, xp.z, xp.w, xp_n0};
+  const float me[4] = {xm.y, xm.z, xm.w, xm_n};
+  const float ype[4] = {yp.x, yp.y, yp.z, yp.w};
+  const float yme[4] = {ym.x, ym.y, ym.z, ym.w};
+  const float be[4] = {bs.x, bs.y, bs.z, bs.w};
+  int lo = rng & 255, hi = rng >> 8;
+  int elo = lo, ehi = hi, e0 = 0;
+  if (EDGE) {
+    const int nlo = einfo & 255, nhi = (einfo >> 8) & 255;
+    e0 = (einfo >> 16) - e_first;
+    elo = lo - nlo;
+    ehi = hi + nhi;
+  }
+  double s[4];
+#pragma unroll
+  for (int i = 0; i < 4; ++i) {
+    double a[CNT];
+    int j = 0;
+    a[j++] = (double)ce[i + 2];
+    a[j++] = (double)ce[i];
+    if (Y) { a[j++] = (double)ype[i]; a[j++] = (double)yme[i]; }
+    a[j++] = (double)pe[i];
+    a[j++] = (double)me[i];
+    a[j] = (double)ce[i + 1];
+    double si = 0.0;
+    if (EDGE) {
+      asm volatile("" ::: "memory");
+      const int p = l4 + 1 + i;
+      const bool g = p >= elo && p < ehi && !(p >= lo && p < hi);
+      const d2_t* q = g ? el + (e0 + (p - elo) - (p >= hi ? hi - lo : 0)) : cl;
+#pragma unroll
+      for (int jp = 0; jp < (CNT + 1) / 2; ++jp) {
+        const d2_t w = q[64 * jp];
+        si += w.x * a[2 * jp];
+        if (2 * jp + 1 < CNT) si += w.y * a[2 * jp + 1];
+      }
+    } else {
+#pragma unroll
+      for (int k = 0; k < CNT; ++k) si += c[k] * a[k];
+    }
+    s[i] = mode_out<8>(si, a[CNT - 1], (double)be[i], pc0, pc1, pc2);
+  }
+  bool v[4];
+#pragma unroll
+  for (int i = 0; i < 4; ++i) v[i] = l4 + 1 + i >= elo && l4 + 1 + i < ehi;
+  if (v[0] && v[1] && v[2] && v[3]) {
+    f4u_t out;
+    out.x = narrow(s[0]); out.y = narrow(s[1]); out.z = narrow(s[2]); out.w = narrow(s[3]);
+    __builtin_nontemporal_store(out, reinterpret_cast<f4u_t*>(yrow));
+  } else {
+#pragma unroll
+    for (int i = 0; i < 4; ++i)
+      if (v[i]) store_one_t(yrow + i, s[i]);
+  }
+  return xc_n0;
+}
+
+template <int CNT, bool EDGE, int KK>
+__device__ __forceinline__ void march_unit_w(int rec, int lane, const float* __restrict__ x, float* __restrict__ y,
+                                             const float* __restrict__ pb, double pc0, double pc1, double pc2,
+                                             const double* __restrict__ e_val, double* sv, double* sx) {
+  constexpr bool Y = CNT == 7;
+  double c[CNT];
+#pragma unroll
+  for (int j = 0; j < CNT; ++j) c[j] = __hiloint2double(rlane(rec, 3 + 2 * j), rlane(rec, 2 + 2 * j));
+  int elane = lane;
+  asm volatile("" : "+v"(elane));
+  const unsigned l4 = 4u * (unsigned)elane;
+  int rb[KK];
+  f4_t ln[KK + 2], ym[KK], yp[KK], bs[KK];
+  const bool act = elane < (rlane(rec, 0) >> 16);
+  f4_t zero;
+  zero.x = zero.y = zero.z = zero.w = 0.0f;
+#pragma unroll
+  for (int q = 0; q < KK + 2; ++q) ln[q] = zero;
+#pragma unroll
+  for (int q = 0; q < KK; ++q) {
+    rb[q] = rlane(rec, 18 + 4 * q);
+    ym[q] = yp[q] = bs[q] = zero;
+  }
+  if (act) {
+    ln[0] = load_quad(x + rlane(rec, 16) + l4);
+#pragma unroll
+    for (int q = 0; q < KK; ++q) ln[q + 1] = load_quad(x + rb[q] + l4);
+    ln[KK + 1] = load_quad(x + rlane(rec, 17) + l4);
+#pragma unroll
+    for (int q = 0; q < KK; ++q) {
+      if (Y) {
+        ym[q] = load_quad(x + (rb[q] + rlane(rec, 19 + 4 * q) + 1) + l4);
+        yp[q] = load_quad(x + (rb[q] + rlane(rec, 20 + 4 * q) + 1) + l4);
+      }
+      bs[q] = load_quad(pb + (rb[q] + 1) + l4);
+    }
+  }
+  const int e_first = rlane(rec, MARCH_EDGE + 2) >> 16;
+  const int e_cnt = rlane(rec, MARCH_EDGE + 1) - e_first;
+  if (EDGE && e_cnt > 0) {
+    const int e_all = rlane(rec, MARCH_EDGE + 1);
+    const double* ep = e_val + (i64)MARCH_ESLOTS * rlane(rec, MARCH_EDGE) + 2 * (e_first + elane);
+    asm volatile("s_waitcnt lgkmcnt(0)" ::: "memory");
+    if (elane < e_cnt) {
+#pragma unroll
+      for (int jp = 0; jp < (CNT + 1) / 2; ++jp)
+        __builtin_amdgcn_global_load_lds((const __attribute__((address_space(1))) void*)(ep + 2 * jp * e_all),
+                                         (__attribute__((address_space(3))) void*)(sv + 128 * jp), 16, 0, 0);
+    }
+    asm volatile("s_waitcnt vmcnt(0)" ::: "memory");
+  }
+  if (EDGE) {
+    const int k = elane - 2;
+    if (k >= 0 && k < 2 * CNT) reinterpret_cast<int*>(sx)[256 * (k >> 2) + (k & 3)] = rec;
+  }
+  const d2_t* el = reinterpret_cast<const d2_t*>(sv);
+  const d2_t* cl = reinterpret_cast<const d2_t*>(sx);
+  float xm_n = lane_up_f(ln[0].x);
+#pragma unroll
+  for (int q = 0; q < KK; ++q)
+    xm_n = march_plane_w<CNT, EDGE>(c, rlane(rec, 21 + 4 * q), (int)l4, y + (rb[q] + 1) + l4, ln[q], xm_n, ln[q + 1], ln[q + 2], ym[q], yp[q],
+                                    bs[q], pc0, pc1, pc2, rlane(rec, MARCH_EDGE + 2 + q), e_first, el, cl);
+}
+
 template <int CNT, int MODE, bool EDGE, class VT>
 __device__ __forceinline__ void march_dispatch(int rec, int lane, const typename VT::TX* __restrict__ x, typename VT::TY* __restrict__ y,
                                       const double* __restrict__ pa, const typename VT::TB* __restrict__ pb, double pc0, double pc1,
                                       double pc2, double& acc0, double& acc1, double& acc2, int dbg,
                                       const double* __restrict__ e_val, double* sv, double* sx, float* __restrict__ p32, double psig) {
   constexpr bool SPLIT = MODE == 3 && MARCH_K == 2 * MARCH_KS && PG_MARCH_SPLIT;
-  if ((rlane(rec, 0) & 255) == MARCH_K) {
+  if constexpr (VT::WIDE) {
+    static_assert(MODE == 8, "wide units are Horner steps");
+    if (MARCH_K_WIDE > MARCH_KS && (rlane(rec, 0) & 255) == MARCH_K_WIDE) march_unit_w<CNT, EDGE, MARCH_K_WIDE>(rec, lane, x, y, pb, pc0, pc1, pc2, e_val, sv, sx);
+    else march_unit_w<CNT, EDGE, MARCH_KS>(rec, lane, x, y, pb, pc0, pc1, pc2, e_val, sv, sx);
+  } else if ((rlane(rec, 0) & 255) == MARCH_K) {
     if (SPLIT) {
       march_unit<CNT, MODE, EDGE, VT, MARCH_KS, 0, MARCH_K>(rec, lane, x, y, pa, pb, pc0, pc1, pc2, acc0, acc1, acc2, dbg, e_val, sv, sx, p32, psig);
       march_unit<CNT, MODE, EDGE, VT, MARCH_KS, MARCH_KS, MARCH_K>(rec, lane, x, y, pa, pb, pc0, pc1, pc2, acc0, acc1, acc2, dbg, e_val, sv, sx, p32, psig);
@@ -927,6 +1081,9 @@
     launch_typed<VecTypes<double, double, float, true>>(A, x, y, sc, grid, st, fin);
   } else if (kind == TYPED_MIDDLE) {
     launch_typed<VecTypes<float, float, float, false>>(A, x, y, sc, grid, st, fin);
+  } else if (kind == TYPED_MIDDLE_WIDE) {
+    PG_REQUIRE(A.wide && A.wide->srec.p, "typed Horner launch (wide middle): the matrix has no wide image (ensure_wide_image)");
+    launch_typed<VecF32Wide>(*A.wide, x, y, sc, grid, st, fin);
   } else {
     PG_REQUIRE(kind == TYPED_HANDOVER, "unknown typed Horner launch");
     launch_typed<VecTypes<float, double, double, false>>(A, x, y, sc, grid, st, fin);
@@ -1079,10 +1236,20 @@
   const int kmax = config().spmv_march_k > 0 ? std::max(1, std::min(MARCH_K, config().spmv_march_k)) : MARCH_K;
   pghost::MarchGeometry geo{MARCH_K, MARCH_KS, MARCH_REC, MARCH_W, RUN_INFO, kmax, A.geo_ext0, A.geo_lines, march_strip(),
                             has_geo(A) ? config().unit_order : 0};
+  if (A.is_wide) {
+    geo.R = MARCH_R_WIDE;
+    geo.W = MARCH_W_WIDE;
+    geo.slack = 16;
+    geo.K = MARCH_K_WIDE;
+    geo.kmax = std::min(kmax, MARCH_K_WIDE);
+  }
   std::vector<pghost::RowRange> fallback;
   i64 rows_m = 0;
   pghost::plan_march_units(A.n, runs, info, geo, mrec, fallback, rows_m, &ukeys, edges);
   A.rows_m = rows_m;
+  A.plane_rows_max = 0;
+  for (size_t q = 0; q + MARCH_REC <= mrec.size(); q += MARCH_REC)
+    for (int i = 0; i < (mrec[q] & 255); ++i) A.plane_rows_max = std::max(A.plane_rows_max, (mrec[q + 21 + 4 * i] >> 8) - (mrec[q + 21 + 4 * i] & 255));
   for (const auto& f : fallback) emit_u_rows(up, f.a, f.b, f.cnt);
 }
 
@@ -1391,6 +1558,7 @@
   laps.lap("    chunks: rowptr download");
   A.chunk_desc.release();
   A.nchunks = 0;
+  A.wide.reset();
   build_slices(A, rp);
 }
 
@@ -1404,6 +1572,30 @@
     for (int l = 1 + threadIdx.x; l < nrows; l += blockDim.x) c += (flags[r0 + l] & need) != need ? 1 : 0;
   }
   if (c) atomicAdd(out, c);
+}
+
+namespace {
+struct BorrowCsr {
+  CsrMatrix& W;
+  BorrowCsr(const CsrMatrix& A, CsrMatrix& W_) : W(W_) {
+    W.rowptr.p = A.rowptr.p; W.rowptr.n = A.rowptr.n;
+    W.col.p = A.col.p; W.col.n = A.col.n;
+    W.val.p = A.val.p; W.val.n = A.val.n;
+  }
+  ~BorrowCsr() {
+    W.rowptr.p = nullptr; W.rowptr.n = 0;
+    W.col.p = nullptr; W.col.n = 0;
+    W.val.p = nullptr; W.val.n = 0;
+  }
+};
+std::unique_ptr<CsrMatrix> new_wide(const CsrMatrix& A) {
+  std::unique_ptr<CsrMatrix> W(new CsrMatrix);
+  W->is_wide = true;
+  W->n = A.n; W->nnz = A.nnz;
+  W->geo_cell = A.geo_cell; W->geo_map = A.geo_map; W->geo_ext0 = A.geo_ext0; W->geo_lines = A.geo_lines;
+  W->want_units = A.want_units;
+  return W;
+}
 }
 
 template <class T>
@@ -1440,7 +1632,7 @@
   A.nslices_int = T.nslices_int;
   A.rows_u = T.rows_u; A.rows_p = T.rows_p; A.rows_g = T.rows_g; A.nnz_p = T.nnz_p; A.nnz_g = T.nnz_g;
   A.spmv_bytes = T.spmv_bytes;
-  A.nunits = T.nunits; A.rows_m = T.rows_m;
+  A.nunits = T.nunits; A.rows_m = T.rows_m; A.plane_rows_max = T.plane_rows_max;
   A.tiles_per_xcd = T.tiles_per_xcd; A.tile_ns = T.tile_ns;
   if (T.tiles_per_xcd > 0) clone_buf(A.tiles, T.tiles, st);
   else A.tiles.release();
@@ -1473,7 +1665,26 @@
                        A.col.p, A.val.p, A.g_col.p, A.g_val.p);
   PG_HIP(hipGetLastError());
   PG_HIP(hipStreamSynchronize(st));
+  A.wide.reset();
+  if (T.wide && !T.is_wide) {
+    std::unique_ptr<CsrMatrix> W = new_wide(A);
+    BorrowCsr mine(A, *W), theirs(T, *T.wide);
+    if (build_slices_like(*T.wide, *W)) A.wide = std::move(W);
+  }
   return true;
+}
+
+void ensure_wide_image(const CsrMatrix& Ac) {
+  CsrMatrix& A = const_cast<CsrMatrix&>(Ac);
+  if (A.wide || A.is_wide || A.n == 0 || !A.srec.p) return;
+  std::unique_ptr<CsrMatrix> W = new_wide(A);
+  {
+    BorrowCsr mine(A, *W);
+    int* rp = static_cast<int*>(pinned_scratch(0, sizeof(int) * (size_t)(A.n + 1)));
+    A.rowptr.download(rp, A.n + 1);
+    build_slices(*W, rp);
+  }
+  A.wide = std::move(W);
 }
 
 bool spmv_supports_preconditioner_product() { return (variant() & 64) != 0; }
diff --git a/penguin/jl_amd/csrc/pg_system.h b/penguin/jl_amd/csrc/pg_system.h
--- a/penguin/jl_amd/csrc/pg_system.h
+++ b/penguin/jl_amd/csrc/pg_system.h
@@ -1,4 +1,5 @@
 #pragma once
+#include <memory>
 #include <vector>
 
 #include "pg_stencil.h"
@@ -48,6 +49,9 @@
   DevBuf<double> g_val;
   DevBuf<int> mrec;
   i64 nunits = 0, rows_m = 0;
+  int plane_rows_max = 0;
+  std::unique_ptr<CsrMatrix> wide;
+  bool is_wide = false;
   DevBuf<int> e_meta;
   DevBuf<double> e_val;
   i64 rows_e = 0, e_slots = 0;
@@ -76,6 +80,7 @@
 };
 constexpr int SPMV_CHUNK_ENTRIES = 508;
 void build_spmv_chunks(CsrMatrix& A);
+void ensure_wide_image(const CsrMatrix& A);
 
 void build_numbering(const SysParams& P, const Slab& slab, Numbering& nb);
 void assemble_csr(const SysParams& P, const Slab& slab, const Numbering& nb, CsrMatrix& A, bool scale = true);
```
